# TrevorS/voxtral-mini-realtime-rs

Hardware: AMD Instinct MI355X
Metric: decode_tok_per_s (higher is better)
Workload: dtype f32

## Files before the change

voxtral-mini-realtime-rs_amd/csrc/vox_api.cpp:

```cpp
#include "../../include/voxtral_hip.h"
#include "vox_kernels.h"
#include "vox_page_pool.h"
#include "vox_host_base.h"

#include <dlfcn.h>
#include <fcntl.h>
#include <sys/mman.h>
#include <sys/stat.h>
#include <unistd.h>

#include <algorithm>
#include <array>
#include <cassert>
#include <chrono>
#include <cmath>
#include <cstdarg>
#include <cstdio>
#include <cstdlib>
#include <cstring>
#include <deque>
#include <map>
#include <mutex>
#include <string>
#include <unordered_map>
// ... 969 lines not shown

extern "C" int32_t vox_q4_model_load(vox_ctx* ctx, const char* path, vox_model** out) { return vox_q4_model_load_ex(ctx, path, 0, out); }

extern "C" int32_t vox_q4_model_load_gguf(vox_ctx* ctx, vox_gguf* g, uint32_t flags, vox_model** out) {
    ARGCHK(ctx && g && out, "null argument"); VOXCHK(ctx_bind(ctx));
    GgufSource src; src.g = g;
    const int32_t r = model_build(ctx, &src, true, (flags & VOX_LOAD_LAYOUT_ONLY) != 0, out);
    src.g = nullptr;
    return r;
}
extern "C" int32_t vox_q4_model_load_ex(vox_ctx* ctx, const char* path, uint32_t flags, vox_model** out) {
    ARGCHK(ctx && path && out, "null argument"); VOXCHK(ctx_bind(ctx));
    GgufSource src; VOXCHK(vox_gguf_open(path, &src.g));
    return model_build(ctx, &src, true, (flags & VOX_LOAD_LAYOUT_ONLY) != 0, out);
}

extern "C" int32_t vox_f32_model_load(vox_ctx* ctx, const char* path, vox_model** out) {
    ARGCHK(ctx && path && out, "null argument"); VOXCHK(ctx_bind(ctx));
    SafeTensorsSource src; VOXCHK(src.open(path));
    return model_build(ctx, &src, false, false, out);
}

extern "C" int32_t vox_model_config(const vox_model* m, vox_model_cfg* out) { ARGCHK(m && out, "null argument"); *out = m->cfg; return VOX_OK; }
extern "C" int32_t vox_model_weight_bytes(const vox_model* m, uint64_t* out) { ARGCHK(m && out, "null argument"); *out = m->arena_bytes; return VOX_OK; }
extern "C" int32_t vox_model_memory(const vox_model* m, uint64_t out[4]) {
    ARGCHK(m && out, "null argument");
    out[0] = m->arena_bytes; out[1] = m->arena_primary_bytes;
    out[2] = (m->eng_stream ? eng_stream_bytes(m->cfg.dec_layers, m->cfg.vocab) : 0) + (m->eng_wob ? engb_wo_stream_bytes(m->cfg.dec_layers) : 0);
    out[3] = m->eng_state ? eng_state_bytes() : 0;
    for (int gi = 0; gi < 4; gi++) if (m->engb_state[gi]) out[3] += engb_state_bytes();
    return VOX_OK;
}
extern "C" int32_t vox_model_arena(const vox_model* m, void** p, uint64_t* n) { ARGCHK(m && p && n, "null argument"); *p = m->arena; *n = m->arena_primary_bytes; return VOX_OK; }
extern "C" int32_t vox_model_arena_finalize(vox_model* m) {
    ARGCHK(m, "null argument"); VOXCHK(ctx_bind(m->ctx));
    for (Q4W* w : m->tiled) HIPCHK(launch_q4_tile_build(*w, const_cast<uint4*>(w->qt), const_cast<uint16_t*>(w->st), m->ctx->stream));
    HIPCHK(hipStreamSynchronize(m->ctx->stream));
    m->eng_ready = false; m->eng_offline.cache = nullptr;
    prefix_release(m);
    if (m->eng_wob) { HIPCHK(hipStreamSynchronize(m->ctx->stream)); (void)hipFree(m->eng_wob); m->eng_wob = nullptr; }
    graphs_destroy(m);
    return VOX_OK;
}

extern "C" int32_t vox_model_replicate(const vox_model* src, vox_ctx* dst_ctx, vox_model** out) {
    ARGCHK(src && dst_ctx && out, "null argument");
    if (!src->is_q4 || src->manifest.empty()) return fail(VOX_ERR_UNSUPPORTED, "vox_model_replicate: Q4 (GGUF) models only");
    VOXCHK(ctx_bind(src->ctx)); HIPCHK(hipStreamSynchronize(src->ctx->stream));
    VOXCHK(ctx_bind(dst_ctx));
    ManifestSource ms; ms.m = &src->manifest;
    vox_model* d = nullptr;
    VOXCHK(model_build(dst_ctx, &ms, true, true, &d));
    if (d->arena_primary_bytes != src->arena_primary_bytes || d->arena_bytes != src->arena_bytes) { model_release(d); return fail(VOX_ERR_INVALID, "internal: replica arena layout differs from the source's"); }
    hipError_t e = src->ctx->device == dst_ctx->device ? hipMemcpyAsync(d->arena, src->arena, src->arena_primary_bytes, hipMemcpyDeviceToDevice, dst_ctx->stream)
                                                       : hipMemcpyPeerAsync(d->arena, dst_ctx->device, src->arena, src->ctx->device, src->arena_primary_bytes, dst_ctx->stream);
    if (e == hipSuccess) e = hipStreamSynchronize(dst_ctx->stream);
    if (e != hipSuccess) { model_release(d); return fail(VOX_ERR_HIP, "vox_model_replicate: device copy failed: %s", hipGetErrorString(e)); }
    const int32_t r = vox_model_arena_finalize(d);
    if (r != VOX_OK) { model_release(d); return r; }
    *out = d; return VOX_OK;
}

extern "C" int32_t vox_model_set_t_embed(vox_model* m, const float* t_embed) {
    ARGCHK(m && t_embed, "null argument"); VOXCHK(ctx_bind(m->ctx));
    const vox_model_cfg& c = m->cfg; vox_ctx* cx = m->ctx;
    if (m->t_embed_set && m->t_embed_host.size() == (size_t)c.dec_dim && !std::memcmp(m->t_embed_host.data(), t_embed, (size_t)c.dec_dim * 4)) return VOX_OK;
    DevBuf dt, dh, ones; HIPCHK(dt.alloc((size_t)c.dec_dim * 4)); HIPCHK(dh.alloc((size_t)c.t_cond_dim * 4)); HIPCHK(ones.alloc((size_t)c.dec_dim * 4));
    std::vector<float> one(c.dec_dim, 1.0f);
    HIPCHK(hipMemcpyAsync(dt.p, t_embed, (size_t)c.dec_dim * 4, hipMemcpyHostToDevice, cx->stream));
    HIPCHK(hipMemcpyAsync(ones.p, one.data(), (size_t)c.dec_dim * 4, hipMemcpyHostToDevice, cx->stream));
    for (int i = 0; i < c.dec_layers; i++) {
        VOXCHK(q4_linear_dev(cx, m->dec[i].ada0.w, nullptr, dt.as<float>(), c.dec_dim, 1, dh.as<float>(), c.t_cond_dim, EPI_GELU));
        VOXCHK(q4_linear_dev(cx, m->dec[i].ada2.w, nullptr, dh.as<float>(), c.t_cond_dim, 1, m->dec[i].ada_mul, c.dec_dim, EPI_RESID, ones.as<float>(), c.dec_dim));
    }
    HIPCHK(hipStreamSynchronize(cx->stream));
    m->t_embed_host.assign(t_embed, t_embed + c.dec_dim); m->t_embed_set = true;
    m->pfx.dec_built = false;
    return VOX_OK;
}

static int conv_len(int L) { return (L + 2 - 3) / 2 + 1; }

static int32_t ensure(float** p, size_t* cap, size_t need) {
    if (*cap >= need) return VOX_OK;
    if (*p) HIPCHK(hipFree(*p));
    *p = nullptr; *cap = 0;
    HIPCHK(hipMalloc((void**)p, need * sizeof(float))); *cap = need; return VOX_OK;
}

static int enc_rows(int T) { return conv_len(conv_len(T)); }
static int enc_row_budget(const vox_model* m, const int* T, int n) {
    int mx = 0; for (int i = 0; i < n; i++) mx = std::max(mx, enc_rows(T[i]));
    const int r = m->cfg.reshape_factor; return n == 1 ? mx : (mx + r - 1) / r * r;
}
static size_t conv_scratch_floats(const vox_model* m, int T) {
    const int D = m->cfg.enc_dim, T1 = conv_len(T);
    return std::max((size_t)D * T1, (size_t)(T + 2) * m->cfg.n_mels + (size_t)(T1 + 2) * D) + 64;
}
static int32_t conv_stem_dev(vox_model* m, const float* d_mel, int T, float* c1, float* x) {
    const vox_model_cfg& c = m->cfg; hipStream_t s = m->ctx->stream; const int D = c.enc_dim, T1 = conv_len(T), S = conv_len(T1);
    const bool conv_mfma = m->conv1_g.qs && m->conv2_g.qs && !knob_str("VOX_CONV_VALU");
    if (conv_mfma) {
        const int Cm = c.n_mels;
        float* melT = c1; float* c1T = melT + (size_t)(T + 2) * Cm;
        HIPCHK(hipMemsetAsync(melT, 0, (size_t)Cm * 4, s)); HIPCHK(hipMemsetAsync(melT + (size_t)(T + 1) * Cm, 0, (size_t)Cm * 4, s));
        HIPCHK(hipMemsetAsync(c1T, 0, (size_t)D * 4, s)); HIPCHK(hipMemsetAsync(c1T + (size_t)(T1 + 1) * D, 0, (size_t)D * 4, s));
        HIPCHK(launch_transpose(d_mel, Cm, T, melT + Cm, s));
        { GemmParams g{}; g.w = m->conv1_g; g.x = melT; g.x_stride = 2 * Cm; g.M = T1; g.out = c1T + D; g.out_stride = D; g.bias = m->conv1_b; HIPCHK(launch_dense2_gemm(g, EPI_GELU, s)); }
        { GemmParams g{}; g.w = m->conv2_g; g.x = c1T; g.x_stride = 2 * D; g.M = S; g.out = x; g.out_stride = D; g.bias = m->conv2_b; HIPCHK(launch_dense2_gemm(g, EPI_GELU, s)); }
    } else {
        HIPCHK(launch_conv1d_gelu(d_mel, c.n_mels, T, m->conv1_w, m->conv1_b, D, c1, 0, s));
        HIPCHK(launch_conv1d_gelu(c1, D, T1, m->conv2_w, m->conv2_b, D, x, 1, s));
    }
    return VOX_OK;
}
static int enc_packed_rows_of(const vox_model* m, int T) { const int R = m->cfg.reshape_factor; return std::max((enc_rows(T) + R - 1) / R * R, R * 40); }
static long enc_packed_rows(const vox_model* m, const int* T, int n) { long r = 0; for (int i = 0; i < n; i++) r += enc_packed_rows_of(m, T[i]); return r; }
struct EncForms { long Mtot = 0; int ksp = 0, ksp_wo = 0, fused_rope = 0; };
static int32_t encode_batch_dev(vox_model* m, int n, const float* const* d_mels, const int* T, float* audio_out, int audio_rows, int* S4_out, long* audio_off_out = nullptr,
                                EncForms* forms = nullptr, int prefix_rows = 0) {
    const vox_model_cfg& c = m->cfg; vox_ctx* cx = m->ctx; hipStream_t s = cx->stream;
    const int D = c.enc_dim, H = c.enc_heads, hd = c.enc_head_dim, QD = H * hd, F = c.enc_ffn, R = c.reshape_factor;
    const bool packed = audio_off_out != nullptr;
    ARGCHK(n <= 128, "internal: encoder stack of %d utterances", n);
    const int S_pad = enc_row_budget(m, T, n);
    int T1max = 0; bool any = false;
    std::vector<int> S(n);
    for (int i = 0; i < n; i++) { S[i] = enc_rows(T[i]); S4_out[i] = S[i] / R; T1max = std::max(T1max, conv_len(T[i])); any = any || S4_out[i] > 0; }
    if (!any || S_pad <= 0) return VOX_OK;
    ARGCHK(S_pad <= m->enc_rope_len, "audio too long for the encoder RoPE table (%d > %d positions); chunk it (--max-mel-frames)", S_pad, m->enc_rope_len);
    std::vector<int> roff(n + 1, 0);
    if (packed) for (int i = 0; i < n; i++) roff[i + 1] = roff[i] + enc_packed_rows_of(m, T[i]);
    const int r0 = prefix_rows;
    ARGCHK(r0 == 0 || (n == 1 && !packed && r0 % R == 0 && r0 < S_pad && m->pfx.enc_built && r0 == m->pfx.RC), "internal: encoder prefix of %d rows", r0);
    const int Mfull = packed ? roff[n] : n * S_pad;
    const int Mtot = Mfull - r0, M4 = packed ? Mtot / R : n == 1 ? S4_out[0] - r0 / R : Mtot / R;
    ARGCHK(!m->pfx.capture || (n == 1 && !packed && r0 == 0 && m->pfx.capture_rows <= S_pad), "internal: prefix capture");
    ARGCHK(packed || n == 1 || audio_rows >= S_pad / R, "internal: audio row budget %d < %d", audio_rows, S_pad / R);
    int Tmax = 0; for (int i = 0; i < n; i++) Tmax = std::max(Tmax, T[i]);
    (void)T1max;
    const size_t c1_floats = conv_scratch_floats(m, Tmax);
    int ksp = 0;
    {
        const Q4W& w2 = m->enc[0].w2.w;
        const long wgs = (long)((w2.N + 127) / 128) * ((Mtot + 31) / 32);
        const bool geom_ok = w2.fmt == WFMT_Q4_0 && w2.qt && w2.st && w2.nb % 16 == 0 && Mtot > 48 && D % 4 == 0 && D <= 4096;
        if (geom_ok && wgs < 1024) ksp = 4;
        if (const char* e = knob_str("VOX_ENC_SPLITK")) ksp = geom_ok && atoi(e) > 1 ? std::min(atoi(e), w2.nb / 4) : 0;
        for (int l = 0; ksp && l < c.enc_layers; l++) if (m->enc[l].w2.w.fmt != WFMT_Q4_0 || !m->enc[l].w2.w.qt || m->enc[l].w2.w.nb / 4 < ksp) ksp = 0;
    }
    int ksp_wo = ksp ? 2 : 0;
    if (ksp) { if (const char* e = knob_str("VOX_ENC_SPLITK_WO")) ksp_wo = atoi(e) > 1 ? std::min(atoi(e), ksp) : 0; }
    for (int l = 0; ksp_wo && l < c.enc_layers; l++) if (m->enc[l].wo.w.fmt != WFMT_Q4_0 || !m->enc[l].wo.w.qt || m->enc[l].wo.w.nb / 4 < ksp_wo || m->enc[l].wo.w.nb % 4) ksp_wo = 0;
    const size_t need = c1_floats + (size_t)Mfull * D + (size_t)Mtot * D + (size_t)Mtot * QD * 4 + (size_t)Mtot * F + (size_t)(M4 + 1) * m->ad0.w.N + (size_t)ksp * Mtot * D + 1024;
    VOXCHK(ensure(&m->ws, &m->ws_floats, need));
    if (forms) { forms->Mtot = Mtot; forms->ksp = ksp; forms->ksp_wo = ksp_wo; forms->fused_rope = 0; }
    float* c1 = m->ws; float* x0 = c1 + c1_floats / 64 * 64; float* x = x0 + (size_t)r0 * D; float* xn = x0 + (size_t)Mfull * D; float* qkv = xn + (size_t)Mtot * D;
    float* att = qkv + (size_t)Mtot * QD * 3; float* ffn = att + (size_t)Mtot * QD; float* ah = ffn + (size_t)Mtot * F; float* w2p = ah + (size_t)(M4 + 1) * m->ad0.w.N;
    const int* d_len = nullptr; const int* d_roff = nullptr; const int* d_rpos = nullptr;
    if (n > 1 || packed) {
        HIPCHK(hipMemsetAsync(x, 0, (size_t)Mtot * D * 4, s));
        HIPCHK(hipMemsetAsync(att, 0, (size_t)Mtot * QD * 4, s));
        if (!m->d_seq_len) HIPCHK(hipMalloc((void**)&m->d_seq_len, 128 * sizeof(int)));
        m->h_seq_len.assign(S.begin(), S.end());
        HIPCHK(hipMemcpyAsync(m->d_seq_len, m->h_seq_len.data(), (size_t)n * 4, hipMemcpyHostToDevice, s));
        d_len = m->d_seq_len;
    }
    if (packed) {
        if (!m->d_seq_off) HIPCHK(hipMalloc((void**)&m->d_seq_off, 128 * sizeof(int)));
        if (m->row_pos_cap < (size_t)Mtot) { if (m->d_row_pos) { HIPCHK(hipStreamSynchronize(s)); HIPCHK(hipFree(m->d_row_pos)); } m->d_row_pos = nullptr; m->row_pos_cap = 0;
                                              HIPCHK(hipMalloc((void**)&m->d_row_pos, (size_t)Mtot * sizeof(int))); m->row_pos_cap = (size_t)Mtot; }
        HIPCHK(hipStreamSynchronize(s));
        m->h_seq_off.assign(roff.begin(), roff.begin() + n); m->h_row_pos.resize((size_t)Mtot);
        for (int i = 0; i < n; i++) for (int r = roff[i]; r < roff[i + 1]; r++) m->h_row_pos[(size_t)r] = std::min(r - roff[i], m->enc_rope_len - 1);
        HIPCHK(hipMemcpyAsync(m->d_seq_off, m->h_seq_off.data(), (size_t)n * 4, hipMemcpyHostToDevice, s)); HIPCHK(hipMemcpyAsync(m->d_row_pos, m->h_row_pos.data(), (size_t)Mtot * 4, hipMemcpyHostToDevice, s));
        d_roff = m->d_seq_off; d_rpos = m->d_row_pos;
    }
    for (int i = 0; i < n; i++) {
        if (S[i] <= 0) continue;
        VOXCHK(conv_stem_dev(m, d_mels[i], T[i], c1, x0 + (packed ? (size_t)roff[i] : (size_t)i * S_pad) * D));
    }
    const int seq_rows = packed ? 0 : n > 1 ? S_pad : 0;
    for (int l = 0; l < c.enc_layers; l++) {
        const EncLayer& L = m->enc[l];
        if (ksp && l > 0) HIPCHK(launch_rms_norm_sumk(x, D, Mtot, D, w2p, (size_t)Mtot * D, ksp, L.attn_norm, c.norm_eps, xn, D, s));
        else HIPCHK(launch_rms_norm(x, D, Mtot, D, L.attn_norm, nullptr, c.norm_eps, xn, D, s));
        if (Mtot > 48) {
            GemmParams g{}; g.w = L.wqkv.w; g.x = xn; g.x_stride = D; g.M = Mtot; g.out = qkv; g.out_stride = 3 * QD; g.bias = L.wqkv.bias;
            g.rope_cos = m->enc_cos + (size_t)r0 * (hd / 2); g.rope_sin = m->enc_sin + (size_t)r0 * (hd / 2);
            g.hd = hd; g.n_q = 2 * QD; g.pos = d_rpos; g.rope_seq_rows = seq_rows;
            bool fused = false; HIPCHK(launch_q4_gemm(g, EPI_ROPE_ROWS, s, &fused));
            if (forms && fused) forms->fused_rope++;
        } else {
            VOXCHK(q4_linear_dev(cx, L.wqkv.w, L.wqkv.bias, xn, D, Mtot, qkv, 3 * QD));
            HIPCHK(launch_rope(qkv, Mtot, 3 * QD, 2 * QD, hd, r0, m->enc_cos, m->enc_sin, s, seq_rows, d_rpos));
        }
        if (m->pfx.capture)
            HIPCHK(hipMemcpy2DAsync(m->pfx.capture + (size_t)l * m->pfx.capture_rows * 2 * QD, (size_t)2 * QD * 4, qkv + QD, (size_t)3 * QD * 4, (size_t)2 * QD * 4, (size_t)m->pfx.capture_rows,
                                    hipMemcpyDeviceToDevice, s));
        AttnParams ap{}; ap.q = qkv; ap.q_stride = 3 * QD; ap.k = qkv + QD; ap.v = qkv + 2 * QD; ap.kv_row_stride = 3 * QD; ap.kv_head_stride = hd;
        ap.out = att; ap.out_stride = QD; ap.M = S_pad - r0; ap.kv_len = S_pad; ap.n_heads = H; ap.n_kv_heads = H; ap.offset = r0; ap.window = c.enc_window;
        if (r0) { ap.prefix_k = m->pfx.enc_kv + (size_t)l * r0 * 2 * QD; ap.prefix_v = ap.prefix_k + QD; ap.prefix_len = r0; ap.prefix_row_stride = 2 * QD; ap.prefix_head_stride = hd; }
        ap.seq_len = d_len; ap.q_seq_stride = S_pad * 3 * QD; ap.out_seq_stride = S_pad * QD; ap.kv_seq_stride = (long)S_pad * 3 * QD; ap.seq_row_off = d_roff;
        HIPCHK(launch_attn_prefill(ap, hd, s, n));
        if (ksp_wo) {
            VOXCHK(q4_linear_dev(cx, L.wo.w, L.wo.bias, att, QD, Mtot, w2p, D, EPI_STORE, nullptr, 0, ksp_wo));
            HIPCHK(launch_rms_norm_sumk(x, D, Mtot, D, w2p, (size_t)Mtot * D, ksp_wo, L.ffn_norm, c.norm_eps, xn, D, s));
        } else {
            VOXCHK(q4_linear_dev(cx, L.wo.w, L.wo.bias, att, QD, Mtot, x, D, EPI_RESID, x, D));
            HIPCHK(launch_rms_norm(x, D, Mtot, D, L.ffn_norm, nullptr, c.norm_eps, xn, D, s));
        }
        VOXCHK(q4_linear_dev(cx, L.w13.w, nullptr, xn, D, Mtot, ffn, F, EPI_SWIGLU));
        if (ksp) VOXCHK(q4_linear_dev(cx, L.w2.w, L.w2.bias, ffn, F, Mtot, w2p, D, EPI_STORE, nullptr, 0, ksp));
        else VOXCHK(q4_linear_dev(cx, L.w2.w, L.w2.bias, ffn, F, Mtot, x, D, EPI_RESID, x, D));
    }
    if (ksp && c.enc_layers > 0) HIPCHK(launch_rms_norm_sumk(x, D, Mtot, D, w2p, (size_t)Mtot * D, ksp, m->enc_norm, c.norm_eps, xn, D, s));
    else HIPCHK(launch_rms_norm(x, D, Mtot, D, m->enc_norm, nullptr, c.norm_eps, xn, D, s));
    VOXCHK(q4_linear_dev(cx, m->ad0.w, nullptr, xn, D * R, M4, ah, m->ad0.w.N, EPI_GELU));
    if (packed) { for (int i = 0; i < n; i++) audio_off_out[i] = (long)(roff[i] / R) * c.dec_dim; }
    if (packed || n == 1 || audio_rows * R == S_pad) VOXCHK(q4_linear_dev(cx, m->ad2.w, nullptr, ah, m->ad0.w.N, M4, audio_out + (size_t)(r0 / R) * c.dec_dim, c.dec_dim));
    else for (int i = 0; i < n; i++)
        VOXCHK(q4_linear_dev(cx, m->ad2.w, nullptr, ah + (size_t)i * (S_pad / R) * m->ad0.w.N, m->ad0.w.N, S_pad / R, audio_out + (size_t)i * audio_rows * c.dec_dim, c.dec_dim));
    return VOX_OK;
}
static int32_t encode_dev(vox_model* m, const float* d_mel, int T, int* S4_out, int prefix_rows = 0) {
    const int S4 = enc_rows(T) / m->cfg.reshape_factor;
    if (S4 > 0) { size_t cap = (size_t)m->audio_cap * m->cfg.dec_dim; VOXCHK(ensure(&m->d_audio, &cap, (size_t)S4 * m->cfg.dec_dim)); m->audio_cap = (int)(cap / m->cfg.dec_dim); }
    return encode_batch_dev(m, 1, &d_mel, &T, m->d_audio, S4, S4_out, nullptr, nullptr, prefix_rows);
}

static int32_t cache_alloc(vox_model* m, int max_seq, vox_cache** out) {
    const vox_model_cfg& c = m->cfg;
    ARGCHK(max_seq > 0 && max_seq <= m->dec_rope_len, "max_seq %d out of range (1..%d)", max_seq, m->dec_rope_len);
    vox_cache* k = new vox_cache(); k->m = m; k->ctx = m->ctx; k->max_seq = max_seq;
    const size_t n = (size_t)c.dec_layers * c.dec_kv_heads * max_seq * c.dec_head_dim * 4;
    if (hipMalloc((void**)&k->k, n) != hipSuccess || hipMalloc((void**)&k->v, n) != hipSuccess) { if (k->k) (void)hipFree(k->k); delete k; return fail(VOX_ERR_HIP, "hipMalloc of KV cache failed"); }
    HIPCHK(hipMemsetAsync(k->k, 0, n, m->ctx->stream)); HIPCHK(hipMemsetAsync(k->v, 0, n, m->ctx->stream));
    k->layer_stride = (size_t)c.dec_kv_heads * max_seq * c.dec_head_dim;
    cache_register(k);
    *out = k; return VOX_OK;
}
extern "C" int32_t vox_decoder_cache_create(vox_model* m, int32_t max_seq, vox_cache** out) { ARGCHK(m && out, "null argument"); VOXCHK(ctx_bind(m->ctx)); return cache_alloc(m, max_seq, out); }
extern "C" int32_t vox_cache_free(vox_cache* k) {
    if (!k) return VOX_OK;
    (void)hipSetDevice(k->ctx->device); (void)hipStreamSynchronize(k->ctx->stream);
    cache_release(k); return VOX_OK;
}
static int32_t pw_sync(vox_model* m);
static int32_t cache_settle_pending(vox_cache* kc) {
    vox_model* m = kc->m;
    if (m && m->pw_pend_rows > 0 && m->pw_pend_cache == kc) { VOXCHK(ctx_bind(kc->ctx)); VOXCHK(pw_sync(m)); }
    return VOX_OK;
}
extern "C" int32_t vox_cache_update(vox_cache* kc, int32_t layer, int32_t pos, const float* k, const float* v, int32_t n_rows, int32_t mem_kind) {
    ARGCHK(kc && k && v && n_rows > 0 && pos >= 0, "bad argument"); VOXCHK(ctx_bind(kc->ctx)); VOXCHK(cache_settle_pending(kc));
    const vox_model_cfg& c = kc->m->cfg;
    const int L = kc->kind == 1 ? c.enc_layers : c.dec_layers, H = kc->kind == 1 ? c.enc_heads : c.dec_kv_heads, hd = kc->kind == 1 ? c.enc_head_dim : c.dec_head_dim;
    ARGCHK(layer >= 0 && layer < L, "layer %d out of range (0..%d)", layer, L - 1);
    ARGCHK(pos + n_rows <= kc->max_seq, "KV cache overflow: %d + %d > %d", pos, n_rows, kc->max_seq);
    hipStream_t s = kc->ctx->stream; const hipMemcpyKind kind = mem_kind == VOX_MEM_DEVICE ? hipMemcpyDeviceToDevice : hipMemcpyHostToDevice;
    for (int h = 0; h < H; h++) {
        const size_t dst = (size_t)layer * kc->layer_stride + ((size_t)h * kc->max_seq + pos) * hd, src = (size_t)h * n_rows * hd, nb = (size_t)n_rows * hd * 4;
        HIPCHK(hipMemcpyAsync(kc->k + dst, k + src, nb, kind, s)); HIPCHK(hipMemcpyAsync(kc->v + dst, v + src, nb, kind, s));
    }
    if (mem_kind != VOX_MEM_DEVICE) HIPCHK(hipStreamSynchronize(s));
    kc->len = std::max(kc->len, pos + n_rows);
    return VOX_OK;
}
extern "C" int32_t vox_cache_truncate(vox_cache* kc, int32_t len) {
    ARGCHK(kc, "null cache"); VOXCHK(cache_settle_pending(kc)); ARGCHK(len >= 0 && len <= kc->len, "truncate to %d: the cache holds %d rows", len, kc->len);
    if (kc->kind == 1) kc->abs_pos -= kc->len - len;
    kc->len = len; return VOX_OK;
}
extern "C" int32_t vox_cache_seq_len(const vox_cache* k, int32_t* out) { ARGCHK(k && out, "null argument"); *out = k->len; return VOX_OK; }
extern "C" int32_t vox_cache_reset(vox_cache* k) {
    ARGCHK(k, "null cache");
    (void)cache_settle_pending(k);
    k->len = 0; k->abs_pos = 0; return VOX_OK;
}

extern "C" int32_t vox_encoder_cache_create(vox_model* m, int32_t capacity_rows, vox_cache** out) {
    ARGCHK(m && out, "null argument"); VOXCHK(ctx_bind(m->ctx));
    const vox_model_cfg& c = m->cfg;
    if (capacity_rows <= 0) capacity_rows = 2 * c.enc_window + 512;
    ARGCHK(capacity_rows > c.enc_window, "encoder cache capacity %d must exceed the sliding window (%d)", capacity_rows, c.enc_window);
    vox_cache* k = new vox_cache(); k->m = m; k->ctx = m->ctx; k->max_seq = capacity_rows; k->kind = 1;
    const size_t n = (size_t)c.enc_layers * c.enc_heads * capacity_rows * c.enc_head_dim * 4;
    if (hipMalloc((void**)&k->k, n) != hipSuccess || hipMalloc((void**)&k->v, n) != hipSuccess) { if (k->k) (void)hipFree(k->k); delete k; return fail(VOX_ERR_HIP, "hipMalloc of encoder KV cache failed"); }
    HIPCHK(hipMemsetAsync(k->k, 0, n, m->ctx->stream)); HIPCHK(hipMemsetAsync(k->v, 0, n, m->ctx->stream));
    k->layer_stride = (size_t)c.enc_heads * capacity_rows * c.enc_head_dim;
    cache_register(k);
    *out = k; return VOX_OK;
}
extern "C" int32_t vox_cache_abs_pos(const vox_cache* k, int32_t* out) { ARGCHK(k && out, "null argument"); *out = k->kind == 1 ? k->abs_pos : k->len; return VOX_OK; }

static int32_t enc_cache_evict(vox_model* m, vox_cache* kc, int keep) {
    const vox_model_cfg& c = m->cfg; hipStream_t s = m->ctx->stream;
    if (keep >= kc->len) return VOX_OK;
    const size_t planes = (size_t)c.enc_layers * c.enc_heads, pitch = (size_t)kc->max_seq * c.enc_head_dim * 4, width = (size_t)keep * c.enc_head_dim * 4;
    VOXCHK(ensure(&m->ws, &m->ws_floats, planes * width / 4 + 64));
    for (float* base : {kc->k, kc->v}) {
        const char* src = reinterpret_cast<const char*>(base) + (size_t)(kc->len - keep) * c.enc_head_dim * 4;
        HIPCHK(hipMemcpy2DAsync(m->ws, width, src, pitch, width, planes, hipMemcpyDeviceToDevice, s));
        HIPCHK(hipMemcpy2DAsync(base, pitch, m->ws, width, width, planes, hipMemcpyDeviceToDevice, s));
    }
    kc->len = keep;
    return VOX_OK;
}
extern "C" int32_t vox_encoder_cache_apply_sliding_window(vox_cache* kc, int32_t window) {
    ARGCHK(kc && kc->kind == 1 && window > 0, "bad argument"); VOXCHK(ctx_bind(kc->ctx));
    VOXCHK(enc_cache_evict(kc->m, kc, window)); HIPCHK(hipStreamSynchronize(kc->ctx->stream)); return VOX_OK;
}

static int32_t enc_stream_rope_ensure(vox_model* m) {
    if (m->enc_cos_s) return VOX_OK;
    const vox_model_cfg& c = m->cfg; const int hd = c.enc_head_dim;
    const int len = 1 << 16, half = hd / 2; std::vector<float> ct((size_t)len * half), st((size_t)len * half);
    for (int i = 0; i < len; i++) for (int j = 0; j < half; j++) { const float inv = 1.0f / std::pow(c.rope_theta, (float)(2 * j) / (float)hd), fr = (float)i * inv; ct[(size_t)i * half + j] = std::cos(fr); st[(size_t)i * half + j] = std::sin(fr); }
    HIPCHK(hipMalloc((void**)&m->enc_cos_s, ct.size() * 4)); HIPCHK(hipMalloc((void**)&m->enc_sin_s, st.size() * 4));
    HIPCHK(hipMemcpy(m->enc_cos_s, ct.data(), ct.size() * 4, hipMemcpyHostToDevice)); HIPCHK(hipMemcpy(m->enc_sin_s, st.data(), st.size() * 4, hipMemcpyHostToDevice));
    m->enc_rope_s_len = len;
    return VOX_OK;
}
static int32_t encode_with_cache_dev(vox_model* m, const float* d_mel, int T, vox_cache* kc, int* S4_out) {
    const vox_model_cfg& c = m->cfg; vox_ctx* cx = m->ctx; hipStream_t s = cx->stream;
    const int D = c.enc_dim, H = c.enc_heads, hd = c.enc_head_dim, QD = H * hd, F = c.enc_ffn, R = c.reshape_factor;
    const int S = enc_rows(T), S4 = S / R; *S4_out = S4;
    if (S <= 0) return VOX_OK;
    ARGCHK(S <= kc->max_seq - std::min(c.enc_window, kc->max_seq - 1), "chunk of %d encoder rows does not fit a cache of %d rows next to the %d-row window", S, kc->max_seq, c.enc_window);
    if (kc->len + S > kc->max_seq) VOXCHK(enc_cache_evict(m, kc, std::min(kc->len, c.enc_window)));
    const float *cos_t = m->enc_cos, *sin_t = m->enc_sin;
    if (kc->abs_pos + S > m->enc_rope_len) {
        VOXCHK(enc_stream_rope_ensure(m));
        ARGCHK(kc->abs_pos + S <= m->enc_rope_s_len, "stream of %d encoder positions exceeds the streaming RoPE table (%d)", kc->abs_pos + S, m->enc_rope_s_len);
        cos_t = m->enc_cos_s; sin_t = m->enc_sin_s;
    }
    if (S4 > 0) { size_t cap = (size_t)m->audio_cap * c.dec_dim; VOXCHK(ensure(&m->d_audio, &cap, (size_t)S4 * c.dec_dim)); m->audio_cap = (int)(cap / c.dec_dim); }
    const size_t c1f = conv_scratch_floats(m, T);
    const size_t need = c1f + (size_t)S * D * 2 + (size_t)S * QD * 4 + (size_t)S * F + (size_t)(S4 + 1) * m->ad0.w.N + 1024;
    VOXCHK(ensure(&m->ws, &m->ws_floats, need));
    float* c1 = m->ws; float* x = c1 + c1f / 64 * 64; float* xn = x + (size_t)S * D; float* qkv = xn + (size_t)S * D;
    float* att = qkv + (size_t)S * QD * 3; float* ffn = att + (size_t)S * QD; float* ah = ffn + (size_t)S * F;
    VOXCHK(conv_stem_dev(m, d_mel, T, c1, x));
    const int off = kc->len; const size_t lf = kc->layer_stride;
    for (int l = 0; l < c.enc_layers; l++) {
        const EncLayer& L = m->enc[l]; float* kl = kc->k + (size_t)l * lf; float* vl = kc->v + (size_t)l * lf;
        HIPCHK(launch_rms_norm(x, D, S, D, L.attn_norm, nullptr, c.norm_eps, xn, D, s));
        VOXCHK(q4_linear_dev(cx, L.wqkv.w, L.wqkv.bias, xn, D, S, qkv, 3 * QD));
        HIPCHK(launch_rope(qkv, S, 3 * QD, 2 * QD, hd, kc->abs_pos, cos_t, sin_t, s, 0));
        HIPCHK(launch_kv_store(qkv, S, 3 * QD, QD, H, hd, off, kl, vl, kc->max_seq * hd, s));
        AttnParams ap{}; ap.q = qkv; ap.q_stride = 3 * QD; ap.k = kl; ap.v = vl; ap.kv_row_stride = hd; ap.kv_head_stride = kc->max_seq * hd;
        ap.out = att; ap.out_stride = QD; ap.M = S; ap.kv_len = off + S; ap.n_heads = H; ap.n_kv_heads = H; ap.offset = off; ap.window = c.enc_window;
        HIPCHK(launch_attn_prefill(ap, hd, s, 1));
        VOXCHK(q4_linear_dev(cx, L.wo.w, L.wo.bias, att, QD, S, x, D, EPI_RESID, x, D));
        HIPCHK(launch_rms_norm(x, D, S, D, L.ffn_norm, nullptr, c.norm_eps, xn, D, s));
        VOXCHK(q4_linear_dev(cx, L.w13.w, nullptr, xn, D, S, ffn, F, EPI_SWIGLU));
        VOXCHK(q4_linear_dev(cx, L.w2.w, L.w2.bias, ffn, F, S, x, D, EPI_RESID, x, D));
    }
    kc->len = off + S; kc->abs_pos += S;
    if (S4 > 0) {
        HIPCHK(launch_rms_norm(x, D, S4 * R, D, m->enc_norm, nullptr, c.norm_eps, xn, D, s));
        VOXCHK(q4_linear_dev(cx, m->ad0.w, nullptr, xn, D * R, S4, ah, m->ad0.w.N, EPI_GELU));
        VOXCHK(q4_linear_dev(cx, m->ad2.w, nullptr, ah, m->ad0.w.N, S4, m->d_audio, c.dec_dim));
    }
    return VOX_OK;
}
// ... 3218 lines not shown
```

voxtral-mini-realtime-rs_amd/csrc/vox_kernels.h:

```cpp
#pragma once
#include <hip/hip_runtime.h>
#include <atomic>
struct DevOnce {
    std::atomic<uint64_t> mask{0};
    bool done(int dev) const { return (mask.load(std::memory_order_acquire) >> (dev & 63)) & 1ull; }
    void set(int dev) { mask.fetch_or(1ull << (dev & 63), std::memory_order_release); }
};
static inline int vox_current_device() { int d = 0; if (hipGetDevice(&d) != hipSuccess) { (void)hipGetLastError(); d = 0; } return d; }
#include <stdint.h>

namespace vox {

struct Q4W {
    const uint4* qs;
    const uint16_t* sc;
    int N, K, nb;
    int fmt;
    const uint4* qt = nullptr; const uint16_t* st = nullptr;
};
enum WFmt { WFMT_Q4_0 = 0, WFMT_BF16 = 1, WFMT_BF16X2 = 2, WFMT_F32 = 3 };

enum Epi { EPI_STORE = 0, EPI_RESID = 1, EPI_SWIGLU = 2, EPI_ROPE_KV = 3, EPI_ARGMAX = 4, EPI_GELU = 5, EPI_SWIGLU_XF = 6, EPI_RESID_XF = 7,
           EPI_ROPE_ROWS = 8,
           EPI_ROPE_KV_PAGED = 9 };
enum Pro { PRO_NONE = 0, PRO_RMS = 1, PRO_RMS_MUL = 2,
           PRO_RMS_MUL_SUM = 3 };

struct GemvParams {
    Q4W w;
    const float* x; int x_stride;
    float* out; int out_stride;
    const float* bias;
    const float* resid; int resid_stride;
    const float* gamma; const float* mul; float eps;
    long long* zero_acc; int zero_n;
    const long long* xacc; float* x_out;
    const int* pos_ptr; int pos_off;
    const float* rope_cos; const float* rope_sin; int hd;
    int n_q, n_k;
    float* kcache; float* vcache; int cache_head_stride;
    float* part_val; int* part_idx;
    int tl_slot;
};
hipError_t launch_q4_gemv(const GemvParams& p, int n_rows_x, int pro, int epi, int R, hipStream_t s);
const char* q4_gemv_kernel_name(int K, int pro, int epi, int R);
int q4_gemv_default_R(int N, int K, int epi);
int q4_gemv_grid(int N, int R);
int q4_gemv_nwv(int K, int epi);
int q4_gemv_grid_k(int N, int K, int R, int epi);
int dense_gemv_grid(int N);

struct GemmParams {
    Q4W w;
    const float* x; int x_stride; int M;
    float* out; int out_stride;
    const float* bias;
    const float* resid; int resid_stride;
    const uint4* xf;
    uint16_t* xf_scratch; size_t xf_scratch_bytes;
    const float* ssq_part; int n_part; float norm_eps;
    uint16_t* xf_out; const float* xf_w; const float* xf_w2; float* ssq_out;
    const int* pos; const float* rope_cos; const float* rope_sin; int hd, n_q, n_kv; float* kc; float* vc; long kv_seq_stride; int kv_head_stride;
    const int* kv_row;
    const int* kv_pos;
    int tl_slot;
    int ksplit;
    float* kz_scratch; size_t kz_scratch_bytes;
    int rope_seq_rows;
    int wide_mt; long xf_gstride , xf_out_gstride , ssq_part_gstride, ssq_out_gstride ;
    int wide_rows;
};
struct WidePlan { int kz, sps, ntw; };
bool q4_wide_plan(const Q4W& w, int mt, int epi, WidePlan* pl);
size_t q4_wide_planes_bytes(const Q4W& w, int mt, const WidePlan& pl);
hipError_t launch_q4_wide(const GemmParams& p, int epi, hipStream_t s);
hipError_t launch_q4_tile_build(Q4W w, uint4* qt, uint16_t* st, hipStream_t s);
hipError_t launch_q4_gemm(const GemmParams& p, int epi, hipStream_t s, bool* fused_rope = nullptr);
hipError_t launch_dense2_gemm(const GemmParams& p, int epi, hipStream_t s);
hipError_t launch_transpose(const float* in, int R, int C, float* out, hipStream_t s);
int q4_skinny_resid_xf_parts(int N);

hipError_t launch_q4_repack(const uint8_t* raw, uint4* qs, uint16_t* sc, int64_t n_blocks, int nb, int row_mul, int row_add, hipStream_t s);
hipError_t launch_q4_dequant(Q4W w, float* out, hipStream_t s);
hipError_t launch_rms_norm(const float* x, int x_stride, int rows, int dim, const float* gamma, const float* mul,
                           float eps, float* out, int out_stride, hipStream_t s);
hipError_t launch_rms_norm_sumk(float* x, int x_stride, int rows, int dim, const float* part, size_t part_stride, int ksplit, const float* gamma, float eps, float* out, int out_stride, hipStream_t s);
int q4_skinny_mt2_plan(const Q4W& w, int M);
hipError_t launch_xf_rows(const float* x, int x_stride, int M, int K, uint16_t* xf, hipStream_t s);
hipError_t launch_q4_skinny_mt2_planes(const GemmParams& p, int KZ, hipStream_t s);
hipError_t launch_splitk_finish_resid(const float* planes, int KZ, int M, int N, float* x, int x_stride, hipStream_t s);
hipError_t launch_splitk_finish_swiglu_xf(const float* planes, int KZ, int M, int N, const float* bias, uint16_t* xf, hipStream_t s);
hipError_t launch_splitk_finish_rope_kv(const float* planes, int KZ, int M, int N, float* q_out, int q_stride, int n_q, int n_kv, int hd, int pos_off,
                                        const float* cos_t, const float* sin_t, float* kc, float* vc, int head_stride, hipStream_t s);
hipError_t launch_rms_norm_xf_sumk(float* x, int x_stride, int rows, int dim, const float* planes, int kz, const float* gamma, const float* mul, float eps, uint16_t* xf, hipStream_t s);
hipError_t launch_rms_norm_xf(const float* x, int x_stride, int rows, int dim, const float* gamma, const float* mul,
                              float eps, uint16_t* xf, hipStream_t s);
hipError_t launch_rope(float* buf, int M, int stride, int n_rot, int hd, int pos_off, const float* cos_t,
                       const float* sin_t, hipStream_t s, int seq_rows = 0, const int* row_pos = nullptr);
hipError_t launch_kv_store(const float* buf, int M, int stride, int k_col, int n_kv, int hd, int pos_off,
                           float* kcache, float* vcache, int cache_head_stride, hipStream_t s, int seq_rows = 0, long kv_seq_stride = 0);

struct AttnParams {
    const float* q; int q_stride;
    const float* k; const float* v;
    int kv_row_stride, kv_head_stride;
    float* out; int out_stride;
    int M, kv_len, n_heads, n_kv_heads, offset, window;
    const int* pos_ptr;
    int pos_per_seq; int q_seq_stride, out_seq_stride; long kv_seq_stride;
    const int* kv_row;
    const int* seq_len;
    const int* seq_row_off;
    uint16_t* out_xf_tiles; long out_xf_tile_stride;
    uint16_t* out_xf;
    long out_xf_gstride;
    int prefer_gqa;
    int no_xcd_remap;
    int tl_slot;
    int spec_zero;
    int spec_rows;
    const float* prefix_k; const float* prefix_v; int prefix_len, prefix_row_stride, prefix_head_stride;
    const int* page_tab; int page_tab_stride, page_shift, score_rows; long page_floats;
};
hipError_t launch_attn_prefill(const AttnParams& p, int hd, hipStream_t s, int n_seq = 1);
bool attn_prefill_prefix_ok(const AttnParams& p, int hd, int n_seq);
bool attn_prefill_small_ok(const AttnParams& p, int hd, int n_seq);
hipError_t launch_attn_decode(const AttnParams& p, int hd, int max_seq, hipStream_t s, int n_seq = 1);
hipError_t launch_attn_decode_paged(const AttnParams& p, int hd, hipStream_t s, int n_seq);
bool attn_wo_supported(const AttnParams& p, const Q4W& wo, int hd, int max_seq);
hipError_t launch_attn_wo(const AttnParams& p, const Q4W& wo, long long* acc, int max_seq, hipStream_t s);
enum AttnForm { ATTN_FORM_PREFILL_SMALL, ATTN_FORM_PREFILL_MFMA, ATTN_FORM_PREFILL_F32, ATTN_FORM_DECODE, ATTN_FORM_DECODE_SPEC, ATTN_FORM_DECODE_GQA, ATTN_FORM_WO,
                ATTN_FORM_ENGINE, ATTN_FORM_STREAM_RING, ATTN_FORM_GROUP_RESAMPLE, ATTN_FORM_STREAM_RESAMPLE,
                ATTN_FORM_DECODE_PAGED, ATTN_FORM_DECODE_GQA_PAGED,
                ATTN_FORM_COUNT };
void attn_form_note(AttnForm f);
void attn_form_counts(unsigned long long out[ATTN_FORM_COUNT]);
enum GemmForm { GEMM_FORM_GEMV_R1, GEMM_FORM_GEMV_R2, GEMM_FORM_GEMV_R4, GEMM_FORM_DENSE_GEMV, GEMM_FORM_SKINNY, GEMM_FORM_SKINNY_MT, GEMM_FORM_SKINNY_MT2, GEMM_FORM_XF_ROWS,
                GEMM_FORM_SPLITK_FINISH, GEMM_FORM_TILE_11, GEMM_FORM_TILE_12, GEMM_FORM_TILE_21, GEMM_FORM_TILE_22, GEMM_FORM_TILE_21_TB, GEMM_FORM_TILE_22_TB, GEMM_FORM_K32,
                GEMM_FORM_BIG, GEMM_FORM_BIG_ROPE, GEMM_FORM_DENSE2, GEMM_FORM_WIDE, GEMM_FORM_COUNT };
void gemm_form_counts(unsigned long long out[GEMM_FORM_COUNT]);

hipError_t launch_conv1d_gelu(const float* in, int Cin, int L, const float* w, const float* b, int Cout, float* out,
                              int out_token_major, hipStream_t s);

struct MelTables { const float* window; const float* cos_t; const float* sin_t; const float* fb; const int* fb_lo; const int* fb_hi; };
hipError_t launch_mel(const float* audio, long n, long left, long right, const float* scale_ptr, MelTables t,
                      float* out, int T, int transposed, hipStream_t s);
hipError_t launch_resample_matrix(const double* H, int new_len, int fft_in, int fft_out, float* At, hipStream_t s);
hipError_t launch_resample(const float* x, long n_in, const float* At, int fft_in, int fft_out, int delay, float* out, long n_out, hipStream_t s);
hipError_t launch_absmax(const float* x, long n, float target_peak, float* scale_out, hipStream_t s);
hipError_t launch_absmax_group(const float* x, long n, unsigned* group_max_cell, hipStream_t s);
hipError_t launch_group_scale(const unsigned* group_max, const int* unit_group, int n, float target, float* unit_scale, hipStream_t s);

hipError_t launch_embed(Q4W tok, const int* ids, int n, const float* audio, int D, const int* pos_ptr, int id_off,
                        int a_off, float* out, hipStream_t s);
hipError_t launch_argmax_final(const float* part_val, const int* part_idx, int n_parts, int* tokens, int* pos_ptr,
                               int tok_off, int inc, hipStream_t s);
hipError_t launch_argmax_embed(const float* part_val, const int* part_idx, int n_parts, int* tokens, int* pos_ptr, Q4W tok,
                               const float* audio, int D, float* h, hipStream_t s);
hipError_t launch_rope_kv_batch(float* qkv, int n, int stride, int n_q, int n_kv, int hd, const int* pos, const float* cos_t, const float* sin_t,
                                float* kcache, float* vcache, long seq_stride, int head_stride, hipStream_t s);
hipError_t launch_argmax_embed_batch(const float* logits, int n, int vocab, int* tokens, int tok_stride, int* pos, const int* seq_len, Q4W tok,
                                     const float* audio, long audio_seq_stride, int D, float* h, hipStream_t s,
                                     uint16_t* xf = nullptr, const float* xf_w = nullptr, float* ssq_out = nullptr,
                                     long xf_group_stride = 0, int ssq_group_stride = 0,
                                     const long* audio_off = nullptr);
struct SlotStepParams {
    const float* logits; int vocab;
    int* tokens; int tok_stride; const int* clip_len;
    int* slot_clip; int* slot_qpos; const int* queue; int q_stride;
    int* pos; int* kv_row; int n_clips; int first_pos;
    Q4W tok; const float* audio; const long* audio_off; int D;
    const float* h0;
    float* h;
    uint16_t* xf; const float* xf_w; float* ssq_out; long xf_group_stride; int ssq_group_stride;
    int init;
};
hipError_t launch_argmax_embed_slots(const SlotStepParams& p, int n_slots, hipStream_t s);
struct BatchTapParams {
    const float* logits; int vocab;
    const int* slot_clip; int clip0; const int* pos; const int* seq_len;
    const int* clip_unit; int n_clips;
    float* out; int* rows; int n_units, max_rows, first_pos;
};
hipError_t launch_batch_tap(const BatchTapParams& p, int n_rows, hipStream_t s);
hipError_t launch_occupy(int workgroups, int micros, hipStream_t s);
hipError_t launch_add_rows(const float* a, const float* b, float* out, long n, hipStream_t s);
hipError_t launch_gelu(float* x, long n, hipStream_t s);
hipError_t launch_argmax_rows(const float* x, int rows, int V, int* out, hipStream_t s);

struct EngLayerTab { const float* attn_norm; const float* ffn_norm; const float* ada_mul; float* kc; float* vc; };
struct EngParams {
    const unsigned char* stream; size_t cu_stride;
    const EngLayerTab* layers; int n_layers;
    const float* h_in;
    const float* final_norm;
    const int* pos_ptr; int pos_off;
    const float* rope_cos; const float* rope_sin;
    int max_seq, window; float eps;
    unsigned long long *H0, *H1, *G, *PW, *A, *P2;
    unsigned long long *SS0, *SS1;
    unsigned long long* XC;
    unsigned* serial; unsigned* err;
    float* part_val; int* part_idx;
    int* tokens; int* pos_rw; const uint4* tok_qs; const uint16_t* tok_sc; int tok_nb; const float* audio;
    float* logits_out;
    int vocab;
    unsigned long long* tl; int tl_layer;
    int flags;
    int ag_delay_ticks;
    int pace_ticks;
};
bool eng_geometry_ok(int D, int n_heads, int n_kv, int hd, int ffn, int vocab, int max_seq);
size_t eng_stream_bytes(int n_layers, int vocab);
size_t eng_state_bytes();
hipError_t launch_eng_pack(const Q4W& w, int op, int layer, int n_layers, unsigned char* stream, int vocab, hipStream_t s);
void eng_state_carve(unsigned char* state, EngParams* p);
hipError_t launch_decode_engine(const EngParams& p, hipStream_t s);
hipError_t launch_eng_hidden(const EngParams& p, float* out, hipStream_t s);
hipError_t eng_occupancy(int* blocks_per_cu);
int eng_lds_bytes();

struct EngBParams {
    const unsigned char* stream;
    const unsigned char* stream_wo;
    const EngLayerTab* layers; int n_layers;
    long kv_seq_stride;
    const float* h_in; int h_stride; int n_rows;
    const float* final_norm;
    const int* pos;
    const int* kv_row;
    const float* rope_cos; const float* rope_sin;
    int max_seq, window; float eps;
    unsigned char *XH0, *XH1;
    float *SS0, *SS1;
    unsigned long long* G;
    unsigned char* XO;
    float* PW;
    unsigned char* XA;
    float* P2;
    unsigned *F0, *F1, *FO, *FW, *FA, *F2;
    unsigned long long* XC; unsigned* serial; unsigned* err;
    uint16_t* xf_out; float* ssq_out;
    unsigned long long* tl; int tl_layer;
    int flags;
};
size_t engb_state_bytes();
size_t engb_wo_stream_bytes(int n_layers);
void engb_state_carve(unsigned char* state, EngBParams* p);
hipError_t engb_state_init(unsigned char* state, hipStream_t s);
hipError_t launch_decode_engine_b16(const EngBParams& p, hipStream_t s);
hipError_t launch_decode_engine_b16x2(const EngBParams& a, const EngBParams& b, hipStream_t s);
hipError_t engb_occupancy(int* blocks_per_cu);
hipError_t engb_prepare_kernels();
hipError_t launch_engb_ssq_fold(const float* ssq256, float* ssq16, hipStream_t s);
int engb_lds_bytes();
int engb_lds_bytes2();

void knobs_load_once();
void knobs_reload();
#define VOX_NO_PK_F32 __attribute__((target("no-packed-fp32-ops")))
const char* knob_str(const char* name);

hipError_t tl_configure(unsigned long long* buf, int n_slots, int n_waves);
int tl_slots_used();
void tl_slot_meta(int slot, int out[4]);

enum StreamWord { STRM_POS = 0,
                  STRM_ENC_POS = 1,
                  STRM_FRAME = 2,
                  STRM_HEAD = 3,
                  STRM_TICKS = 4,
                  STRM_TAP_ROWS = 5,
                  STRM_WORDS = 16 };
struct TokenScore { float logprob, margin; int runner_up, id; };
static const int VOX_ALTS_MAX = 8;
struct TokenAlt { int id; float logprob; };
struct TokenAlts { float entropy; int n; TokenAlt alt[VOX_ALTS_MAX]; };
// ... 65 lines not shown
```

voxtral-mini-realtime-rs_amd/csrc/vox_kernels.hip:

```cpp
#include "vox_kernels.h"

#include <hip/hip_fp16.h>

#include <unistd.h>

#include <algorithm>
#include <atomic>
#include <cstdio>
#include <cstdlib>
#include <cstring>
#include <string>
#include <mutex>
#include <unordered_map>

namespace vox {

static int g_tl_next = -1, g_tl_slots = 0;
#ifdef VOX_TIMELINE
__device__ unsigned long long* g_tl_buf = nullptr;
__device__ int g_tl_waves = 0;
__device__ __forceinline__ void tl_stamp(int slot, int wave_global, int k) {
    if (slot >= 0 && (wave_global & 3) == 0 && (threadIdx.x & 63) == 0 && g_tl_buf && wave_global < g_tl_waves)
        g_tl_buf[((size_t)slot * g_tl_waves + wave_global) * 4 + k] = wall_clock64();
}
// ... 555 lines not shown
    __syncthreads();
    int best_i = 0x7fffffff; float best = -INFINITY;
    const int pos = (EPI == EPI_ROPE_KV) ? (p.pos_ptr ? *p.pos_ptr : 0) + p.pos_off : 0;
    const int n_groups = N / R, n_waves = gridDim.x * 4;
    for (int g = blockIdx.x * 4 + wave; g < n_groups; g += n_waves) {
        const int row0 = g * R;
        const uint4* w0 = (F32W ? p.w.qt : p.w.qs) + (size_t)row0 * nc * (F32W ? 2 : 1);
        const uint4* w1 = w0 + nc * (F32W ? 2 : 1);
        float acc[R] = {0.f, 0.f};
        for (int c0 = 0; c0 < nc; c0 += 128) {
            const int ca = c0 + lane, cb = ca + 64, cca = min(ca, nc - 1), ccb = min(cb, nc - 1);
            const float4 xea = xe[cca], xoa = xo[cca], xeb = xe[ccb], xob = xo[ccb];
            const float ma = ca < nc ? 1.0f : 0.0f, mb = cb < nc ? 1.0f : 0.0f;
            if (F32W) {
                const uint4 a0e = ld_nt_u4(w0 + 2 * cca), a0o = ld_nt_u4(w0 + 2 * cca + 1), a1e = ld_nt_u4(w0 + 2 * ccb), a1o = ld_nt_u4(w0 + 2 * ccb + 1);
                const uint4 b0e = ld_nt_u4(w1 + 2 * cca), b0o = ld_nt_u4(w1 + 2 * cca + 1), b1e = ld_nt_u4(w1 + 2 * ccb), b1o = ld_nt_u4(w1 + 2 * ccb + 1);
                acc[0] += ma * dot8_f32(a0e, a0o, xea, xoa) + mb * dot8_f32(a1e, a1o, xeb, xob);
                acc[1] += ma * dot8_f32(b0e, b0o, xea, xoa) + mb * dot8_f32(b1e, b1o, xeb, xob);
            } else {
                const uint4 a0 = ld_nt_u4(w0 + cca), a1 = ld_nt_u4(w0 + ccb), b0 = ld_nt_u4(w1 + cca), b1 = ld_nt_u4(w1 + ccb);
                acc[0] += ma * dot8_bf16(a0, xea, xoa) + mb * dot8_bf16(a1, xeb, xob);
                acc[1] += ma * dot8_bf16(b0, xea, xoa) + mb * dot8_bf16(b1, xeb, xob);
            }
        }
        acc[0] = wave_sum(acc[0]); acc[1] = wave_sum(acc[1]);
        if (EPI == EPI_STORE || EPI == EPI_RESID || EPI == EPI_GELU) {
#pragma unroll
            for (int r = 0; r < R; r++) {
                const int n = row0 + r;
                if (lane == r) {
                    float v = acc[r];
                    if (p.bias) v += p.bias[n];
                    if (EPI == EPI_RESID) v = v + p.resid[(size_t)y * p.resid_stride + n];
                    if (EPI == EPI_GELU) v = gelu_f(v);
                    p.out[(size_t)y * p.out_stride + n] = v;
                }
            }
        } else if (EPI == EPI_SWIGLU) {
            if (lane == 0) p.out[(size_t)y * p.out_stride + (row0 >> 1)] = silu_f(acc[0]) * acc[1];
        } else if (EPI == EPI_ROPE_KV) {
            const int hd = p.hd, half = hd >> 1, n = row0;
            if (lane == 0) {
                const float a = acc[0], b = acc[1];
                if (n < p.n_q + p.n_k) {
                    const int dd = n % hd;
                    const float c = p.rope_cos[(size_t)pos * half + (dd >> 1)], sn = p.rope_sin[(size_t)pos * half + (dd >> 1)];
                    const float ra = a * c - b * sn, rb = a * sn + b * c;
                    if (n < p.n_q) { p.out[n] = ra; p.out[n + 1] = rb; }
                    else {
                        const int kn = n - p.n_q, kh = kn / hd;
                        float* dst = p.kcache + (size_t)kh * p.cache_head_stride + (size_t)pos * hd + dd;
                        dst[0] = ra; dst[1] = rb;
                    }
                } else {
                    const int vn = n - p.n_q - p.n_k, vh = vn / hd, dd = vn % hd;
                    float* dst = p.vcache + (size_t)vh * p.cache_head_stride + (size_t)pos * hd + dd;
                    dst[0] = a; dst[1] = b;
                }
            }
        } else if (EPI == EPI_ARGMAX) {
#pragma unroll
            for (int r = 0; r < R; r++) {
                const int n = row0 + r;
                if (p.out && lane == r) p.out[(size_t)y * p.out_stride + n] = acc[r];
                argmax_take(best, best_i, acc[r], n);
            }
        }
    }
    if (EPI == EPI_ARGMAX) {
        if (lane == 0) { red[4 + wave] = best; reinterpret_cast<int*>(red)[8 + wave] = best_i; }
        __syncthreads();
        if (tid == 0) {
            float bv = red[4]; int bidx = reinterpret_cast<int*>(red)[8];
            for (int wv = 1; wv < 4; wv++) argmax_take(bv, bidx, red[4 + wv], reinterpret_cast<int*>(red)[8 + wv]);
            p.part_val[(size_t)y * gridDim.x + blockIdx.x] = bv;
            p.part_idx[(size_t)y * gridDim.x + blockIdx.x] = bidx;
        }
    }
}

int dense_gemv_grid(int N) { const int wgs = (N / 2 + 3) / 4; return wgs > 2048 ? 2048 : (wgs < 1 ? 1 : wgs); }

template <int PRO, int EPI>
static hipError_t dense_launch_t(const GemvParams& p, int ny, hipStream_t s) {
    const size_t lds = (size_t)(p.w.K + 16) * sizeof(float);
    gemm_form_note(GEMM_FORM_DENSE_GEMV);
    if (p.w.fmt == WFMT_F32) dense_gemv_kernel<PRO, EPI, 1><<<dim3(dense_gemv_grid(p.w.N), ny), dim3(256), lds, s>>>(p);
    else dense_gemv_kernel<PRO, EPI, 0><<<dim3(dense_gemv_grid(p.w.N), ny), dim3(256), lds, s>>>(p);
    return hipGetLastError();
}
static hipError_t launch_dense_gemv(const GemvParams& p, int ny, int pro, int epi, hipStream_t s) {
    if (p.w.K % 32 || p.w.K > 10240 || p.w.N % 2) return hipErrorInvalidValue;
    if ((pro == PRO_RMS_MUL || pro == PRO_RMS_MUL_SUM) && p.mul == nullptr) return hipErrorInvalidValue;
    if (pro == PRO_RMS_MUL_SUM) return hipErrorInvalidValue;
#define VOX_CASE(P_, E_) if (pro == P_ && epi == E_) return dense_launch_t<P_, E_>(p, ny, s)
    VOX_CASE(PRO_NONE, EPI_STORE); VOX_CASE(PRO_NONE, EPI_RESID); VOX_CASE(PRO_NONE, EPI_GELU); VOX_CASE(PRO_NONE, EPI_SWIGLU);
    VOX_CASE(PRO_RMS, EPI_STORE); VOX_CASE(PRO_RMS, EPI_ARGMAX); VOX_CASE(PRO_RMS, EPI_SWIGLU); VOX_CASE(PRO_RMS_MUL, EPI_SWIGLU);
    VOX_CASE(PRO_RMS, EPI_ROPE_KV);
#undef VOX_CASE
    return hipErrorInvalidValue;
}

typedef __attribute__((__vector_size__(8 * sizeof(__bf16)))) __bf16 bf16x8;
typedef __attribute__((__vector_size__(4 * sizeof(float)))) float f32x4;

__device__ __forceinline__ uint32_t bf16_rne_bits(float x) {
    const uint32_t u = __float_as_uint(x);
    return (u + 0x7FFFu + ((u >> 16) & 1u)) >> 16;
}
typedef __bf16 bf16x2_t __attribute__((ext_vector_type(2)));
typedef float f32x2_t __attribute__((ext_vector_type(2)));
__device__ __forceinline__ uint32_t cvt_pk_bf16(float a, float b) {
    const f32x2_t v = {a, b};
    union { bf16x2_t b; uint32_t u; } c; c.b = __builtin_convertvector(v, bf16x2_t); return c.u;
}
__device__ __forceinline__ void split_pair(float a, float b, uint32_t& hi, uint32_t& lo) {
    hi = cvt_pk_bf16(a, b);
    lo = cvt_pk_bf16(a - __uint_as_float(hi << 16), b - __uint_as_float(hi & 0xFFFF0000u));
}
__device__ __forceinline__ void split_bf16x8(const float4 a, const float4 b, uint4& hi, uint4& lo) {
    split_pair(a.x, a.y, hi.x, lo.x); split_pair(a.z, a.w, hi.y, lo.y);
    split_pair(b.x, b.y, hi.z, lo.z); split_pair(b.z, b.w, hi.w, lo.w);
}
__device__ __forceinline__ uint32_t pack_bf16_exact(float a, float b) {
    return (__float_as_uint(a) >> 16) | (__float_as_uint(b) & 0xFFFF0000u);
}
__device__ __forceinline__ uint4 q4_dword_to_bf16x8(uint32_t w) {
    const uint32_t lo = w & 0x0F0F0F0Fu, hi = (w >> 4) & 0x0F0F0F0Fu;
    uint4 o;
    o.x = pack_bf16_exact(ub0(lo) - 8.0f, ub1(lo) - 8.0f);
    o.y = pack_bf16_exact(ub2(lo) - 8.0f, ub3(lo) - 8.0f);
    o.z = pack_bf16_exact(ub0(hi) - 8.0f, ub1(hi) - 8.0f);
    o.w = pack_bf16_exact(ub2(hi) - 8.0f, ub3(hi) - 8.0f);
    return o;
}
__device__ __forceinline__ bf16x8 as_bf16x8(uint4 v) {
    union { uint4 u; bf16x8 b; } c; c.u = v; return c.b;
}

__device__ __forceinline__ uint4 q4_dword_to_bf16x8_biased(uint32_t w) {
    const uint32_t lo = w & 0x0F0F0F0Fu, hi = (w >> 4) & 0x0F0F0F0Fu, c = 0x43434343u;
    return make_uint4(__builtin_amdgcn_perm(lo, c, 0x00060004u), __builtin_amdgcn_perm(hi, c, 0x00060004u),
                      __builtin_amdgcn_perm(lo, c, 0x00070005u), __builtin_amdgcn_perm(hi, c, 0x00070005u));
}

__device__ __forceinline__ void xf_store4(uint16_t* __restrict__ xf, int K, int row, int k, float4 v) {
    const int q = k >> 7, j = (k >> 5) & 3, e = k & 31, half = e >> 4, g = (e & 15) >> 2;
    const size_t base = ((size_t)((q * 4 + j) * 64 + g * 16 + row)) * 8 + 2 * half;
    const size_t plane = (size_t)(K >> 7) * 256 * 8;
    uint32_t hi, lo;
    split_pair(v.x, v.z, hi, lo); *reinterpret_cast<uint32_t*>(xf + base) = hi; *reinterpret_cast<uint32_t*>(xf + plane + base) = lo;
    split_pair(v.y, v.w, hi, lo); *reinterpret_cast<uint32_t*>(xf + base + 4) = hi; *reinterpret_cast<uint32_t*>(xf + plane + base + 4) = lo;
}

template <int EPI, int FMT>
__global__ __launch_bounds__(256) __attribute__((amdgpu_waves_per_eu(2))) void q4_gemm_k32_kernel(const GemmParams p) {
    __shared__ __attribute__((aligned(16))) uint4 lds[2][2][256];
    const int K = p.w.K, nb = p.w.nb, N = p.w.N, M = p.M;
    (void)K;
    const int tid = threadIdx.x, lane = tid & 63, wave = tid >> 6;
    const int m0 = blockIdx.y * 64, n0 = blockIdx.x * 64;
    const int sm = tid >> 2, sg = tid & 3;
    const bool srow_ok = (m0 + sm) < M;
    const float* xrow = p.x + (size_t)(srow_ok ? (m0 + sm) : 0) * p.x_stride;
    const int slot = ((sm >> 4) * 4 + sg) * 16 + (sm & 15);
    const int wn = n0 + wave * 16 + (lane & 15), wg = lane >> 4;
    const bool wrow_ok = wn < N;
    const uint32_t* wq = reinterpret_cast<const uint32_t*>(p.w.qs) + (size_t)(wrow_ok ? wn : 0) * nb * 4 + wg;
    const uint16_t* ws = FMT == WFMT_Q4_0 ? p.w.sc + (size_t)(wrow_ok ? wn : 0) * nb : nullptr;
    const uint4* wd16 = p.w.qs + (size_t)(wrow_ok ? wn : 0) * nb * 4 + wg;
    const int xoff_a = FMT == WFMT_Q4_0 ? 4 * sg : 8 * sg, xoff_b = FMT == WFMT_Q4_0 ? 16 + 4 * sg : 8 * sg + 4;

    f32x4 acc[4];
#pragma unroll
    for (int i = 0; i < 4; i++) acc[i] = (f32x4){0.f, 0.f, 0.f, 0.f};

#define VOX_GLOAD(B_)                                                                              \
    xa = *reinterpret_cast<const float4*>(xrow + 32 * (B_) + xoff_a);        \
    xb = *reinterpret_cast<const float4*>(xrow + 32 * (B_) + xoff_b);                                               \
    if (FMT == WFMT_Q4_0) { wd = wq[(size_t)(B_) * 4]; wsc = ws[(B_)]; }    \
    else { wdv = wd16[(size_t)(B_) * 4]; }
#define VOX_STAGE(BUF_)                                                                            \
    { uint4 hi_, lo_; split_bf16x8(xa, xb, hi_, lo_); lds[(BUF_)][0][slot] = hi_; lds[(BUF_)][1][slot] = lo_; }
    float4 xa, xb; uint32_t wd = 0; uint16_t wsc = 0; uint4 wdv = make_uint4(0, 0, 0, 0);
    VOX_GLOAD(0)
    VOX_STAGE(0)
    uint32_t cur_wd = wd; uint16_t cur_sc = wsc; uint4 cur_wdv = wdv;
    { const int b1 = min(1, nb - 1); VOX_GLOAD(b1) }
    __syncthreads();
    for (int b = 0; b < nb; b++) {
        const int buf = b & 1;
        const float4 sxa = xa, sxb = xb; const uint32_t swd = wd; const uint16_t ssc = wsc; const uint4 swdv = wdv;
        { const int b2 = min(b + 2, nb - 1); VOX_GLOAD(b2) }
        const bf16x8 bw = as_bf16x8(FMT == WFMT_Q4_0 ? q4_dword_to_bf16x8(cur_wd) : cur_wdv);
        const float d = FMT == WFMT_Q4_0 ? f16_bits_to_f32(cur_sc) : 1.0f;
#pragma unroll
        for (int mt = 0; mt < 4; mt++) {
            const bf16x8 ah = as_bf16x8(lds[buf][0][mt * 64 + lane]);
            const bf16x8 al = as_bf16x8(lds[buf][1][mt * 64 + lane]);
            f32x4 t = __builtin_amdgcn_mfma_f32_16x16x32_bf16(ah, bw, (f32x4){0.f, 0.f, 0.f, 0.f}, 0, 0, 0);
            t = __builtin_amdgcn_mfma_f32_16x16x32_bf16(al, bw, t, 0, 0, 0);
            acc[mt][0] = fmaf(d, t[0], acc[mt][0]); acc[mt][1] = fmaf(d, t[1], acc[mt][1]);
            acc[mt][2] = fmaf(d, t[2], acc[mt][2]); acc[mt][3] = fmaf(d, t[3], acc[mt][3]);
        }
        if (b + 1 < nb) {
            uint4 hi_, lo_; split_bf16x8(sxa, sxb, hi_, lo_); lds[buf ^ 1][0][slot] = hi_; lds[buf ^ 1][1][slot] = lo_;
            cur_wd = swd; cur_sc = ssc; cur_wdv = swdv;
        }
        __syncthreads();
    }
#undef VOX_GLOAD
#undef VOX_STAGE
    const float bias = (p.bias && wrow_ok) ? p.bias[wn] : 0.f;
#pragma unroll
    for (int mt = 0; mt < 4; mt++)
#pragma unroll
        for (int r = 0; r < 4; r++) {
            const int m = m0 + mt * 16 + 4 * (lane >> 4) + r;
            float v = acc[mt][r] + bias;
            if (EPI == EPI_SWIGLU) {
                const float other = dpp_mov<0xB1>(v);
                if (m < M && wrow_ok && !(wn & 1)) p.out[(size_t)m * p.out_stride + (wn >> 1)] = silu_f(v) * other;
            } else if (m < M && wrow_ok) {
                if (EPI == EPI_RESID) v = v + p.resid[(size_t)m * p.resid_stride + wn];
                if (EPI == EPI_GELU) v = gelu_f(v);
                p.out[(size_t)m * p.out_stride + wn] = v;
            }
        }
}

template <int MT, int NT, int EPI, int FMT, int TB = 0>
__global__ __launch_bounds__(256) __attribute__((amdgpu_waves_per_eu(2))) void q4_gemm_kernel(const GemmParams p) {
    extern __shared__ __attribute__((aligned(16))) uint4 glds[];
    constexpr int PLANE = 4 * MT * 64, BUF = 2 * PLANE;
    const int nb = p.w.nb, N = p.w.N, M = p.M, nq = nb >> 2;
    const int tid = threadIdx.x, lane = tid & 63, wave = tid >> 6;
    const int m0 = blockIdx.y * (16 * MT), n0 = blockIdx.x * (64 * NT);
    const int KSP = p.ksplit > 1 ? p.ksplit : 1, kz = blockIdx.z;
    const int qb = (int)((long)nq * kz / KSP), qe = (int)((long)nq * (kz + 1) / KSP);
    const float* xrow[MT]; int slot[MT], xo_a[MT], xo_b[MT];
#pragma unroll
    for (int i = 0; i < MT; i++) {
        const int f = tid + 256 * i, sm = f >> 4, j = (f >> 2) & 3, g = f & 3;
        xrow[i] = p.x + (size_t)min(m0 + sm, M - 1) * p.x_stride;
        slot[i] = (j * MT + (sm >> 4)) * 64 + g * 16 + ((sm & 15) ^ (4 * j + g));
        xo_a[i] = 32 * j + (FMT == WFMT_Q4_0 ? 4 * g : 8 * g); xo_b[i] = 32 * j + (FMT == WFMT_Q4_0 ? 16 + 4 * g : 8 * g + 4);
    }
    const int wg = lane >> 4;
    int rdl[4];
#pragma unroll
    for (int j = 0; j < 4; j++) rdl[j] = (lane & 48) | ((lane & 15) ^ (4 * j + wg));
    const uint32_t* wq[NT]; const uint16_t* ws[NT]; const uint4* wd16[NT]; const uint4* wqt[NT]; int wn[NT]; bool wok[NT];
#pragma unroll
    for (int t = 0; t < NT; t++) {
        wn[t] = n0 + (wave * NT + t) * 16 + (lane & 15); wok[t] = wn[t] < N;
        const size_t row = (size_t)min(wn[t], N - 1);
        wq[t] = reinterpret_cast<const uint32_t*>(p.w.qs) + row * nb * 4 + wg;
        ws[t] = FMT == WFMT_Q4_0 ? p.w.sc + row * nb : nullptr;
        wd16[t] = p.w.qs + row * nb * 4 + wg;
        const size_t T = (size_t)min((n0 >> 4) + wave * NT + t, ((N + 15) >> 4) - 1);
        wqt[t] = TB ? p.w.qt + T * nq * 64 + lane : nullptr;
    }
    f32x4 acc[NT][MT];
#pragma unroll
    for (int t = 0; t < NT; t++)
#pragma unroll
        for (int i = 0; i < MT; i++) acc[t][i] = (f32x4){0.f, 0.f, 0.f, 0.f};

    float4 xa[MT], xb[MT];
    uint32_t wd[NT][4]; uint2 wsc[NT]; uint4 wdv[NT][4];
#define VOX_GLOAD(Q_)                                                                                          \
    _Pragma("unroll") for (int i = 0; i < MT; i++) {                                                           \
        xa[i] = *reinterpret_cast<const float4*>(xrow[i] + 128 * (Q_) + xo_a[i]);                              \
        xb[i] = *reinterpret_cast<const float4*>(xrow[i] + 128 * (Q_) + xo_b[i]);                              \
    }                                                                                                          \
    _Pragma("unroll") for (int t = 0; t < NT; t++) {                                                           \
        if (FMT == WFMT_Q4_0) {                                                                                \
            if (TB) { const uint4 w4 = ld_nt_u4(wqt[t] + (size_t)64 * (Q_)); wd[t][0] = w4.x; wd[t][1] = w4.y; wd[t][2] = w4.z; wd[t][3] = w4.w; } \
            else { _Pragma("unroll") for (int j = 0; j < 4; j++) wd[t][j] = wq[t][(size_t)(4 * (Q_) + j) * 4]; } \
            wsc[t] = *reinterpret_cast<const uint2*>(ws[t] + 4 * (Q_));                                        \
        } else {                                                                                               \
            _Pragma("unroll") for (int j = 0; j < 4; j++) wdv[t][j] = wd16[t][(size_t)(4 * (Q_) + j) * 4];     \
        }                                                                                                      \
    }
#define VOX_STAGE(BUF_)                                                                                        \
    _Pragma("unroll") for (int i = 0; i < MT; i++) {                                                           \
        uint4 hi_, lo_; split_bf16x8(sxa[i], sxb[i], hi_, lo_);                                                \
        glds[(BUF_) * BUF + slot[i]] = hi_; glds[(BUF_) * BUF + PLANE + slot[i]] = lo_;                        \
    }
    VOX_GLOAD(qb)
    float4 sxa[MT], sxb[MT];
#pragma unroll
    for (int i = 0; i < MT; i++) { sxa[i] = xa[i]; sxb[i] = xb[i]; }
    VOX_STAGE(0)
    uint32_t cwd[NT][4]; uint2 csc[NT]; uint4 cwdv[NT][4];
#pragma unroll
    for (int t = 0; t < NT; t++) { csc[t] = wsc[t];
#pragma unroll
        for (int j = 0; j < 4; j++) { cwd[t][j] = wd[t][j]; cwdv[t][j] = wdv[t][j]; } }
    { const int q1 = min(qb + 1, qe - 1); VOX_GLOAD(q1) }
    __syncthreads();
    for (int q = qb; q < qe; q++) {
        const int buf = (q - qb) & 1;
#pragma unroll
        for (int i = 0; i < MT; i++) { sxa[i] = xa[i]; sxb[i] = xb[i]; }
        uint32_t nwd[NT][4]; uint2 nsc[NT]; uint4 nwdv[NT][4];
#pragma unroll
        for (int t = 0; t < NT; t++) { nsc[t] = wsc[t];
#pragma unroll
            for (int j = 0; j < 4; j++) { nwd[t][j] = wd[t][j]; nwdv[t][j] = wdv[t][j]; } }
        { const int q2 = min(q + 2, qe - 1); VOX_GLOAD(q2) }
#pragma unroll
        for (int j = 0; j < 4; j++) {
#pragma unroll
            for (int t = 0; t < NT; t++) {
                const bf16x8 bw = as_bf16x8(FMT == WFMT_Q4_0 ? q4_dword_to_bf16x8(cwd[t][j]) : cwdv[t][j]);
                float d = 1.0f;
                if (FMT == WFMT_Q4_0) {
                    const uint32_t pr = (j & 2) ? csc[t].y : csc[t].x;
                    d = f16_bits_to_f32((uint16_t)((j & 1) ? (pr >> 16) : (pr & 0xFFFFu)));
                }
#pragma unroll
                for (int i = 0; i < MT; i++) {
                    const bf16x8 ah = as_bf16x8(glds[buf * BUF + (j * MT + i) * 64 + rdl[j]]);
                    const bf16x8 al = as_bf16x8(glds[buf * BUF + PLANE + (j * MT + i) * 64 + rdl[j]]);
                    f32x4 tt = __builtin_amdgcn_mfma_f32_16x16x32_bf16(ah, bw, (f32x4){0.f, 0.f, 0.f, 0.f}, 0, 0, 0);
                    tt = __builtin_amdgcn_mfma_f32_16x16x32_bf16(al, bw, tt, 0, 0, 0);
                    acc[t][i][0] = fmaf(d, tt[0], acc[t][i][0]); acc[t][i][1] = fmaf(d, tt[1], acc[t][i][1]);
                    acc[t][i][2] = fmaf(d, tt[2], acc[t][i][2]); acc[t][i][3] = fmaf(d, tt[3], acc[t][i][3]);
                }
            }
        }
        if (q + 1 < qe) {
            VOX_STAGE(buf ^ 1)
#pragma unroll
            for (int t = 0; t < NT; t++) { csc[t] = nsc[t];
#pragma unroll
                for (int j = 0; j < 4; j++) { cwd[t][j] = nwd[t][j]; cwdv[t][j] = nwdv[t][j]; } }
        }
        __syncthreads();
    }
#undef VOX_GLOAD
#undef VOX_STAGE
#pragma unroll
    for (int t = 0; t < NT; t++) {
        const float bias = (p.bias && wok[t] && kz == 0) ? p.bias[wn[t]] : 0.f;
#pragma unroll
        for (int i = 0; i < MT; i++)
#pragma unroll
            for (int r = 0; r < 4; r++) {
                const int m = m0 + i * 16 + 4 * (lane >> 4) + r;
                float v = acc[t][i][r] + bias;
                if (EPI == EPI_SWIGLU) {
                    const float other = dpp_mov<0xB1>(v);
                    if (m < M && wok[t] && !(wn[t] & 1)) p.out[(size_t)m * p.out_stride + (wn[t] >> 1)] = silu_f(v) * other;
                } else if (m < M && wok[t]) {
                    if (EPI == EPI_RESID) v = v + p.resid[(size_t)m * p.resid_stride + wn[t]];
                    if (EPI == EPI_GELU) v = gelu_f(v);
                    (p.out + (size_t)kz * p.M * p.out_stride)[(size_t)m * p.out_stride + wn[t]] = v;
                }
            }
    }
}

__global__ void q4_tile_build_kernel(Q4W w, uint4* __restrict__ qt, uint16_t* __restrict__ st, int n_tiles) {
    const int nq = w.nb >> 2;
    const long total = (long)n_tiles * nq * 64;
    for (long i = (long)blockIdx.x * blockDim.x + threadIdx.x; i < total; i += (long)gridDim.x * blockDim.x) {
        const int lane = (int)(i & 63); const long tq = i >> 6; const int q = (int)(tq % nq), T = (int)(tq / nq);
        const int g = lane >> 4, n = T * 16 + (lane & 15);
        uint32_t d[4] = {0x88888888u, 0x88888888u, 0x88888888u, 0x88888888u};
        if (n < w.N) {
            const uint32_t* src = reinterpret_cast<const uint32_t*>(w.qs) + ((size_t)n * w.nb + 4 * q) * 4 + g;
#pragma unroll
            for (int j = 0; j < 4; j++) d[j] = src[j * 4];
        }
        qt[i] = make_uint4(d[0], d[1], d[2], d[3]);
        if (g == 0) {
#pragma unroll
            for (int j = 0; j < 4; j++) st[(tq * 16 + (lane & 15)) * 4 + j] = n < w.N ? w.sc[(size_t)n * w.nb + 4 * q + j] : (uint16_t)0;
        }
    }
}
hipError_t launch_q4_tile_build(Q4W w, uint4* qt, uint16_t* st, hipStream_t s) {
    if (w.nb % 4) return hipErrorInvalidValue;
    const int n_tiles = (w.N + 15) / 16;
    q4_tile_build_kernel<<<dim3(2048), dim3(256), 0, s>>>(w, qt, st, n_tiles);
    return hipGetLastError();
}

template <int NTW, int EPI, int TILED, int XIN, int PRO, int STEPS = 0>
__global__ __launch_bounds__(NTW == 3 ? 256 : 512, NTW == 3 ? 3 : 1) void q4_skinny_kernel(const GemmParams p) {
    extern __shared__ __attribute__((aligned(16))) float sred[];
    __shared__ float s_rstd[16]; __shared__ float s_pp[32 * 16];
    constexpr bool KVP = EPI == EPI_ROPE_KV_PAGED, ROPE_KV = EPI == EPI_ROPE_KV || KVP;
    const int nb = p.w.nb, N = p.w.N, M = p.M, nq = nb >> 2;
    const int tid = threadIdx.x, lane = tid & 63, wave = tid >> 6, KS = blockDim.x >> 6;
    const int g = lane >> 4, li = lane & 15;
    const int nbase = blockIdx.x * (16 * NTW);
    const int tlw = wave == 0 ? (int)blockIdx.x * 4 : 1; (void)tlw;
    VOX_TL(p.tl_slot, tlw, 0);
    const float* xrow = p.x + (size_t)min(li, M - 1) * p.x_stride;
    const uint4* wq[NTW]; const uint16_t* ws[NTW];
    const int n_tiles = (N + 15) >> 4;
#pragma unroll
    for (int t = 0; t < NTW; t++) {
        if (TILED) {
            const size_t T = (size_t)min(blockIdx.x * NTW + t, n_tiles - 1);
            wq[t] = p.w.qt + T * nq * 64 + lane; ws[t] = p.w.st + (T * nq * 16 + li) * 4;
        } else {
            const size_t row = (size_t)min(nbase + t * 16 + li, N - 1);
            wq[t] = p.w.qs + row * nb + g; ws[t] = p.w.sc + row * nb;
        }
    }
    f32x4 acc[NTW];
#pragma unroll
    for (int t = 0; t < NTW; t++) acc[t] = (f32x4){0.f, 0.f, 0.f, 0.f};
    uint4 wv[NTW], wvn[NTW]; uint2 sv[NTW], svn[NTW]; float4 xa[4], xb[4];
    const uint4* xfh = p.xf + lane; const uint4* xfl = p.xf + (size_t)nq * 256 + lane;
#define VOX_WLOAD(WV_, SV_, Q_)                                                                            \
    _Pragma("unroll") for (int t = 0; t < NTW; t++) {                                                      \
        WV_[t] = ld_nt_u4(wq[t] + (TILED ? 64 : 4) * (Q_)); SV_[t] = *reinterpret_cast<const uint2*>(ws[t] + (TILED ? 64 : 4) * (Q_)); }
#define VOX_XLOAD(Q_)                                                                                      \
    _Pragma("unroll") for (int j = 0; j < 4; j++) {                                                        \
        if (XIN) {                                                                                         \
            xa[j] = *reinterpret_cast<const float4*>(xfh + ((Q_) * 4 + j) * 64);                           \
            xb[j] = *reinterpret_cast<const float4*>(xfl + ((Q_) * 4 + j) * 64);                           \
        } else {                                                                                           \
            xa[j] = *reinterpret_cast<const float4*>(xrow + 128 * (Q_) + 32 * j + 4 * g);                  \
            xb[j] = *reinterpret_cast<const float4*>(xrow + 128 * (Q_) + 32 * j + 16 + 4 * g); } }
#define VOX_SSTEP(WV_, SV_, XA_, XB_)                                                                      \
    {                                                                                                      \
        const bf16x8 m136 = as_bf16x8(make_uint4(0xC308C308u, 0xC308C308u, 0xC308C308u, 0xC308C308u));     \
        uint32_t dw[NTW][4];                                                                               \
        _Pragma("unroll") for (int t = 0; t < NTW; t++) {                                                  \
            dw[t][0] = WV_[t].x; dw[t][1] = WV_[t].y; dw[t][2] = WV_[t].z; dw[t][3] = WV_[t].w;            \
            if (!TILED) {                            \
                auto s01 = __builtin_amdgcn_permlane16_swap(WV_[t].x, WV_[t].y, false, false);             \
                auto s23 = __builtin_amdgcn_permlane16_swap(WV_[t].z, WV_[t].w, false, false);             \
                auto u02 = __builtin_amdgcn_permlane32_swap(s01[0], s23[0], false, false);                 \
                auto u13 = __builtin_amdgcn_permlane32_swap(s01[1], s23[1], false, false);                 \
                dw[t][0] = u02[0]; dw[t][1] = u13[0]; dw[t][2] = u02[1]; dw[t][3] = u13[1];                \
            }                                                                                              \
        }                                                                                                  \
               \
        _Pragma("unroll") for (int j = 0; j < 4; j++) {                                                    \
            uint4 ah, al;                                                                                  \
            if (XIN) {                                                                                     \
                ah = make_uint4(__float_as_uint(XA_[j].x), __float_as_uint(XA_[j].y), __float_as_uint(XA_[j].z), __float_as_uint(XA_[j].w)); \
                al = make_uint4(__float_as_uint(XB_[j].x), __float_as_uint(XB_[j].y), __float_as_uint(XB_[j].z), __float_as_uint(XB_[j].w)); \
            } else {                                                                                       \
                split_pair(XA_[j].x, XA_[j].z, ah.x, al.x); split_pair(XB_[j].x, XB_[j].z, ah.y, al.y);    \
                split_pair(XA_[j].y, XA_[j].w, ah.z, al.z); split_pair(XB_[j].y, XB_[j].w, ah.w, al.w);    \
            }                                                                                              \
            const f32x4 sx = __builtin_amdgcn_mfma_f32_16x16x32_bf16(as_bf16x8(ah), m136, (f32x4){0.f, 0.f, 0.f, 0.f}, 0, 0, 0); \
            const f32x4 cs = __builtin_amdgcn_mfma_f32_16x16x32_bf16(as_bf16x8(al), m136, sx, 0, 0, 0);    \
            _Pragma("unroll") for (int t = 0; t < NTW; t++) {                                              \
                const bf16x8 bw = as_bf16x8(q4_dword_to_bf16x8_biased(dw[t][j]));                          \
                const uint32_t sc2 = (j >> 1) ? SV_[t].y : SV_[t].x;                                       \
                const float d = f16_bits_to_f32((uint16_t)((j & 1) ? (sc2 >> 16) : (sc2 & 0xFFFFu)));      \
                f32x4 tt = __builtin_amdgcn_mfma_f32_16x16x32_bf16(as_bf16x8(ah), bw, cs, 0, 0, 0);        \
                tt = __builtin_amdgcn_mfma_f32_16x16x32_bf16(as_bf16x8(al), bw, tt, 0, 0, 0);              \
                acc[t] = __builtin_elementwise_fma((f32x4){d, d, d, d}, tt, acc[t]);                        \
            }                                                                                              \
        }                                                                                                  \
    }
    float pv[12]; const int prow = tid & 15, pch = tid >> 4, nch = blockDim.x >> 4;
    float pre_res[4] = {0.f, 0.f, 0.f, 0.f}; float pre_xw = 0.f; int pre_pos[4] = {0, 0, 0, 0}; int pre_row[4] = {0, 0, 0, 0}; int pre_kvp[4] = {0, 0, 0, 0};
#define VOX_PRELOADS                                                                                       \
    {                                                                                                      \
        if (PRO) {                                                                                         \
            _Pragma("unroll") for (int u = 0; u < 12; u++) {                                               \
                const int pi = pch + u * nch;                                                              \
                const float v = p.ssq_part[(size_t)min(pi, p.n_part - 1) * 16 + prow];                     \
                pv[u] = pi < p.n_part ? v : 0.f;                                                           \
            }                                                                                              \
        }                                                                                                  \
        const int n0_ = min(nbase + min(wave, NTW - 1) * 16 + li, N - 1);                                  \
        if (EPI == EPI_RESID_XF || EPI == EPI_RESID) {                                                     \
            _Pragma("unroll") for (int r = 0; r < 4; r++) pre_res[r] = p.resid[(size_t)min(4 * g + r, M - 1) * p.resid_stride + n0_]; \
        }                                                                                                  \
        if (EPI == EPI_RESID_XF) { pre_xw = p.xf_w[n0_]; if (p.xf_w2) pre_xw *= p.xf_w2[n0_]; }            \
        if (ROPE_KV) {                                                                                     \
            _Pragma("unroll") for (int r = 0; r < 4; r++) pre_pos[r] = p.pos[min(4 * g + r, M - 1)];       \
            _Pragma("unroll") for (int r = 0; r < 4; r++) pre_row[r] = p.kv_row ? p.kv_row[min(4 * g + r, M - 1)] : min(4 * g + r, M - 1); \
            if (KVP) { _Pragma("unroll") for (int r = 0; r < 4; r++) pre_kvp[r] = p.kv_pos[min(4 * g + r, M - 1)]; } \
        }                                                                                                  \
    }
    constexpr bool STRAIGHT = STEPS > 0 && TILED && XIN;
    if (!STRAIGHT) VOX_PRELOADS
    const int per = (nq + KS - 1) / KS;
    int q = TILED ? wave * per : wave;
    const int qend = TILED ? min(q + per, nq) : nq, qs = TILED ? 1 : KS;
    if (STRAIGHT) {
        constexpr int D = NTW >= 3 ? 2 : 3, DB = STEPS <= 0 ? 1 : (D < STEPS ? D : STEPS);
        uint4 wr[DB][NTW]; uint2 sr[DB][NTW]; float4 xr[DB][2][4];
#define VOX_ISSUE(B_, Q_)                                                                                  \
        { VOX_WLOAD(wr[B_], sr[B_], (Q_))                                                                  \
          _Pragma("unroll") for (int j = 0; j < 4; j++) {                                                  \
              xr[B_][0][j] = *reinterpret_cast<const float4*>(xfh + ((Q_) * 4 + j) * 64);                  \
              xr[B_][1][j] = *reinterpret_cast<const float4*>(xfl + ((Q_) * 4 + j) * 64); } }
        VOX_ISSUE(0, q)
        __builtin_amdgcn_sched_barrier(0);
        VOX_PRELOADS
        __builtin_amdgcn_sched_barrier(0);
#pragma unroll
        for (int u = 1; u < DB; u++) VOX_ISSUE(u, q + u)
#pragma unroll
// ... 641 lines not shown
}
template <int MT, int NTW>
static hipError_t skinny_mt_launch(const GemmParams& p, int epi, hipStream_t s) {
    dim3 grid((p.w.N + 16 * NTW - 1) / (16 * NTW));
    const size_t lds = (size_t)4 * MT * NTW * 64 * 4 * sizeof(float);
    if (epi != EPI_STORE && epi != EPI_RESID && epi != EPI_GELU && epi != EPI_SWIGLU) return hipErrorInvalidValue;
    gemm_form_note(GEMM_FORM_SKINNY_MT);
    if (p.xf) {
        switch (epi) {
        case EPI_STORE: q4_skinny_mt_kernel<MT, NTW, EPI_STORE, true><<<grid, dim3(256), lds, s>>>(p); break;
        case EPI_RESID: q4_skinny_mt_kernel<MT, NTW, EPI_RESID, true><<<grid, dim3(256), lds, s>>>(p); break;
        case EPI_GELU: q4_skinny_mt_kernel<MT, NTW, EPI_GELU, true><<<grid, dim3(256), lds, s>>>(p); break;
        case EPI_SWIGLU: q4_skinny_mt_kernel<MT, NTW, EPI_SWIGLU, true><<<grid, dim3(256), lds, s>>>(p); break;
        default: return hipErrorInvalidValue;
        }
        return hipGetLastError();
    }
    switch (epi) {
    case EPI_STORE: q4_skinny_mt_kernel<MT, NTW, EPI_STORE><<<grid, dim3(256), lds, s>>>(p); break;
    case EPI_RESID: q4_skinny_mt_kernel<MT, NTW, EPI_RESID><<<grid, dim3(256), lds, s>>>(p); break;
    case EPI_GELU: q4_skinny_mt_kernel<MT, NTW, EPI_GELU><<<grid, dim3(256), lds, s>>>(p); break;
    case EPI_SWIGLU: q4_skinny_mt_kernel<MT, NTW, EPI_SWIGLU><<<grid, dim3(256), lds, s>>>(p); break;
    default: return hipErrorInvalidValue;
    }
    return hipGetLastError();
}
static bool prefill_wide_plan(const Q4W& w, int M, WidePlan* pl) {
    return M > 16 && M <= 48 && w.N % 16 == 0 && q4_wide_plan(w, (M + 15) / 16, EPI_ROPE_KV, pl);
}
int q4_skinny_mt2_plan(const Q4W& w, int M) {
    if (w.fmt != WFMT_Q4_0 || !w.qt || !w.st || w.nb % 4 || w.N % 2 || M <= 16 || M > 48) return 0;
    { WidePlan pl; if (prefill_wide_plan(w, M, &pl)) return pl.kz; }
    const int tiles = (w.N + 15) / 16, nq = w.nb / 4, wg1 = (tiles + 3) / 4;
    return std::min(std::min(8, nq), std::max(1, (384 + wg1 - 1) / wg1));
}
hipError_t launch_xf_rows(const float* x, int x_stride, int M, int K, uint16_t* xf, hipStream_t s) {
    const int mt = (M + 15) / 16; const long total = (long)mt * 16 * (K >> 2);
    if (K % 128) return hipErrorInvalidValue;
    gemm_form_note(GEMM_FORM_XF_ROWS);
    xf_rows_kernel<<<dim3((unsigned)std::min<long>((total + 255) / 256, 1024)), dim3(256), 0, s>>>(x, x_stride, M, K, xf, mt);
    return hipGetLastError();
}
hipError_t launch_q4_skinny_mt2_planes(const GemmParams& p_in, int KZ, hipStream_t s) {
    GemmParams p = p_in; p.ksplit = KZ; p.out = p_in.kz_scratch;
    const int mt = (p.M + 15) / 16, n_tiles = (p.w.N + 15) / 16;
    if (!p.xf || !p.kz_scratch || (size_t)KZ * p.M * p.w.N * 4 > p.kz_scratch_bytes || KZ < 1) return hipErrorInvalidValue;
    { WidePlan pl;
      if (prefill_wide_plan(p.w, p.M, &pl) && pl.kz == KZ) {
          GemmParams q = p_in; q.wide_mt = mt; q.wide_rows = p.M; q.M = 16 * mt; q.xf_gstride = (long)2 * (p.w.nb / 4) * 256;
          return launch_q4_wide(q, EPI_ROPE_KV | 0x100, s);
      } }
    if (mt == 2 || mt == 3) gemm_form_note(GEMM_FORM_SKINNY_MT2);
    if (mt == 2) q4_skinny_mt2_kernel<2, 1><<<dim3((n_tiles + 3) / 4, KZ), dim3(256), (size_t)2 * 2 * 8 * 64 * 16, s>>>(p);
    else if (mt == 3) q4_skinny_mt2_kernel<3, 1><<<dim3((n_tiles + 3) / 4, KZ), dim3(256), (size_t)2 * 3 * 8 * 64 * 16, s>>>(p);
    else return hipErrorInvalidValue;
    return hipGetLastError();
}
__global__ __launch_bounds__(256) void splitk_finish_swiglu_xf_kernel(const float* __restrict__ planes, int KZ, int M, int N, const float* __restrict__ bias, uint16_t* __restrict__ xf) {
    const int K2 = N >> 1, k4 = K2 >> 2;
    const long total = (long)M * k4; const size_t plane = (size_t)M * N, tile_stride = (size_t)2 * (K2 >> 7) * 256 * 8;
    for (long i = (long)blockIdx.x * blockDim.x + threadIdx.x; i < total; i += (long)gridDim.x * blockDim.x) {
        const int row = (int)(i / k4), k = (int)(i % k4) * 4, n = 2 * k;
        const float4* p0 = reinterpret_cast<const float4*>(planes + (size_t)row * N + n);
        float4 a = p0[0], b = p0[1];
        if (KZ > 1) { plane_sum_add(a, p0 + (plane >> 2), plane >> 2, KZ - 1); plane_sum_add(b, p0 + (plane >> 2) + 1, plane >> 2, KZ - 1); }
        if (bias) { const float4 ba = *reinterpret_cast<const float4*>(bias + n), bb = *reinterpret_cast<const float4*>(bias + n + 4); a = a + ba; b = b + bb; }
        xf_store4(xf + (size_t)(row >> 4) * tile_stride, K2, row & 15, k, make_float4(silu_f(a.x) * a.y, silu_f(a.z) * a.w, silu_f(b.x) * b.y, silu_f(b.z) * b.w));
    }
}
__global__ __launch_bounds__(256) void splitk_finish_rope_kv_kernel(const float* __restrict__ planes, int KZ, int M, int N, float* __restrict__ q_out, int q_stride, int n_q, int n_kv, int hd,
                                                                   int pos_off, const float* __restrict__ cos_t, const float* __restrict__ sin_t, float* __restrict__ kc, float* __restrict__ vc,
                                                                   int head_stride) {
    const int n4 = N >> 2, kd = n_kv * hd;
    const long total = (long)M * n4; const size_t plane = (size_t)M * N;
    for (long i = (long)blockIdx.x * blockDim.x + threadIdx.x; i < total; i += (long)gridDim.x * blockDim.x) {
        const int m = (int)(i / n4), n = (int)(i % n4) * 4;
        const float4* p0 = reinterpret_cast<const float4*>(planes + (size_t)m * N + n);
        float4 v = p0[0];
        if (KZ > 1) plane_sum_add(v, p0 + (plane >> 2), plane >> 2, KZ - 1);
        const int pos = pos_off + m;
        if (n < n_q + kd) {
            const size_t ti = (size_t)pos * (hd >> 1) + ((n % hd) >> 1);
            const float c0 = cos_t[ti], s0 = sin_t[ti], c1 = cos_t[ti + 1], s1 = sin_t[ti + 1];
            v = make_float4(v.x * c0 - v.y * s0, v.x * s0 + v.y * c0, v.z * c1 - v.w * s1, v.z * s1 + v.w * c1);
        }
        if (n < n_q) *reinterpret_cast<float4*>(q_out + (size_t)m * q_stride + n) = v;
        else {
            const int cidx = n < n_q + kd ? n - n_q : n - n_q - kd;
            float* dst = (n < n_q + kd ? kc : vc) + (size_t)(cidx / hd) * head_stride + (size_t)pos * hd + (cidx % hd);
            *reinterpret_cast<float4*>(dst) = v;
        }
    }
}
hipError_t launch_splitk_finish_swiglu_xf(const float* planes, int KZ, int M, int N, const float* bias, uint16_t* xf, hipStream_t s) {
    if (KZ < 1 || M < 1 || M > 48 || N % 256) return hipErrorInvalidValue;
    const long total = (long)M * (N >> 3);
    splitk_finish_swiglu_xf_kernel<<<(int)std::min<long>((total + 255) / 256, 2048), 256, 0, s>>>(planes, KZ, M, N, bias, xf);
    return hipGetLastError();
}
hipError_t launch_splitk_finish_rope_kv(const float* planes, int KZ, int M, int N, float* q_out, int q_stride, int n_q, int n_kv, int hd, int pos_off,
                                        const float* cos_t, const float* sin_t, float* kc, float* vc, int head_stride, hipStream_t s) {
    if (KZ < 1 || M < 1 || N % 4 || hd % 4 || n_q % hd || N != n_q + 2 * n_kv * hd) return hipErrorInvalidValue;
    const long total = (long)M * (N >> 2);
    splitk_finish_rope_kv_kernel<<<(int)std::min<long>((total + 255) / 256, 2048), 256, 0, s>>>(planes, KZ, M, N, q_out, q_stride, n_q, n_kv, hd, pos_off, cos_t, sin_t, kc, vc, head_stride);
    return hipGetLastError();
}
hipError_t launch_splitk_finish_resid(const float* planes, int KZ, int M, int N, float* x, int x_stride, hipStream_t s) {
    const long total = (long)M * N;
    gemm_form_note(GEMM_FORM_SPLITK_FINISH);
    splitk_finish_kernel<EPI_RESID><<<(int)std::min<long>((total + 255) / 256, 2048), 256, 0, s>>>(planes, KZ, M, N, nullptr, x, x_stride, x, x_stride);
    return hipGetLastError();
}
static hipError_t launch_q4_skinny_mt(const GemmParams& p_in, int epi, hipStream_t s) {
    GemmParams p = p_in;
    const int mt = (p.M + 15) / 16, tiles = (p.w.N + 15) / 16;
    if (!p.xf && p.xf_scratch && p.xf_scratch_bytes >= (size_t)mt * p.w.K * 64 && p.w.K % 128 == 0) {
        const long total = (long)mt * 16 * (p.w.K >> 2);
        gemm_form_note(GEMM_FORM_XF_ROWS);
        xf_rows_kernel<<<dim3((unsigned)std::min<long>((total + 255) / 256, 1024)), dim3(256), 0, s>>>(p.x, p.x_stride, p.M, p.w.K, p.xf_scratch, mt);
        p.xf = reinterpret_cast<const uint4*>(p.xf_scratch);
    }
    int ntw = tiles >= 512 ? 2 : 1;
    if (p.xf && p.kz_scratch && p.w.N % 2 == 0) {
        ntw = 1;
        const int nq = p.w.nb / 4, wg1 = (tiles + 3) / 4;
        const int KZ = std::min(std::min(8, nq), std::max(1, (384 + wg1 - 1) / wg1));
        if ((size_t)KZ * p.M * p.w.N * 4 <= p.kz_scratch_bytes) {
            if (mt == 2) return skinny_mt2_launch<2, 1>(p, epi, KZ, s);
            if (mt == 3) return skinny_mt2_launch<3, 1>(p, epi, KZ, s);
        }
    }
#define VOX_MTN(M_, N_) if (mt == M_ && ntw == N_) return skinny_mt_launch<M_, N_>(p, epi, s)
    VOX_MTN(2, 1); VOX_MTN(2, 2); VOX_MTN(3, 1); VOX_MTN(3, 2);
#undef VOX_MTN
    return hipErrorInvalidValue;
}

__device__ __forceinline__ f32x4 scale_fma(float d, f32x4 t, f32x4 acc) {
    float dd = d; asm("" : "+v"(dd));
    f32x4 o;
#pragma unroll
    for (int r = 0; r < 4; r++) { float a = fmaf(dd, t[r], acc[r]); asm("" : "+v"(a)); o[r] = a; }
    return o;
}

typedef __amdgpu_buffer_rsrc_t vsrd_t;
typedef unsigned vu32x4_t __attribute__((ext_vector_type(4)));
typedef unsigned vu32x2_t __attribute__((ext_vector_type(2)));
__device__ __forceinline__ vsrd_t vmake_srd(const void* base, unsigned bytes) { return __builtin_amdgcn_make_buffer_rsrc(const_cast<void*>(base), 0, (int)bytes, 0x00020000); }
__device__ __forceinline__ float4 vbuf_f4(vsrd_t sd, unsigned voff, unsigned soff) { const vu32x4_t v = __builtin_bit_cast(vu32x4_t, __builtin_amdgcn_raw_buffer_load_b128(sd, (int)voff, (int)soff, 0)); return make_float4(__uint_as_float(v.x), __uint_as_float(v.y), __uint_as_float(v.z), __uint_as_float(v.w)); }
__device__ __forceinline__ uint4 vbuf_u4(vsrd_t sd, unsigned voff, unsigned soff) { const vu32x4_t v = __builtin_bit_cast(vu32x4_t, __builtin_amdgcn_raw_buffer_load_b128(sd, (int)voff, (int)soff, 0)); return make_uint4(v.x, v.y, v.z, v.w); }
__device__ __forceinline__ uint2 vbuf_u2(vsrd_t sd, unsigned voff, unsigned soff) { const vu32x2_t v = __builtin_bit_cast(vu32x2_t, __builtin_amdgcn_raw_buffer_load_b64(sd, (int)voff, (int)soff, 0)); return make_uint2(v.x, v.y); }

template <int WGM, int WGN, int EPI>
__global__ __launch_bounds__(256) __attribute__((amdgpu_waves_per_eu(2))) void q4_gemm_big_kernel(const GemmParams p) {
    constexpr int BM = 64 * WGM, MTB = BM / 16;
    constexpr int PAIRS = 4 * MTB, NU = PAIRS / 4;
    extern __shared__ __attribute__((aligned(16))) uint4 blds[];
    constexpr int PLANE = 4 * MTB * 64;
    const int nb = p.w.nb, N = p.w.N, M = p.M, nq = nb >> 2;
    const int tid = threadIdx.x, lane = tid & 63, wave = tid >> 6, g = lane >> 4, li = lane & 15;
    const int wm = wave / WGN, wn = wave % WGN;
    const int m0 = blockIdx.y * BM, n0 = blockIdx.x * (64 * WGN);
    const int n_tiles = (N + 15) >> 4;
    static_assert(WGM == 1, "the staging map below is written for 64-row workgroups");
    const vsrd_t xsrd = vmake_srd(p.x, (unsigned)min((size_t)0xFFFFFFF0u, ((size_t)(M - 1) * p.x_stride + (size_t)p.w.K) * 4));
    const vsrd_t qsrd = vmake_srd(p.w.qt, (unsigned)((size_t)n_tiles * nq * 1024)), ssrd = vmake_srd(p.w.st, (unsigned)((size_t)n_tiles * nq * 128));
    const unsigned xo = (unsigned)(((size_t)min(m0 + 16 * wave + li, M - 1) * p.x_stride + 4 * g) * 4);
    const unsigned qo = (unsigned)lane * 16u, so = (unsigned)li * 8u;
    const int tile0 = __builtin_amdgcn_readfirstlane((n0 >> 4) + wn * 4);
    f32x4 acc[4][4];
#pragma unroll
    for (int t = 0; t < 4; t++)
#pragma unroll
        for (int i = 0; i < 4; i++) acc[t][i] = (f32x4){0.f, 0.f, 0.f, 0.f};
    float4 xa[NU], xb[NU]; uint4 bw[4], bwn[4]; uint2 bs[4], bsn[4];
#define VOX_ALOAD(Q_)                                                                                          \
    _Pragma("unroll") for (int u = 0; u < NU; u++) {                                                           \
        xa[u] = vbuf_f4(xsrd, xo + (unsigned)(Q_) * 512u + (unsigned)u * 128u, 0);                             \
        xb[u] = vbuf_f4(xsrd, xo + (unsigned)(Q_) * 512u + (unsigned)u * 128u + 64u, 0); }
#define VOX_BLOAD(W_, S_, Q_)                                                                                  \
    _Pragma("unroll") for (int t = 0; t < 4; t++) {                                                            \
        W_[t] = vbuf_u4(qsrd, qo + (unsigned)(Q_) * 1024u, (unsigned)(tile0 + t) * (unsigned)nq * 1024u);      \
        S_[t] = vbuf_u2(ssrd, so + (unsigned)(Q_) * 128u, (unsigned)(tile0 + t) * (unsigned)nq * 128u); }
    VOX_ALOAD(0)
    VOX_BLOAD(bw, bs, 0)
    const bf16x8 m136 = as_bf16x8(make_uint4(0xC308C308u, 0xC308C308u, 0xC308C308u, 0xC308C308u));
    __shared__ __attribute__((aligned(16))) float s_bcs[2][4][MTB][4][4];
#define VOX_STAGE(BUF_)                                                                                        \
    _Pragma("unroll") for (int u = 0; u < NU; u++) {      \
        uint4 hi, lo;                                                                                          \
        split_pair(xa[u].x, xa[u].z, hi.x, lo.x); split_pair(xb[u].x, xb[u].z, hi.y, lo.y);                    \
        split_pair(xa[u].y, xa[u].w, hi.z, lo.z); split_pair(xb[u].y, xb[u].w, hi.w, lo.w);                    \
        f32x4 c_ = __builtin_amdgcn_mfma_f32_16x16x32_bf16(as_bf16x8(hi), m136, (f32x4){0.f, 0.f, 0.f, 0.f}, 0, 0, 0); \
        c_ = __builtin_amdgcn_mfma_f32_16x16x32_bf16(as_bf16x8(lo), m136, c_, 0, 0, 0);                        \
        if (li == 0) *reinterpret_cast<f32x4*>(&s_bcs[(BUF_) == blds ? 0 : 1][u][wave][g][0]) = c_;             \
        (BUF_)[(wave + 4 * u) * 64 + lane] = hi; (BUF_)[PLANE + (wave + 4 * u) * 64 + lane] = lo; }
    VOX_STAGE(blds)
    __syncthreads();
    { const int q1 = min(1, nq - 1); VOX_ALOAD(q1) VOX_BLOAD(bwn, bsn, q1) }
    for (int q = 0; q < nq; q++) {
        uint4* const cur = blds + (q & 1) * (2 * PLANE);
        uint4* const nxt = blds + ((q + 1) & 1) * (2 * PLANE);
        if (q + 1 < nq) { VOX_STAGE(nxt) }
        if (q > 0) { const int q1 = min(q + 1, nq - 1); VOX_BLOAD(bwn, bsn, q1) }
        { const int q2 = min(q + 2, nq - 1); VOX_ALOAD(q2) }
        f32x4 tp[4] = {}; float dp[4] = {0.f, 0.f, 0.f, 0.f};
#pragma unroll
        for (int jj = 0; jj < 4; jj++) {
            bf16x8 bf[4]; float d[4];
#pragma unroll
            for (int t = 0; t < 4; t++) {
                const uint32_t w_ = jj == 0 ? bw[t].x : jj == 1 ? bw[t].y : jj == 2 ? bw[t].z : bw[t].w;
                bf[t] = as_bf16x8(q4_dword_to_bf16x8_biased(w_));
                const uint32_t pr = (jj & 2) ? bs[t].y : bs[t].x;
                d[t] = f16_bits_to_f32((uint16_t)((jj & 1) ? (pr >> 16) : (pr & 0xFFFFu)));
            }
#pragma unroll
            for (int i = 0; i < 4; i++) {
                const bf16x8 ah = as_bf16x8(cur[(jj * MTB + wm * 4 + i) * 64 + lane]);
                const bf16x8 al = as_bf16x8(cur[PLANE + (jj * MTB + wm * 4 + i) * 64 + lane]);
                const f32x4 cs = *reinterpret_cast<const f32x4*>(&s_bcs[q & 1][jj][wm * 4 + i][g][0]);
                f32x4 tn[4];
#pragma unroll
                for (int t = 0; t < 4; t++) tn[t] = __builtin_amdgcn_mfma_f32_16x16x32_bf16(ah, bf[t], cs, 0, 0, 0);
#pragma unroll
                for (int t = 0; t < 4; t++) tn[t] = __builtin_amdgcn_mfma_f32_16x16x32_bf16(al, bf[t], tn[t], 0, 0, 0);
                if (jj > 0 || i > 0) {
                    const int ip = i > 0 ? i - 1 : 3;
#pragma unroll
                    for (int t = 0; t < 4; t++) acc[t][ip] = scale_fma(dp[t], tp[t], acc[t][ip]);
                }
#pragma unroll
                for (int t = 0; t < 4; t++) { tp[t] = tn[t]; dp[t] = d[t]; }
            }
        }
#pragma unroll
        for (int t = 0; t < 4; t++) acc[t][3] = scale_fma(dp[t], tp[t], acc[t][3]);
#pragma unroll
        for (int t = 0; t < 4; t++) { bw[t] = bwn[t]; bs[t] = bsn[t]; }
        __syncthreads();
    }
#undef VOX_STAGE
#undef VOX_ALOAD
#undef VOX_BLOAD
#pragma unroll
    for (int t = 0; t < 4; t++) {
        const int n = n0 + (wn * 4 + t) * 16 + li; const bool nok = n < N;
        const float bias = (p.bias && nok) ? p.bias[n] : 0.f;
#pragma unroll
        for (int i = 0; i < 4; i++)
#pragma unroll
            for (int r = 0; r < 4; r++) {
                const int m = m0 + (wm * 4 + i) * 16 + 4 * g + r;
                float v = acc[t][i][r] + bias;
                if (EPI == EPI_SWIGLU) {
                    const float other = dpp_mov<0xB1>(v);
                    if (m < M && nok && !(n & 1)) p.out[(size_t)m * p.out_stride + (n >> 1)] = silu_f(v) * other;
                } else if (EPI == EPI_ROPE_ROWS) {
                    const float other = dpp_mov<0xB1>(v);
                    if (m < M && nok) {
                        if (n < p.n_q) {
                            const int pos = p.pos ? p.pos[m] : (p.rope_seq_rows > 0 ? m % p.rope_seq_rows : m);
                            const size_t ti = (size_t)pos * (p.hd >> 1) + ((n & (p.hd - 1)) >> 1);
                            const float c = p.rope_cos[ti], sn = p.rope_sin[ti];
                            const float os = __fmul_rn(other, sn);
                            v = (n & 1) ? __fmaf_rn(v, c, os) : __fmaf_rn(v, c, -os);
                        }
                        p.out[(size_t)m * p.out_stride + n] = v;
                    }
                } else if (m < M && nok) {
                    if (EPI == EPI_RESID) v = v + p.resid[(size_t)m * p.resid_stride + n];
                    if (EPI == EPI_GELU) v = gelu_f(v);
                    p.out[(size_t)m * p.out_stride + n] = v;
                }
            }
    }
}
template <int WGM, int WGN>
static hipError_t gemm_big_launch(const GemmParams& p, int epi, hipStream_t s) {
    dim3 grid((p.w.N + 64 * WGN - 1) / (64 * WGN), (p.M + 64 * WGM - 1) / (64 * WGM));
    const size_t lds = (size_t)2 * 2 * 4 * (4 * WGM) * 64 * sizeof(uint4);
#define VOX_E(E_) case E_: { auto kern = q4_gemm_big_kernel<WGM, WGN, E_>; static DevOnce done;          \
        hipError_t e = ensure_dyn_lds(kern, lds, &done); if (e != hipSuccess) return e;                       \
        gemm_form_note(E_ == EPI_ROPE_ROWS ? GEMM_FORM_BIG_ROPE : GEMM_FORM_BIG); kern<<<grid, dim3(256), lds, s>>>(p); break; }
    switch (epi) { VOX_E(EPI_STORE) VOX_E(EPI_RESID) VOX_E(EPI_GELU) VOX_E(EPI_SWIGLU) VOX_E(EPI_ROPE_ROWS) default: return hipErrorInvalidValue; }
#undef VOX_E
    return hipGetLastError();
}

template <int NTW, int EPI, bool KTAIL = false>
__global__ __launch_bounds__(256) __attribute__((amdgpu_waves_per_eu(2))) void dense2_gemm_kernel(const GemmParams p) {
    extern __shared__ __attribute__((aligned(16))) uint4 dlds[];
    constexpr int PLANE = 4 * 4 * 64;
    const int N = p.w.N, K = p.w.K, M = p.M, nq = KTAIL ? (K + 127) >> 7 : K >> 7;
    const int tid = threadIdx.x, lane = tid & 63, wave = tid >> 6, g = lane >> 4, li = lane & 15;
    const int m0 = blockIdx.y * 64, n0 = blockIdx.x * (64 * NTW);
    const float* xrow[4];
#pragma unroll
    for (int u = 0; u < 4; u++) {
        const int pair = wave + 4 * u, j = pair >> 2, i = pair & 3;
        xrow[u] = p.x + (size_t)min(m0 + 16 * i + li, M - 1) * p.x_stride + 32 * j + 8 * g;
    }
    const uint4* wh[NTW]; const uint4* wl[NTW];
#pragma unroll
    for (int t = 0; t < NTW; t++) {
        const size_t row = (size_t)min(n0 + (wave * NTW + t) * 16 + li, N - 1);
        wh[t] = p.w.qs + row * (K >> 3) + g; wl[t] = reinterpret_cast<const uint4*>(p.w.sc) + row * (K >> 3) + g;
    }
    f32x4 acc[NTW][4];
#pragma unroll
    for (int t = 0; t < NTW; t++)
#pragma unroll
        for (int i = 0; i < 4; i++) acc[t][i] = (f32x4){0.f, 0.f, 0.f, 0.f};
    float4 xa[4], xb[4]; uint4 bh[NTW][4], bl[NTW][4], bhn[NTW][4], bln[NTW][4];
#define VOX_ALOAD(Q_)                                                                                          \
    _Pragma("unroll") for (int u = 0; u < 4; u++) {                \
        const int ko = 128 * (Q_) - ((KTAIL && 128 * (Q_) + 32 * u >= K) ? 32 * u : 0);                       \
        xa[u] = *reinterpret_cast<const float4*>(xrow[u] + ko);                                                \
        xb[u] = *reinterpret_cast<const float4*>(xrow[u] + ko + 4); }
#define VOX_BLOAD(H_, L_, Q_)                                                                                  \
    _Pragma("unroll") for (int t = 0; t < NTW; t++)                                                            \
        _Pragma("unroll") for (int j = 0; j < 4; j++) { const int jo = (KTAIL && 128 * (Q_) + 32 * j >= K) ? 0 : j * 4;   \
            H_[t][j] = wh[t][(Q_) * 16 + jo]; L_[t][j] = wl[t][(Q_) * 16 + jo]; }
    VOX_ALOAD(0)
    VOX_BLOAD(bh, bl, 0)
    for (int q = 0; q < nq; q++) {
        __syncthreads();
#pragma unroll
        for (int u = 0; u < 4; u++) {
            uint4 hi, lo; split_bf16x8(xa[u], xb[u], hi, lo);
            if (KTAIL && 128 * q + 32 * u >= K) hi = lo = make_uint4(0u, 0u, 0u, 0u);
            dlds[(wave + 4 * u) * 64 + lane] = hi; dlds[PLANE + (wave + 4 * u) * 64 + lane] = lo;
        }
        __syncthreads();
        { const int q1 = min(q + 1, nq - 1); VOX_ALOAD(q1) VOX_BLOAD(bhn, bln, q1) }
        __builtin_amdgcn_sched_barrier(0);
#pragma unroll
        for (int j = 0; j < 4; j++)
#pragma unroll
            for (int i = 0; i < 4; i++) {
                const bf16x8 ah = as_bf16x8(dlds[(j * 4 + i) * 64 + lane]);
                const bf16x8 al = as_bf16x8(dlds[PLANE + (j * 4 + i) * 64 + lane]);
#pragma unroll
                for (int t = 0; t < NTW; t++) {
                    acc[t][i] = __builtin_amdgcn_mfma_f32_16x16x32_bf16(ah, as_bf16x8(bh[t][j]), acc[t][i], 0, 0, 0);
                    acc[t][i] = __builtin_amdgcn_mfma_f32_16x16x32_bf16(al, as_bf16x8(bh[t][j]), acc[t][i], 0, 0, 0);
                    acc[t][i] = __builtin_amdgcn_mfma_f32_16x16x32_bf16(ah, as_bf16x8(bl[t][j]), acc[t][i], 0, 0, 0);
                }
            }
#pragma unroll
        for (int t = 0; t < NTW; t++)
#pragma unroll
            for (int j = 0; j < 4; j++) { bh[t][j] = bhn[t][j]; bl[t][j] = bln[t][j]; }
    }
#undef VOX_ALOAD
#undef VOX_BLOAD
#pragma unroll
    for (int t = 0; t < NTW; t++) {
        const int n = n0 + (wave * NTW + t) * 16 + li; const bool nok = n < N;
        const float bias = (p.bias && nok) ? p.bias[n] : 0.f;
#pragma unroll
        for (int i = 0; i < 4; i++)
#pragma unroll
            for (int r = 0; r < 4; r++) {
                const int m = m0 + i * 16 + 4 * g + r;
                float v = acc[t][i][r] + bias;
                if (EPI == EPI_SWIGLU) {
                    const float other = dpp_mov<0xB1>(v);
                    if (m < M && nok && !(n & 1)) p.out[(size_t)m * p.out_stride + (n >> 1)] = silu_f(v) * other;
                } else {
                    if (EPI == EPI_GELU) v = gelu_f(v);
                    if (EPI == EPI_RESID && m < M && nok) v = v + p.resid[(size_t)m * p.resid_stride + n];
                    if (m < M && nok) p.out[(size_t)m * p.out_stride + n] = v;
                }
            }
    }
}
hipError_t launch_dense2_gemm(const GemmParams& p, int epi, hipStream_t s) {
    if (p.w.fmt != WFMT_BF16X2 || p.w.K % 32 || (p.x_stride % 4) || p.M <= 0) return hipErrorInvalidValue;
    if (p.w.K % 128) {
        dim3 tgrid((p.w.N + 63) / 64, (p.M + 63) / 64);
        switch (epi) {
#define VOX_D2T(E_) case E_: gemm_form_note(GEMM_FORM_DENSE2); dense2_gemm_kernel<1, E_, true><<<tgrid, dim3(256), (size_t)2 * 4 * 4 * 64 * sizeof(uint4), s>>>(p); break;
        VOX_D2T(EPI_STORE) VOX_D2T(EPI_GELU) VOX_D2T(EPI_RESID) VOX_D2T(EPI_SWIGLU) default: return hipErrorInvalidValue;
#undef VOX_D2T
        }
        return hipGetLastError();
    }
    const long wg2 = (long)((p.w.N + 127) / 128) * ((p.M + 63) / 64);
    const size_t lds = (size_t)2 * 4 * 4 * 64 * sizeof(uint4);
    const bool wide = wg2 >= 400;
    dim3 grid(wide ? (p.w.N + 127) / 128 : (p.w.N + 63) / 64, (p.M + 63) / 64);
#define VOX_D2(E_) case E_: gemm_form_note(GEMM_FORM_DENSE2); if (wide) dense2_gemm_kernel<2, E_><<<grid, dim3(256), lds, s>>>(p); else dense2_gemm_kernel<1, E_><<<grid, dim3(256), lds, s>>>(p); break;
    switch (epi) { VOX_D2(EPI_STORE) VOX_D2(EPI_GELU) VOX_D2(EPI_RESID) VOX_D2(EPI_SWIGLU) default: return hipErrorInvalidValue; }
#undef VOX_D2
    return hipGetLastError();
}
__global__ void transpose_kernel(const float* __restrict__ in, int R, int C, float* __restrict__ out) {
    __shared__ float tile[32][33];
    const int c0 = blockIdx.x * 32, r0 = blockIdx.y * 32, tx = threadIdx.x & 31, ty = threadIdx.x >> 5;
    for (int k = ty; k < 32; k += 8) { const int r = r0 + k, c = c0 + tx; tile[k][tx] = (r < R && c < C) ? in[(size_t)r * C + c] : 0.f; }
    __syncthreads();
    for (int k = ty; k < 32; k += 8) { const int c = c0 + k, r = r0 + tx; if (c < C && r < R) out[(size_t)c * R + r] = tile[tx][k]; }
}
hipError_t launch_transpose(const float* in, int R, int C, float* out, hipStream_t s) {
    transpose_kernel<<<dim3((C + 31) / 32, (R + 31) / 32), dim3(256), 0, s>>>(in, R, C, out);
    return hipGetLastError();
}

template <int NTW, int TILED>
static hipError_t skinny_launch_n(const GemmParams& p, int epi, int ks, hipStream_t s) {
    if (epi == EPI_ROPE_KV && p.kv_pos) epi = EPI_ROPE_KV_PAGED;
    dim3 grid((p.w.N + 16 * NTW - 1) / (16 * NTW));
    const size_t lds = (size_t)ks * NTW * 64 * 4 * sizeof(float);
    if (p.xf) {
        if (!TILED) return hipErrorInvalidValue;
        const bool pro = p.ssq_part != nullptr;
        if (pro && (p.n_part < 1 || p.n_part > 12 * (64 * ks / 16))) return hipErrorInvalidValue;
        const int nq = p.w.nb / 4, per = nq % ks == 0 ? nq / ks : 0;
        if (per) {
#define VOX_ST(N_, E_, P_, S_) if (NTW == N_ && epi == E_ && (int)pro == P_ && per == S_) { \
            if (E_ == EPI_RESID_XF && (!p.xf_out || !p.xf_w || !p.ssq_out)) return hipErrorInvalidValue; \
            q4_skinny_kernel<N_, E_, 1, 1, P_, S_><<<grid, dim3(64 * ks), lds, s>>>(p); return hipGetLastError(); }
            VOX_ST(2, EPI_ROPE_KV, 1, 3) VOX_ST(2, EPI_ROPE_KV_PAGED, 1, 3) VOX_ST(2, EPI_SWIGLU_XF, 1, 6) VOX_ST(1, EPI_SWIGLU_XF, 1, 6) VOX_ST(1, EPI_RESID_XF, 0, 4) VOX_ST(4, EPI_SWIGLU_XF, 1, 6) VOX_ST(1, EPI_RESID_XF, 0, 9) VOX_ST(4, EPI_STORE, 1, 6)
#undef VOX_ST
        }
        if (epi == EPI_RESID_XF) {
            if (NTW != 1 || pro || !p.xf_out || !p.xf_w || !p.ssq_out) return hipErrorInvalidValue;
            q4_skinny_kernel<1, EPI_RESID_XF, 1, 1, 0><<<grid, dim3(64 * ks), lds, s>>>(p);
        } else if (pro) {
            switch (epi) {
            case EPI_STORE: q4_skinny_kernel<NTW, EPI_STORE, 1, 1, 1><<<grid, dim3(64 * ks), lds, s>>>(p); break;
            case EPI_ROPE_KV: q4_skinny_kernel<NTW, EPI_ROPE_KV, 1, 1, 1><<<grid, dim3(64 * ks), lds, s>>>(p); break;
            case EPI_ROPE_KV_PAGED: q4_skinny_kernel<NTW, EPI_ROPE_KV_PAGED, 1, 1, 1><<<grid, dim3(64 * ks), lds, s>>>(p); break;
            case EPI_SWIGLU_XF: q4_skinny_kernel<NTW, EPI_SWIGLU_XF, 1, 1, 1><<<grid, dim3(64 * ks), lds, s>>>(p); break;
            default: return hipErrorInvalidValue;
            }
        } else {
            switch (epi) {
            case EPI_STORE: q4_skinny_kernel<NTW, EPI_STORE, 1, 1, 0><<<grid, dim3(64 * ks), lds, s>>>(p); break;
            case EPI_RESID: q4_skinny_kernel<NTW, EPI_RESID, 1, 1, 0><<<grid, dim3(64 * ks), lds, s>>>(p); break;
            case EPI_SWIGLU_XF: q4_skinny_kernel<NTW, EPI_SWIGLU_XF, 1, 1, 0><<<grid, dim3(64 * ks), lds, s>>>(p); break;
            default: return hipErrorInvalidValue;
            }
        }
        return hipGetLastError();
    }
    switch (epi) {
    case EPI_STORE: q4_skinny_kernel<NTW, EPI_STORE, TILED, 0, 0><<<grid, dim3(64 * ks), lds, s>>>(p); break;
    case EPI_RESID: q4_skinny_kernel<NTW, EPI_RESID, TILED, 0, 0><<<grid, dim3(64 * ks), lds, s>>>(p); break;
    case EPI_GELU: q4_skinny_kernel<NTW, EPI_GELU, TILED, 0, 0><<<grid, dim3(64 * ks), lds, s>>>(p); break;
    case EPI_SWIGLU: q4_skinny_kernel<NTW, EPI_SWIGLU, TILED, 0, 0><<<grid, dim3(64 * ks), lds, s>>>(p); break;
    default: return hipErrorInvalidValue;
    }
    return hipGetLastError();
}
int q4_skinny_resid_xf_parts(int N) { return (N + 15) / 16; }
static hipError_t launch_q4_skinny(const GemmParams& p_in, int epi, hipStream_t s) {
    GemmParams p = p_in; p.tl_slot = tl_take_slot(2, epi, p.w.N, p.w.K);
    const int nq = p.w.nb / 4, tiles = (p.w.N + 15) / 16;
    int ntw = tiles >= 4 * 192 ? 4 : (tiles >= 2 * 192 ? 2 : 1);
    int ks = nq >= 4 ? 4 : (nq >= 2 ? 2 : 1);
    if (tiles / ntw < 256 && nq >= 16) ks = 8;
    if (epi == EPI_RESID_XF) ntw = 1;
    const bool tiled = p.w.qt && p.w.st;
    hipError_t e;
    if (ntw == 4) e = tiled ? skinny_launch_n<4, 1>(p, epi, ks, s) : skinny_launch_n<4, 0>(p, epi, ks, s);
    else if (ntw == 2) e = tiled ? skinny_launch_n<2, 1>(p, epi, ks, s) : skinny_launch_n<2, 0>(p, epi, ks, s);
    else e = tiled ? skinny_launch_n<1, 1>(p, epi, ks, s) : skinny_launch_n<1, 0>(p, epi, ks, s);
    if (e == hipSuccess) gemm_form_note(GEMM_FORM_SKINNY);
    return e;
}

template <int MT, int NT, int FMT, int TB = 0>
static hipError_t gemm_launch_mn(const GemmParams& p, int epi, hipStream_t s) {
    if (p.ksplit > 1 && (epi != EPI_STORE || p.ksplit > p.w.nb / 4)) return hipErrorInvalidValue;
    dim3 grid((p.w.N + 64 * NT - 1) / (64 * NT), (p.M + 16 * MT - 1) / (16 * MT), p.ksplit > 1 ? p.ksplit : 1);
    const size_t lds = (size_t)2 * 2 * 4 * MT * 64 * sizeof(uint4);
#define VOX_E(E_) case E_: { auto kern = q4_gemm_kernel<MT, NT, E_, FMT, TB>; static DevOnce done;      \
        hipError_t e = ensure_dyn_lds(kern, lds, &done); if (e != hipSuccess) return e;                       \
        gemm_form_note(TB ? (NT == 2 ? GEMM_FORM_TILE_22_TB : GEMM_FORM_TILE_21_TB) : MT == 1 ? (NT == 2 ? GEMM_FORM_TILE_12 : GEMM_FORM_TILE_11) : (NT == 2 ? GEMM_FORM_TILE_22 : GEMM_FORM_TILE_21)); \
        kern<<<grid, dim3(256), lds, s>>>(p); break; }
    switch (epi) { VOX_E(EPI_STORE) VOX_E(EPI_RESID) VOX_E(EPI_GELU) VOX_E(EPI_SWIGLU) default: return hipErrorInvalidValue; }
#undef VOX_E
    return hipGetLastError();
}
template <int FMT>
static hipError_t gemm_launch_f(const GemmParams& p, int epi, hipStream_t s) {
    if (p.w.nb % 4) {
        dim3 grid((p.w.N + 63) / 64, (p.M + 63) / 64);
        if (epi != EPI_STORE && epi != EPI_RESID && epi != EPI_GELU && epi != EPI_SWIGLU) return hipErrorInvalidValue;
        gemm_form_note(GEMM_FORM_K32);
        switch (epi) {
        case EPI_STORE: q4_gemm_k32_kernel<EPI_STORE, FMT><<<grid, dim3(256), 0, s>>>(p); break;
        case EPI_RESID: q4_gemm_k32_kernel<EPI_RESID, FMT><<<grid, dim3(256), 0, s>>>(p); break;
        case EPI_GELU: q4_gemm_k32_kernel<EPI_GELU, FMT><<<grid, dim3(256), 0, s>>>(p); break;
        case EPI_SWIGLU: q4_gemm_k32_kernel<EPI_SWIGLU, FMT><<<grid, dim3(256), 0, s>>>(p); break;
        default: return hipErrorInvalidValue;
        }
        return hipGetLastError();
    }
    const int mt = p.M <= 48 ? 1 : 2;
    int nt = 2;
    auto wgs = [&](int mt_, int nt_) { return (long)((p.w.N + 64 * nt_ - 1) / (64 * nt_)) * ((p.M + 16 * mt_ - 1) / (16 * mt_)); };
    if (wgs(mt, 2) < 256) nt = 1;
    if (FMT == WFMT_Q4_0 && p.w.qt && p.w.st && mt == 2) {
        if (wgs(2, 2) >= 128) nt = 2;
        return nt == 2 ? gemm_launch_mn<2, 2, WFMT_Q4_0, 1>(p, epi, s) : gemm_launch_mn<2, 1, WFMT_Q4_0, 1>(p, epi, s);
    }
#define VOX_MN(M_, N_) if (mt == M_ && nt == N_) return gemm_launch_mn<M_, N_, FMT>(p, epi, s)
    VOX_MN(1, 1); VOX_MN(1, 2); VOX_MN(2, 1); VOX_MN(2, 2);
#undef VOX_MN
    return hipErrorInvalidValue;
}
hipError_t launch_rope(float* buf, int M, int stride, int n_rot, int hd, int pos_off, const float* cos_t, const float* sin_t, hipStream_t s, int seq_rows, const int* row_pos);
static hipError_t launch_q4_gemm_epi(const GemmParams& p, int epi, hipStream_t s, bool* fused_rope);
hipError_t launch_q4_gemm(const GemmParams& p, int epi, hipStream_t s, bool* fused_rope) {
    if (fused_rope) *fused_rope = false;
    if (epi != EPI_ROPE_ROWS) return launch_q4_gemm_epi(p, epi, s, nullptr);
    if (!p.rope_cos || !p.rope_sin || p.hd <= 0 || p.n_q <= 0 || p.n_q > p.w.N || p.n_q % 2) return hipErrorInvalidValue;
    bool fused = false;
    hipError_t e = launch_q4_gemm_epi(p, EPI_ROPE_ROWS, s, &fused);
    if (fused_rope) *fused_rope = fused;
    if (e != hipSuccess || fused) return e;
    return launch_rope(p.out, p.M, p.out_stride, p.n_q, p.hd, 0, p.rope_cos, p.rope_sin, s, p.rope_seq_rows, p.pos);
}
static hipError_t launch_q4_gemm_epi(const GemmParams& p, int epi_in, hipStream_t s, bool* fused_rope) {
    int epi = epi_in == EPI_ROPE_ROWS ? EPI_STORE : epi_in;
    if (p.w.K % 32 || p.M <= 0) return hipErrorInvalidValue;
    if (p.kv_pos && !(p.xf && p.M <= 16)) return hipErrorInvalidValue;
    if (p.ksplit > 1 && (p.M <= 48 || p.xf || p.w.nb % 4 || p.w.fmt == WFMT_F32)) return hipErrorInvalidValue;
    if (p.w.fmt == WFMT_F32) {
        if (p.xf) return hipErrorInvalidValue;
        GemmParams v = p; v.w.fmt = WFMT_BF16X2; v.w.qt = nullptr; v.w.st = nullptr;
        return launch_dense2_gemm(v, epi, s);
    }
    if (p.xf && p.M > 16) return (p.M <= 48 && p.w.fmt == WFMT_Q4_0 && p.w.nb % 4 == 0 && p.w.qt && p.w.st && (epi == EPI_STORE || epi == EPI_RESID || epi == EPI_GELU || epi == EPI_SWIGLU))
                                     ? launch_q4_skinny_mt(p, epi, s) : hipErrorInvalidValue;
    if (p.xf) return (p.M <= 16 && p.w.fmt == WFMT_Q4_0 && p.w.nb % 4 == 0 && p.w.qt) ? launch_q4_skinny(p, epi, s) : hipErrorInvalidValue;
    if (p.M <= 16 && p.w.fmt == WFMT_Q4_0 && p.w.nb % 4 == 0 && !env_int("VOX_NO_SKINNY")) return launch_q4_skinny(p, epi, s);
    if (p.M > 16 && p.M <= 48 && p.w.fmt == WFMT_Q4_0 && p.w.qt && p.w.st && p.w.nb % 4 == 0 && (p.x_stride % 4) == 0 && (epi == EPI_STORE || epi == EPI_RESID || epi == EPI_GELU || epi == EPI_SWIGLU) &&
        !env_int("VOX_NO_SKINNY_MT")) {
        return launch_q4_skinny_mt(p, epi, s);
    }
    if (p.w.fmt == WFMT_Q4_0 && p.w.qt && p.w.st && p.w.nb % 4 == 0 && (p.x_stride % 4) == 0) {
        const int big = env_int("VOX_GEMM_BIG");
        const long wg14 = (long)((p.w.N + 255) / 256) * ((p.M + 63) / 64);
        const int big_min = 200;
        const bool fits32 = ((size_t)(p.M - 1) * p.x_stride + (size_t)p.w.K) * 4 < 0xFFFFFFF0ull && (size_t)((p.w.N + 15) / 16) * (p.w.nb / 4) * 1024 < 0xFFFFFFF0ull;
        if (p.ksplit <= 1 && fits32 && p.w.N % 256 == 0 && (big == 1 || (big == 0 && wg14 >= big_min))) {
            if (epi_in == EPI_ROPE_ROWS && wg14 >= 1024 && (p.hd & (p.hd - 1)) == 0 && !knob_str("VOX_NO_ROPE_FUSE")) { if (fused_rope) *fused_rope = true; return gemm_big_launch<1, 4>(p, EPI_ROPE_ROWS, s); }
            return gemm_big_launch<1, 4>(p, epi, s);
        }
    }
    return p.w.fmt == WFMT_BF16 ? gemm_launch_f<WFMT_BF16>(p, epi, s) : gemm_launch_f<WFMT_Q4_0>(p, epi, s);
}

__global__ __launch_bounds__(256) void rms_norm_kernel(const float* __restrict__ x, int x_stride, int rows, int dim,
                                                       const float* __restrict__ gamma, const float* __restrict__ mul,
                                                       float eps, float* __restrict__ out, int out_stride) {
    const int row = min(blockIdx.x * 4 + (threadIdx.x >> 6), rows - 1), lane = threadIdx.x & 63;
    const float4* xr = reinterpret_cast<const float4*>(x + (size_t)row * x_stride);
    const int n4 = dim >> 2;
    float4 v[16];
    float ss = 0.f;
#pragma unroll
    for (int i = 0; i < 16; i++) {
        const int c = lane + 64 * i;
        v[i] = xr[min(c, n4 - 1)];
        if (c < n4) ss += (v[i].x * v[i].x + v[i].y * v[i].y) + (v[i].z * v[i].z + v[i].w * v[i].w);
    }
    for (int c = lane + 1024; c < n4; c += 64) { const float4 t = xr[c]; ss += (t.x * t.x + t.y * t.y) + (t.z * t.z + t.w * t.w); }
    ss = wave_sum(ss);
    const float rms = sqrtf(ss / (float)dim + eps);
    float4* o = reinterpret_cast<float4*>(out + (size_t)row * out_stride);
    const float4* g4 = reinterpret_cast<const float4*>(gamma);
    const float4* m4 = reinterpret_cast<const float4*>(mul);
#define VOX_RMS_OUT(T_, C_)                                                                                     \
    { float4 t = (T_); const float4 gm = g4[C_];                                                                \
      t.x = (t.x / rms) * gm.x; t.y = (t.y / rms) * gm.y; t.z = (t.z / rms) * gm.z; t.w = (t.w / rms) * gm.w;   \
      if (mul) { const float4 mm = m4[C_]; t.x *= mm.x; t.y *= mm.y; t.z *= mm.z; t.w *= mm.w; }               \
      o[C_] = t; }
#pragma unroll
    for (int i = 0; i < 16; i++) {
        const int c = lane + 64 * i;
        if (c < n4) VOX_RMS_OUT(v[i], c)
    }
    for (int c = lane + 1024; c < n4; c += 64) VOX_RMS_OUT(xr[c], c)
#undef VOX_RMS_OUT
}
__global__ __launch_bounds__(256) void rms_norm_row_kernel(const float* __restrict__ x, int x_stride, int dim, const float* __restrict__ gamma,
                                                           const float* __restrict__ mul, float eps, float* __restrict__ out, int out_stride,
                                                           uint16_t* __restrict__ xf, const float* __restrict__ planes = nullptr, size_t plane_stride = 0, int kz = 0,
                                                           float* __restrict__ x_rw = nullptr) {
    __shared__ float red[4];
    const int row = blockIdx.x, tid = threadIdx.x, n4 = dim >> 2;
    const float4* xr = reinterpret_cast<const float4*>(x + (size_t)row * x_stride);
    float4 v[10]; float ss = 0.f;
#pragma unroll
    for (int i = 0; i < 10; i++) {
        const int c = tid + 256 * i;
        v[i] = xr[min(c, n4 - 1)];
        if (planes && c < n4) {
            plane_sum_add(v[i], reinterpret_cast<const float4*>(planes + (size_t)row * dim) + c, plane_stride >> 2, kz);
            reinterpret_cast<float4*>(x_rw + (size_t)row * x_stride)[c] = v[i];
        }
        if (c < n4) ss += (v[i].x * v[i].x + v[i].y * v[i].y) + (v[i].z * v[i].z + v[i].w * v[i].w);
    }
    ss = wave_sum(ss);
    if ((tid & 63) == 0) red[tid >> 6] = ss;
    __syncthreads();
    const float rms = sqrtf(((red[0] + red[1]) + (red[2] + red[3])) / (float)dim + eps);
    float4* o = reinterpret_cast<float4*>(out + (size_t)row * out_stride);
    const float4* g4 = reinterpret_cast<const float4*>(gamma);
    const float4* m4 = reinterpret_cast<const float4*>(mul);
#pragma unroll
    for (int i = 0; i < 10; i++) {
        const int c = tid + 256 * i;
        if (c < n4) {
            float4 t = v[i]; const float4 gm = g4[c];
            t.x = (t.x / rms) * gm.x; t.y = (t.y / rms) * gm.y; t.z = (t.z / rms) * gm.z; t.w = (t.w / rms) * gm.w;
            if (mul) { const float4 mm = m4[c]; t.x *= mm.x; t.y *= mm.y; t.z *= mm.z; t.w *= mm.w; }
            if (xf) xf_store4(xf + (size_t)(row >> 4) * ((size_t)2 * (dim >> 7) * 256 * 8), dim, row & 15, 4 * c, t); else o[c] = t;
        }
    }
}
__global__ __launch_bounds__(256) VOX_NO_PK_F32 void rms_norm_sumk_kernel(float* __restrict__ x, int x_stride, int rows, int dim, const float* __restrict__ part, size_t part_stride, int ks,
                                                            const float* __restrict__ gamma, float eps, float* __restrict__ out, int out_stride) {
    const int row = blockIdx.x * 4 + (threadIdx.x >> 6), lane = threadIdx.x & 63;
    if (row >= rows) return;
    float4* xr = reinterpret_cast<float4*>(x + (size_t)row * x_stride);
    const int n4 = dim >> 2;
    float4 v[16];
    float ss = 0.f;
#pragma unroll
    for (int i = 0; i < 16; i++) {
        const int c = lane + 64 * i;
        if (c < n4) {
            float4 a = xr[c];
            plane_sum_add(a, reinterpret_cast<const float4*>(part + (size_t)row * dim) + c, part_stride >> 2, ks);
            v[i] = a; xr[c] = a;
            ss += (a.x * a.x + a.y * a.y) + (a.z * a.z + a.w * a.w);
        } else v[i] = make_float4(0.f, 0.f, 0.f, 0.f);
    }
    ss = wave_sum(ss);
    const float rms = sqrtf(ss / (float)dim + eps);
    float4* o = reinterpret_cast<float4*>(out + (size_t)row * out_stride);
    const float4* g4 = reinterpret_cast<const float4*>(gamma);
#pragma unroll
    for (int i = 0; i < 16; i++) {
        const int c = lane + 64 * i;
        if (c < n4) { const float4 g = g4[c]; o[c] = make_float4((v[i].x / rms) * g.x, (v[i].y / rms) * g.y, (v[i].z / rms) * g.z, (v[i].w / rms) * g.w); }
    }
}
hipError_t launch_rms_norm_sumk(float* x, int x_stride, int rows, int dim, const float* part, size_t part_stride, int ksplit, const float* gamma, float eps, float* out, int out_stride, hipStream_t s) {
    if (dim % 4 || dim > 4096 || rows <= 0 || ksplit < 1) return hipErrorInvalidValue;
    rms_norm_sumk_kernel<<<dim3((rows + 3) / 4), dim3(256), 0, s>>>(x, x_stride, rows, dim, part, part_stride, ksplit, gamma, eps, out, out_stride);
    return hipGetLastError();
}
hipError_t launch_rms_norm_xf_sumk(float* x, int x_stride, int rows, int dim, const float* planes, int kz, const float* gamma, const float* mul, float eps,
                                   uint16_t* xf, hipStream_t s) {
    if (rows > 48 || dim > 10240 || dim % 128 || kz < 1 || !planes) return hipErrorInvalidValue;
    rms_norm_row_kernel<<<dim3(rows), dim3(256), 0, s>>>(x, x_stride, dim, gamma, mul, eps, nullptr, 0, xf, planes, (size_t)rows * dim, kz, x);
    return hipGetLastError();
}
hipError_t launch_rms_norm_xf(const float* x, int x_stride, int rows, int dim, const float* gamma, const float* mul, float eps,
                              uint16_t* xf, hipStream_t s) {
    if (rows > 48 || dim > 10240 || dim % 128) return hipErrorInvalidValue;
    rms_norm_row_kernel<<<dim3(rows), dim3(256), 0, s>>>(x, x_stride, dim, gamma, mul, eps, nullptr, 0, xf);
    return hipGetLastError();
}
hipError_t launch_rms_norm(const float* x, int x_stride, int rows, int dim, const float* gamma, const float* mul, float eps,
                           float* out, int out_stride, hipStream_t s) {
    if (rows <= 64 && dim <= 10240 && dim >= 1024)
        rms_norm_row_kernel<<<dim3(rows), dim3(256), 0, s>>>(x, x_stride, dim, gamma, mul, eps, out, out_stride, nullptr);
    else
        rms_norm_kernel<<<dim3((rows + 3) / 4), dim3(256), 0, s>>>(x, x_stride, rows, dim, gamma, mul, eps, out, out_stride);
    return hipGetLastError();
}

__global__ VOX_NO_PK_F32 void rope_kernel(float* __restrict__ buf, int M, int stride, int n_rot, int hd, int pos_off,
                            const float* __restrict__ cos_t, const float* __restrict__ sin_t, int seq_rows, const int* __restrict__ row_pos) {
    const int half_cols = n_rot >> 1;
    const long total = (long)M * half_cols;
    for (long i = (long)blockIdx.x * blockDim.x + threadIdx.x; i < total; i += (long)gridDim.x * blockDim.x) {
        const int m = (int)(i / half_cols), pc = (int)(i % half_cols);
        const int col = pc * 2, j = (col % hd) >> 1;
        const size_t ti = (size_t)(pos_off + (row_pos ? row_pos[m] : seq_rows > 0 ? m % seq_rows : m)) * (hd >> 1) + j;
        const float c = cos_t[ti], sn = sin_t[ti];
        float* p = buf + (size_t)m * stride + col;
        const float xr = p[0], xi = p[1];
        p[0] = xr * c - xi * sn; p[1] = xr * sn + xi * c;
    }
}
hipError_t launch_rope(float* buf, int M, int stride, int n_rot, int hd, int pos_off, const float* cos_t, const float* sin_t,
                       hipStream_t s, int seq_rows, const int* row_pos) {
    const long total = (long)M * (n_rot / 2);
    int blocks = (int)((total + 255) / 256); if (blocks > 2048) blocks = 2048; if (blocks < 1) blocks = 1;
    rope_kernel<<<dim3(blocks), dim3(256), 0, s>>>(buf, M, stride, n_rot, hd, pos_off, cos_t, sin_t, seq_rows, row_pos);
    return hipGetLastError();
}

__global__ void kv_store_kernel(const float* __restrict__ buf, int M, int stride, int k_col, int n_kv, int hd, int pos_off,
                                float* __restrict__ kc, float* __restrict__ vc, int head_stride, int seq_rows, long kv_seq_stride) {
    const int w = n_kv * hd;
    const long total = (long)M * w;
    for (long i = (long)blockIdx.x * blockDim.x + threadIdx.x; i < total; i += (long)gridDim.x * blockDim.x) {
        const int m = (int)(i / w), c = (int)(i % w), h = c / hd, d = c % hd;
        const int sq = seq_rows > 0 ? m / seq_rows : 0, mm = seq_rows > 0 ? m % seq_rows : m;
        const size_t dst = (size_t)sq * kv_seq_stride + (size_t)h * head_stride + (size_t)(pos_off + mm) * hd + d;
        kc[dst] = buf[(size_t)m * stride + k_col + c];
        vc[dst] = buf[(size_t)m * stride + k_col + w + c];
    }
}
hipError_t launch_kv_store(const float* buf, int M, int stride, int k_col, int n_kv, int hd, int pos_off, float* kc, float* vc,
                           int head_stride, hipStream_t s, int seq_rows, long kv_seq_stride) {
    const long total = (long)M * n_kv * hd;
    int blocks = (int)((total + 255) / 256); if (blocks > 2048) blocks = 2048; if (blocks < 1) blocks = 1;
    kv_store_kernel<<<dim3(blocks), dim3(256), 0, s>>>(buf, M, stride, k_col, n_kv, hd, pos_off, kc, vc, head_stride, seq_rows, kv_seq_stride);
    return hipGetLastError();
}

template <int HD>
__global__ __launch_bounds__(256) void attn_prefill_kernel(const AttnParams p) {
    constexpr int DP = HD / 4;
    extern __shared__ __attribute__((aligned(16))) float smem[];
    float* Ks = smem;
    float* Vs = smem + 64 * HD;
    const int tid = threadIdx.x, lane = tid & 63, wave = tid >> 6;
    const int h = blockIdx.y, kvh = h / (p.n_heads / p.n_kv_heads);
    const int m0 = blockIdx.x * 64;
    const int qi = lane & 15, part = lane >> 4;
    const int m = m0 + wave * 16 + qi;
    const bool q_ok = m < p.M;
    const int pos = p.offset + (q_ok ? m : (p.M - 1));
    const float scale = 1.0f / sqrtf((float)HD);

    float qv[DP], o[DP];
    {
        const float* qp = p.q + (size_t)(q_ok ? m : 0) * p.q_stride + h * HD + part * DP;
#pragma unroll
        for (int e = 0; e < DP; e += 4) {
            const float4 v = *reinterpret_cast<const float4*>(qp + e);
            qv[e] = v.x; qv[e + 1] = v.y; qv[e + 2] = v.z; qv[e + 3] = v.w;
        }
#pragma unroll
        for (int e = 0; e < DP; e++) o[e] = 0.f;
    }
    float mx = -INFINITY, l = 0.f;

    const int last_m = min(m0 + 63, p.M - 1);
    int j_lo = 0;
    if (p.window >= 0) j_lo = max(0, p.offset + m0 - p.window);
    const int j_hi = min(p.kv_len - 1, p.offset + last_m);
    const float* kbase = p.k + (size_t)kvh * p.kv_head_stride;
    const float* vbase = p.v + (size_t)kvh * p.kv_head_stride;

    for (int j0 = (j_lo / 64) * 64; j0 <= j_hi; j0 += 64) {
        __syncthreads();
        for (int i = tid; i < 64 * (HD / 4); i += 256) {
            const int jj = i / (HD / 4), d4 = i % (HD / 4), j = j0 + jj;
            const int jc = min(j, p.kv_len - 1);
            float4 kk = *reinterpret_cast<const float4*>(kbase + (size_t)jc * p.kv_row_stride + d4 * 4);
            float4 vv = *reinterpret_cast<const float4*>(vbase + (size_t)jc * p.kv_row_stride + d4 * 4);
            reinterpret_cast<float4*>(Ks)[i] = kk;
            reinterpret_cast<float4*>(Vs)[i] = vv;
        }
        __syncthreads();
        for (int jj = 0; jj < 64; jj += 4) {
            float sc[4];
#pragma unroll
            for (int kk = 0; kk < 4; kk++) {
                const float* kr = Ks + (jj + kk) * HD + part * DP;
                float s = 0.f;
#pragma unroll
                for (int e = 0; e < DP; e += 4) {
                    const float4 kv = *reinterpret_cast<const float4*>(kr + e);
                    s = fmaf(qv[e], kv.x, s); s = fmaf(qv[e + 1], kv.y, s); s = fmaf(qv[e + 2], kv.z, s); s = fmaf(qv[e + 3], kv.w, s);
                }
                s += __shfl_xor(s, 16, 64); s += __shfl_xor(s, 32, 64);
                const int j = j0 + jj + kk;
                bool vis = (j < p.kv_len) && (j <= pos);
                if (p.window >= 0) vis = vis && (pos - j <= p.window);
                sc[kk] = vis ? s * scale : -INFINITY;
            }
            const float mnew = fmaxf(fmaxf(fmaxf(sc[0], sc[1]), fmaxf(sc[2], sc[3])), mx);
            if (mnew > -INFINITY) {
                const float alpha = expf(mx - mnew);
                float pr[4];
#pragma unroll
                for (int kk = 0; kk < 4; kk++) pr[kk] = expf(sc[kk] - mnew);
                l = l * alpha + ((pr[0] + pr[1]) + (pr[2] + pr[3]));
#pragma unroll
                for (int e = 0; e < DP; e++) o[e] *= alpha;
#pragma unroll
                for (int kk = 0; kk < 4; kk++) {
                    const float* vr = Vs + (jj + kk) * HD + part * DP;
#pragma unroll
                    for (int e = 0; e < DP; e += 4) {
                        const float4 vv = *reinterpret_cast<const float4*>(vr + e);
                        o[e] = fmaf(pr[kk], vv.x, o[e]); o[e + 1] = fmaf(pr[kk], vv.y, o[e + 1]);
                        o[e + 2] = fmaf(pr[kk], vv.z, o[e + 2]); o[e + 3] = fmaf(pr[kk], vv.w, o[e + 3]);
                    }
                }
                mx = mnew;
            }
        }
    }
    if (q_ok) {
        float* op = p.out + (size_t)m * p.out_stride + h * HD + part * DP;
// ... 13 lines not shown
    uint16_t* Vl = Vh + HD * VROW;
    const int tid = threadIdx.x, lane = tid & 63, wave = tid >> 6, c = lane & 15, g = lane >> 4;
    int bx = blockIdx.x, h = blockIdx.y, sq = blockIdx.z;
    {
        const int nblk = gridDim.x, pairs = gridDim.y * gridDim.z;
        if (nblk > 1 && pairs % 8 == 0) {
            const int lin = (blockIdx.z * gridDim.y + blockIdx.y) * nblk + blockIdx.x, xcd = lin & 7, slot = lin >> 3;
            const int pair = xcd * (pairs >> 3) + slot / nblk;
            bx = slot % nblk; h = pair % (int)gridDim.y; sq = pair / (int)gridDim.y;
        }
    }
    const int kvh = h / (p.n_heads / p.n_kv_heads);
    const int M = p.seq_len ? p.seq_len[sq] : p.M, kv_len = p.seq_len ? p.offset + M : p.kv_len;
    const int m0 = ((int)gridDim.x - 1 - bx) * 64;
    if (m0 >= M) return;
    const int m = m0 + wave * 16 + c;
    const int mq = min(m, M - 1);
    const int pos = p.offset + mq;
    const int wave_pos_hi = p.offset + min(m0 + wave * 16 + 15, M - 1);
    const float scale = 1.0f / sqrtf((float)HD);

    bf16x8 qh[KS], ql[KS];
    {
        const float* qp = p.q + (p.seq_row_off ? (size_t)p.seq_row_off[sq] * p.q_stride : (size_t)sq * p.q_seq_stride) + (size_t)mq * p.q_stride + h * HD + 8 * g;
#pragma unroll
        for (int ks = 0; ks < KS; ks++) {
            const float4 a = *reinterpret_cast<const float4*>(qp + ks * 32), b = *reinterpret_cast<const float4*>(qp + ks * 32 + 4);
            uint4 hi, lo; split_bf16x8(a, b, hi, lo); qh[ks] = as_bf16x8(hi); ql[ks] = as_bf16x8(lo);
        }
    }
    f32x4 o[DT];
#pragma unroll
    for (int dt = 0; dt < DT; dt++) o[dt] = (f32x4){0.f, 0.f, 0.f, 0.f};
    float mx = -INFINITY, lsum = 0.f;

    const int last_m = min(m0 + 63, M - 1);
    int j_lo = 0;
    if (p.window >= 0) j_lo = max(0, p.offset + m0 - p.window);
    const int j_hi = min(kv_len - 1, p.offset + last_m);
    const size_t kvso = p.seq_row_off ? (size_t)p.seq_row_off[sq] * p.kv_row_stride : (size_t)sq * p.kv_seq_stride;
    const float* kbase = p.k + kvso + (size_t)kvh * p.kv_head_stride;
    const float* vbase = p.v + kvso + (size_t)kvh * p.kv_head_stride;
    const int n_pfx = PFX ? p.prefix_len : 0;
    const float* pkbase = PFX ? p.prefix_k + (size_t)kvh * p.prefix_head_stride : nullptr;
    const float* pvbase = PFX ? p.prefix_v + (size_t)kvh * p.prefix_head_stride : nullptr;
#define VOX_ATT_ROW(BASE_, PBASE_, J_) \
    ((PFX && (J_) < n_pfx) ? (PBASE_) + (size_t)(J_) * p.prefix_row_stride : (BASE_) + (size_t)((J_) - n_pfx) * p.kv_row_stride)

    constexpr int NK = (64 * (HD / 4)) / 256, NV = (32 * (HD / 4)) / 256;
    float4 kreg[NK], vra[NV], vrb[NV];
#define VOX_ATT_LOAD(J0_)                                                                                           \
    _Pragma("unroll") for (int u = 0; u < NK; u++) {                                                                \
        const int i = tid + 256 * u, key = i / (HD / 4), d4 = i % (HD / 4);                                         \
        const int jc = min((J0_) + key, kv_len - 1);      \
        kreg[u] = *reinterpret_cast<const float4*>(VOX_ATT_ROW(kbase, pkbase, jc) + d4 * 4);                        \
    }                                                                                                               \
    _Pragma("unroll") for (int u = 0; u < NV; u++) {                                                                \
        const int i = tid + 256 * u, kp = i / (HD / 4), d4 = i % (HD / 4);                                          \
        const int ja = min((J0_) + 2 * kp, kv_len - 1), jb = min((J0_) + 2 * kp + 1, kv_len - 1);               \
        vra[u] = *reinterpret_cast<const float4*>(VOX_ATT_ROW(vbase, pvbase, ja) + d4 * 4);                         \
        vrb[u] = *reinterpret_cast<const float4*>(VOX_ATT_ROW(vbase, pvbase, jb) + d4 * 4);                         \
    }
    const int j_first = (j_lo / 64) * 64, j_last = (j_hi / 64) * 64;
    VOX_ATT_LOAD(j_first)
    for (int j0 = j_first; j0 <= j_hi; j0 += 64) {
        __syncthreads();
#pragma unroll
        for (int u = 0; u < NK; u++) {
            const int i = tid + 256 * u, key = i / (HD / 4), d4 = i % (HD / 4);
            uint2 hi, lo; split_pair(kreg[u].x, kreg[u].y, hi.x, lo.x); split_pair(kreg[u].z, kreg[u].w, hi.y, lo.y);
            *reinterpret_cast<uint2*>(Kh + key * KROW + d4 * 4) = hi;
            *reinterpret_cast<uint2*>(Kl + key * KROW + d4 * 4) = lo;
        }
#pragma unroll
        for (int u = 0; u < NV; u++) {
            const int i = tid + 256 * u, kp = i / (HD / 4), d4 = i % (HD / 4);
            const float4 va = vra[u], vb = vrb[u];
            uint32_t hi, lo;
            split_pair(va.x, vb.x, hi, lo); *reinterpret_cast<uint32_t*>(Vh + (d4 * 4 + 0) * VROW + 2 * kp) = hi; *reinterpret_cast<uint32_t*>(Vl + (d4 * 4 + 0) * VROW + 2 * kp) = lo;
            split_pair(va.y, vb.y, hi, lo); *reinterpret_cast<uint32_t*>(Vh + (d4 * 4 + 1) * VROW + 2 * kp) = hi; *reinterpret_cast<uint32_t*>(Vl + (d4 * 4 + 1) * VROW + 2 * kp) = lo;
            split_pair(va.z, vb.z, hi, lo); *reinterpret_cast<uint32_t*>(Vh + (d4 * 4 + 2) * VROW + 2 * kp) = hi; *reinterpret_cast<uint32_t*>(Vl + (d4 * 4 + 2) * VROW + 2 * kp) = lo;
            split_pair(va.w, vb.w, hi, lo); *reinterpret_cast<uint32_t*>(Vh + (d4 * 4 + 3) * VROW + 2 * kp) = hi; *reinterpret_cast<uint32_t*>(Vl + (d4 * 4 + 3) * VROW + 2 * kp) = lo;
        }
        __syncthreads();
        { const int jn = min(j0 + 64, j_last); VOX_ATT_LOAD(jn) }
        __builtin_amdgcn_sched_barrier(0);
        if (j0 > wave_pos_hi) continue;

        f32x4 sc[4];
#pragma unroll
        for (int kt = 0; kt < 4; kt++) {
            sc[kt] = (f32x4){0.f, 0.f, 0.f, 0.f};
            if (j0 + kt * 16 <= wave_pos_hi) {
#pragma unroll
                for (int ks = 0; ks < KS; ks++) {
                    const bf16x8 ah = as_bf16x8(*reinterpret_cast<const uint4*>(Kh + (kt * 16 + c) * KROW + ks * 32 + 8 * g));
                    const bf16x8 al = as_bf16x8(*reinterpret_cast<const uint4*>(Kl + (kt * 16 + c) * KROW + ks * 32 + 8 * g));
                    sc[kt] = __builtin_amdgcn_mfma_f32_16x16x32_bf16(ah, qh[ks], sc[kt], 0, 0, 0);
                    sc[kt] = __builtin_amdgcn_mfma_f32_16x16x32_bf16(ah, ql[ks], sc[kt], 0, 0, 0);
                    sc[kt] = __builtin_amdgcn_mfma_f32_16x16x32_bf16(al, qh[ks], sc[kt], 0, 0, 0);
                }
            }
        }
        float mt = -INFINITY;
#pragma unroll
        for (int kt = 0; kt < 4; kt++)
#pragma unroll
            for (int r = 0; r < 4; r++) {
                const int j = j0 + kt * 16 + 4 * g + r;
                bool vis = (j < kv_len) && (j <= pos);
                if (p.window >= 0) vis = vis && (pos - j <= p.window);
                const float v = vis ? sc[kt][r] * scale : -INFINITY;
                sc[kt][r] = v; mt = fmaxf(mt, v);
            }
        mt = fmaxf(mt, __shfl_xor(mt, 16, 64)); mt = fmaxf(mt, __shfl_xor(mt, 32, 64));
        const float mnew = fmaxf(mx, mt);
        const float msafe = (mnew == -INFINITY) ? 0.f : mnew;
        const float alpha = __expf(mx - msafe);
        float ps = 0.f;
#pragma unroll
        for (int kt = 0; kt < 4; kt++)
#pragma unroll
            for (int r = 0; r < 4; r++) { const float e = __expf(sc[kt][r] - msafe); sc[kt][r] = e; ps += e; }
        lsum = lsum * alpha + ps; mx = mnew;
#pragma unroll
        for (int dt = 0; dt < DT; dt++) { o[dt][0] *= alpha; o[dt][1] *= alpha; o[dt][2] *= alpha; o[dt][3] *= alpha; }
#pragma unroll
        for (int kk = 0; kk < 2; kk++) {
            if (j0 + kk * 32 <= wave_pos_hi) {
                uint4 ph, pl;
                split_pair(sc[2 * kk][0], sc[2 * kk][1], ph.x, pl.x); split_pair(sc[2 * kk][2], sc[2 * kk][3], ph.y, pl.y);
                split_pair(sc[2 * kk + 1][0], sc[2 * kk + 1][1], ph.z, pl.z); split_pair(sc[2 * kk + 1][2], sc[2 * kk + 1][3], ph.w, pl.w);
                const bf16x8 bh = as_bf16x8(ph), bl = as_bf16x8(pl);
#pragma unroll
                for (int dt = 0; dt < DT; dt++) {
                    const uint16_t* vh = Vh + (dt * 16 + c) * VROW + kk * 32 + 4 * g;
                    const uint16_t* vl = Vl + (dt * 16 + c) * VROW + kk * 32 + 4 * g;
                    const uint2 h0 = *reinterpret_cast<const uint2*>(vh), h1 = *reinterpret_cast<const uint2*>(vh + 16);
                    const uint2 l0 = *reinterpret_cast<const uint2*>(vl), l1 = *reinterpret_cast<const uint2*>(vl + 16);
                    const bf16x8 ah = as_bf16x8(make_uint4(h0.x, h0.y, h1.x, h1.y)), al = as_bf16x8(make_uint4(l0.x, l0.y, l1.x, l1.y));
                    o[dt] = __builtin_amdgcn_mfma_f32_16x16x32_bf16(ah, bh, o[dt], 0, 0, 0);
                    o[dt] = __builtin_amdgcn_mfma_f32_16x16x32_bf16(ah, bl, o[dt], 0, 0, 0);
                    o[dt] = __builtin_amdgcn_mfma_f32_16x16x32_bf16(al, bh, o[dt], 0, 0, 0);
                }
            }
        }
    }
#undef VOX_ATT_LOAD
#undef VOX_ATT_ROW
    lsum += __shfl_xor(lsum, 16, 64); lsum += __shfl_xor(lsum, 32, 64);
    if (m < M) {
        const float inv = 1.0f / lsum;
        float* op = p.out + (p.seq_row_off ? (size_t)p.seq_row_off[sq] * p.out_stride : (size_t)sq * p.out_seq_stride) + (size_t)m * p.out_stride + h * HD + 4 * g;
#pragma unroll
        for (int dt = 0; dt < DT; dt++)
            *reinterpret_cast<float4*>(op + dt * 16) = make_float4(o[dt][0] * inv, o[dt][1] * inv, o[dt][2] * inv, o[dt][3] * inv);
    }
}
template <int HD, bool PFX>
static hipError_t attn_prefill_mfma_launch(const AttnParams& p, hipStream_t s, int n_seq) {
    constexpr size_t lds = ((size_t)2 * 64 * (HD + 8) + (size_t)2 * HD * 72) * sizeof(uint16_t);
    auto kern = attn_prefill_mfma_kernel<HD, PFX>;
    static DevOnce attr_done;
    hipError_t e = ensure_dyn_lds(kern, lds, &attr_done);
    if (e != hipSuccess) return e;
    kern<<<dim3((p.M + 63) / 64, p.n_heads, n_seq), dim3(256), lds, s>>>(p);
    attn_form_note(ATTN_FORM_PREFILL_MFMA);
    return hipGetLastError();
}
template <int HD>
__global__ __launch_bounds__(256) void attn_prefill_small_kernel(const AttnParams p) {
    constexpr int KROW = HD + 4, MAXR = 48;
    extern __shared__ __attribute__((aligned(16))) float sms[];
    float* Ks = sms; float* Vs = Ks + MAXR * KROW; float* Qs = Vs + MAXR * HD; float* Ps = Qs + 4 * HD;
    const int tid = threadIdx.x, lane = tid & 63, wave = tid >> 6;
    const int h = blockIdx.x, sq = blockIdx.y, kvh = h / (p.n_heads / p.n_kv_heads);
    const int M = p.seq_len ? p.seq_len[sq] : p.M;
    const int r = 4 * (int)blockIdx.z + wave;
    const int n_keys = min(M, 4 * (int)blockIdx.z + 4);
    if (4 * (int)blockIdx.z >= M) {
        if (p.out_xf_tiles && lane < 32) xf_store4(p.out_xf_tiles + (size_t)(r >> 4) * p.out_xf_tile_stride, p.n_heads * HD, r & 15, h * HD + 4 * lane, make_float4(0.f, 0.f, 0.f, 0.f));
        return;
    }
    const size_t kvso = (size_t)sq * p.kv_seq_stride;
    const float* kbase = p.k + kvso + (size_t)kvh * p.kv_head_stride; const float* vbase = p.v + kvso + (size_t)kvh * p.kv_head_stride;
    for (int i = tid; i < n_keys * (HD / 4); i += 256) {
        const int j = i / (HD / 4), d4 = i % (HD / 4);
        *reinterpret_cast<float4*>(Ks + j * KROW + 4 * d4) = *reinterpret_cast<const float4*>(kbase + (size_t)j * p.kv_row_stride + 4 * d4);
        *reinterpret_cast<float4*>(Vs + j * HD + 4 * d4) = *reinterpret_cast<const float4*>(vbase + (size_t)j * p.kv_row_stride + 4 * d4);
    }
    float* qs = Qs + wave * HD; float* ps = Ps + wave * 64;
    if (r < M) { const float* qp = p.q + (size_t)sq * p.q_seq_stride + (size_t)r * p.q_stride + h * HD; for (int d = lane; d < HD; d += 64) qs[d] = qp[d]; }
    __syncthreads();
    const float scale = 1.0f / sqrtf((float)HD);
    float4 o = make_float4(0.f, 0.f, 0.f, 0.f);
    if (r < M) {
        const float* kr = Ks + min(lane, n_keys - 1) * KROW;
        float s0 = 0.f, s1 = 0.f, s2 = 0.f, s3 = 0.f;
#pragma unroll 8
        for (int d = 0; d < HD; d += 4) {
            const float4 kv = *reinterpret_cast<const float4*>(kr + d), qv = *reinterpret_cast<const float4*>(qs + d);
            s0 = fmaf(qv.x, kv.x, s0); s1 = fmaf(qv.y, kv.y, s1); s2 = fmaf(qv.z, kv.z, s2); s3 = fmaf(qv.w, kv.w, s3);
        }
        const bool vis = lane <= r && (p.window < 0 || r - lane <= p.window);
        const float sc = vis ? ((s0 + s1) + (s2 + s3)) * scale : -INFINITY;
        const float mx = wave_max(sc);
        const float e = vis ? expf(sc - mx) : 0.f;
        const float sum = wave_sum(e);
        ps[lane] = e / sum;
        __builtin_amdgcn_wave_barrier();
        const int c = lane & 31, half = lane >> 5;
        for (int j = half; j <= r; j += 2) {
            const float pj = ps[j]; const float4 vv = *reinterpret_cast<const float4*>(Vs + j * HD + 4 * c);
            o.x = fmaf(pj, vv.x, o.x); o.y = fmaf(pj, vv.y, o.y); o.z = fmaf(pj, vv.z, o.z); o.w = fmaf(pj, vv.w, o.w);
        }
        o.x += __shfl_xor(o.x, 32, 64); o.y += __shfl_xor(o.y, 32, 64); o.z += __shfl_xor(o.z, 32, 64); o.w += __shfl_xor(o.w, 32, 64);
    }
    if (lane < 32) {
        const int col = h * HD + 4 * lane;
        if (p.out_xf_tiles) xf_store4(p.out_xf_tiles + (size_t)(r >> 4) * p.out_xf_tile_stride, p.n_heads * HD, r & 15, col, o);
        else if (r < M) *reinterpret_cast<float4*>(p.out + (size_t)sq * p.out_seq_stride + (size_t)r * p.out_stride + col) = o;
    }
}
bool attn_prefill_small_ok(const AttnParams& p, int hd, int n_seq) {
    return hd == 128 && p.M >= 1 && p.M <= 48 && p.offset == 0 && p.kv_len == p.M && !p.seq_row_off && (p.window < 0 || p.window >= p.M) && (p.q_stride % 4) == 0 && (p.kv_row_stride % 4) == 0 &&
           n_seq == 1  &&
           !env_int("VOX_ATTN_F32");
}
static hipError_t attn_prefill_small_launch(const AttnParams& p, hipStream_t s, int n_seq) {
    constexpr int HD = 128;
    const size_t lds = (size_t)(48 * (HD + 4) + 48 * HD + 4 * HD + 4 * 64) * sizeof(float);
    auto kern = attn_prefill_small_kernel<HD>; static DevOnce done;
    hipError_t e = ensure_dyn_lds(kern, lds, &done); if (e != hipSuccess) return e;
    const int rows = p.out_xf_tiles ? ((p.M + 15) / 16) * 16 : p.M;
    kern<<<dim3(p.n_heads, n_seq, (rows + 3) / 4), dim3(256), lds, s>>>(p);
    attn_form_note(ATTN_FORM_PREFILL_SMALL);
    return hipGetLastError();
}
bool attn_prefill_prefix_ok(const AttnParams& p, int hd, int n_seq) {
    return (hd == 64 || hd == 128) && n_seq == 1 && !p.seq_len && !p.seq_row_off && !p.out_xf_tiles && p.prefix_k && p.prefix_v && p.prefix_len > 0 && p.offset == p.prefix_len &&
           p.M >= 1 && p.kv_len == p.prefix_len + p.M && (p.q_stride % 4) == 0 && (p.kv_row_stride % 4) == 0 && (p.prefix_row_stride % 4) == 0 && (p.prefix_head_stride % 4) == 0 &&
           !env_int("VOX_ATTN_F32");
}
hipError_t launch_attn_prefill(const AttnParams& p, int hd, hipStream_t s, int n_seq) {
    if (attn_prefill_small_ok(p, hd, n_seq)) return attn_prefill_small_launch(p, s, n_seq);
    if (p.out_xf_tiles) return hipErrorInvalidValue;
    const int f32_only = env_int("VOX_ATTN_F32");
    if (p.prefix_len > 0) {
        if (!attn_prefill_prefix_ok(p, hd, n_seq)) return hipErrorInvalidValue;
        return hd == 64 ? attn_prefill_mfma_launch<64, true>(p, s, 1) : attn_prefill_mfma_launch<128, true>(p, s, 1);
    }
    if (!f32_only && (p.q_stride % 4) == 0 && (p.kv_row_stride % 4) == 0) {
        if (hd == 64) return attn_prefill_mfma_launch<64, false>(p, s, n_seq);
        if (hd == 128) return attn_prefill_mfma_launch<128, false>(p, s, n_seq);
    }
    if (n_seq != 1 || p.seq_len) return hipErrorInvalidValue;
    dim3 grid((p.M + 63) / 64, p.n_heads);
    const size_t lds = (size_t)2 * 64 * hd * sizeof(float);
    if (hd == 64) {
        attn_prefill_kernel<64><<<grid, dim3(256), lds, s>>>(p);
    } else if (hd == 128) {
        auto kern = attn_prefill_kernel<128>;
        static DevOnce attr_done;
        hipError_t e = ensure_dyn_lds(kern, lds, &attr_done);
        if (e != hipSuccess) return e;
        kern<<<grid, dim3(256), lds, s>>>(p);
    } else return hipErrorInvalidValue;
    attn_form_note(ATTN_FORM_PREFILL_F32);
    return hipGetLastError();
}

template <bool NT>
__device__ __forceinline__ float4 ldf4(const float* p) {
    if (NT) { const u32x4_t v = __builtin_nontemporal_load(reinterpret_cast<const u32x4_t*>(p)); return make_float4(__uint_as_float(v.x), __uint_as_float(v.y), __uint_as_float(v.z), __uint_as_float(v.w)); }
    return *reinterpret_cast<const float4*>(p);
}
template <int HD, bool NT, bool LATE_V, bool SPEC, class Hook, class Rows>
__device__ __forceinline__ float4 attn_decode_core(const float* __restrict__ qh, const Rows rows,
                                                   int pos_in, int window, float* __restrict__ sc, float* __restrict__ red, float4* __restrict__ osum, int tl_slot, int tlw,
                                                   int spec_rows, Hook after_issue) {
    static_assert(HD == 128 || HD == 64, "head_dim");
    constexpr int PER = HD / 8;
    const int tid = threadIdx.x, lane = tid & 63, wave = tid >> 6;
    const float scale = 1.0f / sqrtf((float)HD);
    const int ks = tid >> 3, part = tid & 7;
    (void)tl_slot; (void)tlw;
    float qv[PER];
#pragma unroll
    for (int e = 0; e < PER; e += 4) {
        const float4 v = ldf4<NT>(qh + part * PER + e);
        qv[e] = v.x; qv[e + 1] = v.y; qv[e + 2] = v.z; qv[e + 3] = v.w;
    }
    constexpr int NPRE = LATE_V ? 4 : 5, COLS = HD / 4, GROUPS = 256 / COLS;
    static_assert(4 * GROUPS == 32 || HD != 128, "prefetch tiling assumes 32 keys per P.V iteration for HD = 128");
    const int grp = tid / COLS, col = tid % COLS;
    float4 kpre[NPRE][PER / 4], vpre[NPRE][4];
#define VOX_KPRE(ROW_)                                                                                        \
    _Pragma("unroll") for (int u = 0; u < NPRE; u++) {                                                        \
        const int jc = (ROW_);                                                                                \
        const float* kr = rows.k(jc) + part * PER;                                                            \
        _Pragma("unroll") for (int e = 0; e < PER / 4; e++) kpre[u][e] = ldf4<NT>(kr + 4 * e);                \
    }
#define VOX_VPRE_AT(ROW_)                                                                                     \
    _Pragma("unroll") for (int u = 0; u < NPRE; u++)                                                          \
        _Pragma("unroll") for (int w = 0; w < 4; w++) {                                                       \
            const int iv = u * 4 * GROUPS + grp + w * GROUPS;                                                 \
            vpre[u][w] = ldf4<NT>(rows.v(ROW_) + col * 4);                                                    \
        }
#define VOX_VPRE VOX_VPRE_AT(j_lo + min(iv, n - 1))
    static_assert(!SPEC || !LATE_V, "speculative rows: K and V are both requested up front");
    if (SPEC) {
        VOX_KPRE(min(32 * u + ks, spec_rows - 1))
        VOX_VPRE_AT(min(iv, spec_rows - 1))
        __builtin_amdgcn_sched_barrier(0);
    }
    const int pos = SPEC ? __builtin_amdgcn_readfirstlane(pos_in) : pos_in;
    const int len = pos + 1;
    const int j_lo = window >= 0 ? max(0, pos - window) : 0;
    const int n = len - j_lo;
    if (SPEC) {
        if (j_lo != 0) {
            VOX_KPRE(j_lo + min(32 * u + ks, n - 1))
            VOX_VPRE
        }
    } else {
        VOX_KPRE(j_lo + min(32 * u + ks, n - 1))
        if (!LATE_V) { VOX_VPRE }
    }
    __builtin_amdgcn_sched_barrier(0);
    after_issue();
    __builtin_amdgcn_sched_barrier(0);
#undef VOX_KPRE
#pragma unroll
    for (int u = 0; u < NPRE; u++) {
        float s = 0.f;
#pragma unroll
        for (int e = 0; e < PER / 4; e++) {
            const float4 kv = kpre[u][e];
            s = fmaf(qv[4 * e], kv.x, s); s = fmaf(qv[4 * e + 1], kv.y, s); s = fmaf(qv[4 * e + 2], kv.z, s); s = fmaf(qv[4 * e + 3], kv.w, s);
        }
        s = group8_sum(s);
        const int i = 32 * u + ks;
        if (part == 0 && i < n) sc[i] = s * scale;
    }
    if (LATE_V) { VOX_VPRE }
#undef VOX_VPRE
#undef VOX_VPRE_AT
    for (int i0 = 32 * NPRE; i0 < n; i0 += 64) {
        float s2[2];
#pragma unroll
        for (int u = 0; u < 2; u++) {
            const int i = i0 + 32 * u + ks, jc = j_lo + min(i, n - 1);
            const float* kr = rows.k(jc) + part * PER;
            float s = 0.f;
#pragma unroll
            for (int e = 0; e < PER; e += 4) {
                const float4 kv = ldf4<NT>(kr + e);
                s = fmaf(qv[e], kv.x, s); s = fmaf(qv[e + 1], kv.y, s); s = fmaf(qv[e + 2], kv.z, s); s = fmaf(qv[e + 3], kv.w, s);
            }
            s2[u] = s;
        }
#pragma unroll
        for (int u = 0; u < 2; u++) {
            const float s = group8_sum(s2[u]);
            const int i = i0 + 32 * u + ks;
            if (part == 0 && i < n) sc[i] = s * scale;
        }
    }
    __syncthreads();
    VOX_TL(tl_slot, tlw, 1);
    float mx = -INFINITY;
    for (int i = tid; i < n; i += 256) mx = fmaxf(mx, sc[i]);
    mx = wave_max(mx);
    if (lane == 0) red[wave] = mx;
    __syncthreads();
    mx = fmaxf(fmaxf(red[0], red[1]), fmaxf(red[2], red[3]));
    float sum = 0.f;
    for (int i = tid; i < n; i += 256) { const float e = expf(sc[i] - mx); sc[i] = e; sum += e; }
    sum = wave_sum(sum);
    if (lane == 0) red[4 + wave] = sum;
    __syncthreads();
    VOX_TL(tl_slot, tlw, 2);
    sum = (red[4] + red[5]) + (red[6] + red[7]);
    float4 o = make_float4(0.f, 0.f, 0.f, 0.f);
    if (4 * GROUPS == 32) {
#pragma unroll
        for (int u = 0; u < NPRE; u++)
#pragma unroll
            for (int w = 0; w < 4; w++) {
                const int i = u * 32 + grp + w * GROUPS;
                const float pr = i < n ? sc[min(i, n - 1)] : 0.f;
                float4 vv = vpre[u][w];
                if (SPEC && i >= n) vv = make_float4(0.f, 0.f, 0.f, 0.f);
                o.x = fmaf(pr, vv.x, o.x); o.y = fmaf(pr, vv.y, o.y); o.z = fmaf(pr, vv.z, o.z); o.w = fmaf(pr, vv.w, o.w);
            }
    }
    for (int i0 = (4 * GROUPS == 32 ? 32 * NPRE : 0) + grp; i0 < n; i0 += 4 * GROUPS) {
// ... 1487 lines not shown
```

Before: 1491.

## Emit split-bf16 activation tiles from encoder producers and consume them in Q4 GEMMs

Encoder RMS norm, attention prefill and the SwiGLU GEMM epilogue now write their outputs directly in the pre-split bf16 hi/lo tile layout that the Q4 GEMM consumes. A new XIN template path in the GEMM kernel loads these pre-swizzled tiles instead of converting f32 rows on the fly. This aims to cut per-GEMM conversion work and global traffic in the encoder prefill. The trade-off is padding buffers to 16 rows and adding more kernel specializations and layout-consistency checks across layers. Since this touches only the encoder, the decode throughput metric may move little.

```diff
diff --git a/voxtral-mini-realtime-rs_amd/csrc/vox_api.cpp b/voxtral-mini-realtime-rs_amd/csrc/vox_api.cpp
--- a/voxtral-mini-realtime-rs_amd/csrc/vox_api.cpp
+++ b/voxtral-mini-realtime-rs_amd/csrc/vox_api.cpp
@@ -1145,15 +1145,31 @@
     int ksp_wo = ksp ? 2 : 0;
     if (ksp) { if (const char* e = knob_str("VOX_ENC_SPLITK_WO")) ksp_wo = atoi(e) > 1 ? std::min(atoi(e), ksp) : 0; }
     for (int l = 0; ksp_wo && l < c.enc_layers; l++) if (m->enc[l].wo.w.fmt != WFMT_Q4_0 || !m->enc[l].wo.w.qt || m->enc[l].wo.w.nb / 4 < ksp_wo || m->enc[l].wo.w.nb % 4) ksp_wo = 0;
-    const size_t need = c1_floats + (size_t)Mfull * D + (size_t)Mtot * D + (size_t)Mtot * QD * 4 + (size_t)Mtot * F + (size_t)(M4 + 1) * m->ad0.w.N + (size_t)ksp * Mtot * D + 1024;
+    int xf_qkv = 0, xf_wo = 0, xf_w13 = 0, xf_w2 = 0;
+    if (Mtot > 48 && !(knob_str("VOX_ENC_XF") && atoi(knob_str("VOX_ENC_XF")) == 0)) {
+        xf_qkv = q4_gemm_xf_rows_form(m->enc[0].wqkv.w, Mtot, 0); xf_wo = q4_gemm_xf_rows_form(m->enc[0].wo.w, Mtot, ksp_wo);
+        xf_w13 = q4_gemm_xf_rows_form(m->enc[0].w13.w, Mtot, 0); xf_w2 = q4_gemm_xf_rows_form(m->enc[0].w2.w, Mtot, ksp);
+        for (int l = 1; l < c.enc_layers; l++) {
+            const EncLayer& L = m->enc[l];
+            if (q4_gemm_xf_rows_form(L.wqkv.w, Mtot, 0) != xf_qkv) xf_qkv = 0;
+            if (q4_gemm_xf_rows_form(L.wo.w, Mtot, ksp_wo) != xf_wo) xf_wo = 0;
+            if (q4_gemm_xf_rows_form(L.w13.w, Mtot, 0) != xf_w13) xf_w13 = 0;
+            if (q4_gemm_xf_rows_form(L.w2.w, Mtot, ksp) != xf_w2) xf_w2 = 0;
+        }
+        if (D % 128 || D > 4096) xf_qkv = xf_w13 = 0;
+        if (!xf_w13 || F % 128) xf_w2 = 0;
+    }
+    const size_t Mt16 = ((size_t)Mtot + 15) / 16 * 16;
+    const size_t need = c1_floats + (size_t)Mfull * D + Mt16 * D + (size_t)Mtot * QD * 3 + Mt16 * QD + Mt16 * F + (size_t)(M4 + 1) * m->ad0.w.N + (size_t)ksp * Mtot * D + 1024;
     VOXCHK(ensure(&m->ws, &m->ws_floats, need));
     if (forms) { forms->Mtot = Mtot; forms->ksp = ksp; forms->ksp_wo = ksp_wo; forms->fused_rope = 0; }
-    float* c1 = m->ws; float* x0 = c1 + c1_floats / 64 * 64; float* x = x0 + (size_t)r0 * D; float* xn = x0 + (size_t)Mfull * D; float* qkv = xn + (size_t)Mtot * D;
-    float* att = qkv + (size_t)Mtot * QD * 3; float* ffn = att + (size_t)Mtot * QD; float* ah = ffn + (size_t)Mtot * F; float* w2p = ah + (size_t)(M4 + 1) * m->ad0.w.N;
+    float* c1 = m->ws; float* x0 = c1 + c1_floats / 64 * 64; float* x = x0 + (size_t)r0 * D; float* xn = x0 + (size_t)Mfull * D; float* qkv = xn + Mt16 * D;
+    float* att = qkv + (size_t)Mtot * QD * 3; float* ffn = att + Mt16 * QD; float* ah = ffn + Mt16 * F; float* w2p = ah + (size_t)(M4 + 1) * m->ad0.w.N;
+    uint16_t* const xn_xf = reinterpret_cast<uint16_t*>(xn); uint16_t* const att_xf = reinterpret_cast<uint16_t*>(att); uint16_t* const ffn_xf = reinterpret_cast<uint16_t*>(ffn);
     const int* d_len = nullptr; const int* d_roff = nullptr; const int* d_rpos = nullptr;
     if (n > 1 || packed) {
         HIPCHK(hipMemsetAsync(x, 0, (size_t)Mtot * D * 4, s));
-        HIPCHK(hipMemsetAsync(att, 0, (size_t)Mtot * QD * 4, s));
+        HIPCHK(hipMemsetAsync(att, 0, Mt16 * QD * 4, s));
         if (!m->d_seq_len) HIPCHK(hipMalloc((void**)&m->d_seq_len, 128 * sizeof(int)));
         m->h_seq_len.assign(S.begin(), S.end());
         HIPCHK(hipMemcpyAsync(m->d_seq_len, m->h_seq_len.data(), (size_t)n * 4, hipMemcpyHostToDevice, s));
@@ -1174,12 +1190,16 @@
         VOXCHK(conv_stem_dev(m, d_mels[i], T[i], c1, x0 + (packed ? (size_t)roff[i] : (size_t)i * S_pad) * D));
     }
     const int seq_rows = packed ? 0 : n > 1 ? S_pad : 0;
+    if (xf_wo && Mt16 > (size_t)Mtot && !(n > 1 || packed)) HIPCHK(hipMemsetAsync(att + (Mt16 - 16) * QD, 0, (size_t)16 * QD * 4, s));
+    if (xf_w2 && Mt16 > (size_t)Mtot) HIPCHK(hipMemsetAsync(ffn + (Mt16 - 16) * F, 0, (size_t)16 * F * 4, s));
     for (int l = 0; l < c.enc_layers; l++) {
         const EncLayer& L = m->enc[l];
-        if (ksp && l > 0) HIPCHK(launch_rms_norm_sumk(x, D, Mtot, D, w2p, (size_t)Mtot * D, ksp, L.attn_norm, c.norm_eps, xn, D, s));
+        if (ksp && l > 0) HIPCHK(launch_rms_norm_sumk(x, D, Mtot, D, w2p, (size_t)Mtot * D, ksp, L.attn_norm, c.norm_eps, xn, D, s, xf_qkv ? xn_xf : nullptr, xf_qkv == 2));
+        else if (xf_qkv) HIPCHK(launch_rms_norm_xf_rows(x, D, Mtot, D, L.attn_norm, c.norm_eps, xn_xf, xf_qkv == 2, s));
         else HIPCHK(launch_rms_norm(x, D, Mtot, D, L.attn_norm, nullptr, c.norm_eps, xn, D, s));
         if (Mtot > 48) {
             GemmParams g{}; g.w = L.wqkv.w; g.x = xn; g.x_stride = D; g.M = Mtot; g.out = qkv; g.out_stride = 3 * QD; g.bias = L.wqkv.bias;
+            if (xf_qkv) { g.x = nullptr; g.xf = reinterpret_cast<const uint4*>(xn_xf); g.xf_nat = xf_qkv == 2; }
             g.rope_cos = m->enc_cos + (size_t)r0 * (hd / 2); g.rope_sin = m->enc_sin + (size_t)r0 * (hd / 2);
             g.hd = hd; g.n_q = 2 * QD; g.pos = d_rpos; g.rope_seq_rows = seq_rows;
             bool fused = false; HIPCHK(launch_q4_gemm(g, EPI_ROPE_ROWS, s, &fused));
@@ -1195,16 +1215,28 @@
         ap.out = att; ap.out_stride = QD; ap.M = S_pad - r0; ap.kv_len = S_pad; ap.n_heads = H; ap.n_kv_heads = H; ap.offset = r0; ap.window = c.enc_window;
         if (r0) { ap.prefix_k = m->pfx.enc_kv + (size_t)l * r0 * 2 * QD; ap.prefix_v = ap.prefix_k + QD; ap.prefix_len = r0; ap.prefix_row_stride = 2 * QD; ap.prefix_head_stride = hd; }
         ap.seq_len = d_len; ap.q_seq_stride = S_pad * 3 * QD; ap.out_seq_stride = S_pad * QD; ap.kv_seq_stride = (long)S_pad * 3 * QD; ap.seq_row_off = d_roff;
+        const bool att_xf_on = xf_wo && attn_prefill_xf_rows_ok(ap, hd, n);
+        if (att_xf_on) { ap.out_xf_rows = att_xf; ap.out_xf_nat = xf_wo == 2; }
         HIPCHK(launch_attn_prefill(ap, hd, s, n));
+        auto xf_gemm = [&](const Lin& lin, const uint16_t* xf, int form, float* out, int out_stride, int epi, const float* resid, int ksplit, uint16_t* xf_out, int xf_out_form) -> int32_t {
+            GemmParams g{}; g.w = lin.w; g.bias = lin.bias; g.xf = reinterpret_cast<const uint4*>(xf); g.xf_nat = form == 2; g.M = Mtot; g.out = out; g.out_stride = out_stride;
+            g.resid = resid; g.resid_stride = D; g.ksplit = ksplit; g.xf_out = xf_out; g.xf_out_nat = xf_out_form == 2;
+            HIPCHK(launch_q4_gemm(g, epi, s)); return VOX_OK;
+        };
         if (ksp_wo) {
-            VOXCHK(q4_linear_dev(cx, L.wo.w, L.wo.bias, att, QD, Mtot, w2p, D, EPI_STORE, nullptr, 0, ksp_wo));
-            HIPCHK(launch_rms_norm_sumk(x, D, Mtot, D, w2p, (size_t)Mtot * D, ksp_wo, L.ffn_norm, c.norm_eps, xn, D, s));
+            if (att_xf_on) VOXCHK(xf_gemm(L.wo, att_xf, xf_wo, w2p, D, EPI_STORE, nullptr, ksp_wo, nullptr, 0));
+            else VOXCHK(q4_linear_dev(cx, L.wo.w, L.wo.bias, att, QD, Mtot, w2p, D, EPI_STORE, nullptr, 0, ksp_wo));
+            HIPCHK(launch_rms_norm_sumk(x, D, Mtot, D, w2p, (size_t)Mtot * D, ksp_wo, L.ffn_norm, c.norm_eps, xn, D, s, xf_w13 ? xn_xf : nullptr, xf_w13 == 2));
         } else {
-            VOXCHK(q4_linear_dev(cx, L.wo.w, L.wo.bias, att, QD, Mtot, x, D, EPI_RESID, x, D));
-            HIPCHK(launch_rms_norm(x, D, Mtot, D, L.ffn_norm, nullptr, c.norm_eps, xn, D, s));
-        }
-        VOXCHK(q4_linear_dev(cx, L.w13.w, nullptr, xn, D, Mtot, ffn, F, EPI_SWIGLU));
-        if (ksp) VOXCHK(q4_linear_dev(cx, L.w2.w, L.w2.bias, ffn, F, Mtot, w2p, D, EPI_STORE, nullptr, 0, ksp));
+            if (att_xf_on) VOXCHK(xf_gemm(L.wo, att_xf, xf_wo, x, D, EPI_RESID, x, 0, nullptr, 0));
+            else VOXCHK(q4_linear_dev(cx, L.wo.w, L.wo.bias, att, QD, Mtot, x, D, EPI_RESID, x, D));
+            if (xf_w13) HIPCHK(launch_rms_norm_xf_rows(x, D, Mtot, D, L.ffn_norm, c.norm_eps, xn_xf, xf_w13 == 2, s));
+            else HIPCHK(launch_rms_norm(x, D, Mtot, D, L.ffn_norm, nullptr, c.norm_eps, xn, D, s));
+        }
+        if (xf_w13) VOXCHK(xf_gemm(L.w13, xn_xf, xf_w13, ffn, F, EPI_SWIGLU, nullptr, 0, xf_w2 ? ffn_xf : nullptr, xf_w2));
+        else VOXCHK(q4_linear_dev(cx, L.w13.w, nullptr, xn, D, Mtot, ffn, F, EPI_SWIGLU));
+        if (xf_w2) { if (ksp) VOXCHK(xf_gemm(L.w2, ffn_xf, xf_w2, w2p, D, EPI_STORE, nullptr, ksp, nullptr, 0)); else VOXCHK(xf_gemm(L.w2, ffn_xf, xf_w2, x, D, EPI_RESID, x, 0, nullptr, 0)); }
+        else if (ksp) VOXCHK(q4_linear_dev(cx, L.w2.w, L.w2.bias, ffn, F, Mtot, w2p, D, EPI_STORE, nullptr, 0, ksp));
         else VOXCHK(q4_linear_dev(cx, L.w2.w, L.w2.bias, ffn, F, Mtot, x, D, EPI_RESID, x, D));
     }
     if (ksp && c.enc_layers > 0) HIPCHK(launch_rms_norm_sumk(x, D, Mtot, D, w2p, (size_t)Mtot * D, ksp, m->enc_norm, c.norm_eps, xn, D, s));
diff --git a/voxtral-mini-realtime-rs_amd/csrc/vox_kernels.h b/voxtral-mini-realtime-rs_amd/csrc/vox_kernels.h
--- a/voxtral-mini-realtime-rs_amd/csrc/vox_kernels.h
+++ b/voxtral-mini-realtime-rs_amd/csrc/vox_kernels.h
@@ -69,7 +69,10 @@
     int rope_seq_rows;
     int wide_mt; long xf_gstride , xf_out_gstride , ssq_part_gstride, ssq_out_gstride ;
     int wide_rows;
-};
+    int xf_nat;
+    int xf_out_nat;
+};
+int q4_gemm_xf_rows_form(const Q4W& w, int M, int ksplit);
 struct WidePlan { int kz, sps, ntw; };
 bool q4_wide_plan(const Q4W& w, int mt, int epi, WidePlan* pl);
 size_t q4_wide_planes_bytes(const Q4W& w, int mt, const WidePlan& pl);
@@ -84,7 +87,9 @@
 hipError_t launch_q4_dequant(Q4W w, float* out, hipStream_t s);
 hipError_t launch_rms_norm(const float* x, int x_stride, int rows, int dim, const float* gamma, const float* mul,
                            float eps, float* out, int out_stride, hipStream_t s);
-hipError_t launch_rms_norm_sumk(float* x, int x_stride, int rows, int dim, const float* part, size_t part_stride, int ksplit, const float* gamma, float eps, float* out, int out_stride, hipStream_t s);
+hipError_t launch_rms_norm_sumk(float* x, int x_stride, int rows, int dim, const float* part, size_t part_stride, int ksplit, const float* gamma, float eps, float* out, int out_stride, hipStream_t s,
+                                uint16_t* xf_rows = nullptr, int xf_nat = 0);
+hipError_t launch_rms_norm_xf_rows(const float* x, int x_stride, int rows, int dim, const float* gamma, float eps, uint16_t* xf_rows, int xf_nat, hipStream_t s);
 int q4_skinny_mt2_plan(const Q4W& w, int M);
 hipError_t launch_xf_rows(const float* x, int x_stride, int M, int K, uint16_t* xf, hipStream_t s);
 hipError_t launch_q4_skinny_mt2_planes(const GemmParams& p, int KZ, hipStream_t s);
@@ -112,6 +117,7 @@
     const int* seq_len;
     const int* seq_row_off;
     uint16_t* out_xf_tiles; long out_xf_tile_stride;
+    uint16_t* out_xf_rows; int out_xf_nat;
     uint16_t* out_xf;
     long out_xf_gstride;
     int prefer_gqa;
@@ -124,6 +130,7 @@
 };
 hipError_t launch_attn_prefill(const AttnParams& p, int hd, hipStream_t s, int n_seq = 1);
 bool attn_prefill_prefix_ok(const AttnParams& p, int hd, int n_seq);
+bool attn_prefill_xf_rows_ok(const AttnParams& p, int hd, int n_seq);
 bool attn_prefill_small_ok(const AttnParams& p, int hd, int n_seq);
 hipError_t launch_attn_decode(const AttnParams& p, int hd, int max_seq, hipStream_t s, int n_seq = 1);
 hipError_t launch_attn_decode_paged(const AttnParams& p, int hd, hipStream_t s, int n_seq);
diff --git a/voxtral-mini-realtime-rs_amd/csrc/vox_kernels.hip b/voxtral-mini-realtime-rs_amd/csrc/vox_kernels.hip
--- a/voxtral-mini-realtime-rs_amd/csrc/vox_kernels.hip
+++ b/voxtral-mini-realtime-rs_amd/csrc/vox_kernels.hip
@@ -731,6 +731,42 @@
     split_pair(v.x, v.z, hi, lo); *reinterpret_cast<uint32_t*>(xf + base) = hi; *reinterpret_cast<uint32_t*>(xf + plane + base) = lo;
     split_pair(v.y, v.w, hi, lo); *reinterpret_cast<uint32_t*>(xf + base + 4) = hi; *reinterpret_cast<uint32_t*>(xf + plane + base + 4) = lo;
 }
+__device__ __forceinline__ size_t xf_tile_elems(int K) { return (size_t)2 * (K >> 7) * 256 * 8; }
+__device__ __forceinline__ void xf_rows_store4(uint16_t* __restrict__ xf, int K, int row, int k, float4 v, int nat) {
+    uint16_t* t = xf + (size_t)(row >> 4) * xf_tile_elems(K);
+    if (!nat) { xf_store4(t, K, row & 15, k, v); return; }
+    const int q = k >> 7, j = (k >> 5) & 3, e = k & 31, half = e >> 4, g = (e & 15) >> 2;
+    const size_t base = ((size_t)((q * 4 + j) * 64 + g * 16 + (row & 15))) * 8 + 4 * half;
+    const size_t plane = (size_t)(K >> 7) * 256 * 8;
+    uint2 hi, lo;
+    split_pair(v.x, v.y, hi.x, lo.x); split_pair(v.z, v.w, hi.y, lo.y);
+    *reinterpret_cast<uint2*>(t + base) = hi; *reinterpret_cast<uint2*>(t + plane + base) = lo;
+}
+__device__ __forceinline__ void xf_rows_store8(uint16_t* __restrict__ xf, int K, int row, int k32, int g, float4 a, float4 b, int nat) {
+    uint4* t = reinterpret_cast<uint4*>(xf + (size_t)(row >> 4) * xf_tile_elems(K)) + (size_t)((k32 >> 5) * 64 + g * 16 + (row & 15));
+    uint4 hi, lo;
+    if (nat) split_bf16x8(a, b, hi, lo);
+    else { split_pair(a.x, a.z, hi.x, lo.x); split_pair(b.x, b.z, hi.y, lo.y); split_pair(a.y, a.w, hi.z, lo.z); split_pair(b.y, b.w, hi.w, lo.w); }
+    t[0] = hi; t[(size_t)(K >> 7) * 256] = lo;
+}
+__device__ __forceinline__ void xf_rows_store_wave(uint16_t* __restrict__ xf, int K, int row, int c, float4 v, int nat, bool live) {
+    uint32_t h0, h1, l0, l1;
+    if (nat) { split_pair(v.x, v.y, h0, l0); split_pair(v.z, v.w, h1, l1); } else { split_pair(v.x, v.z, h0, l0); split_pair(v.y, v.w, h1, l1); }
+    const bool second = (c >> 2) & 1;
+    const uint32_t r0 = (uint32_t)__shfl_xor((int)(second ? h0 : l0), 4, 64), r1 = (uint32_t)__shfl_xor((int)(second ? h1 : l1), 4, 64);
+    if (!live) return;
+    const int k = 4 * c, g = c & 3;
+    uint4* t = reinterpret_cast<uint4*>(xf + (size_t)(row >> 4) * xf_tile_elems(K)) + (size_t)((k >> 5) * 64 + g * 16 + (row & 15)) + (second ? (size_t)(K >> 7) * 256 : 0);
+    const uint32_t a0 = second ? r0 : h0, a1 = second ? r1 : h1, b0 = second ? l0 : r0, b1 = second ? l1 : r1;
+    *t = nat ? make_uint4(a0, a1, b0, b1) : make_uint4(a0, b0, a1, b1);
+}
+__device__ __forceinline__ void xf_rows_store1(uint16_t* __restrict__ xf, int K, int row, int k, float v, int nat) {
+    const int q = k >> 7, j = (k >> 5) & 3, e = k & 31, half = e >> 4, g = (e & 15) >> 2, ix = e & 3;
+    const int sl = nat ? 4 * half + ix : 2 * half + (ix >> 1) + 4 * (ix & 1);
+    const size_t base = (size_t)(row >> 4) * xf_tile_elems(K) + ((size_t)((q * 4 + j) * 64 + g * 16 + (row & 15))) * 8 + sl;
+    uint32_t hi, lo; split_pair(v, 0.f, hi, lo);
+    xf[base] = (uint16_t)hi; xf[base + (size_t)(K >> 7) * 256 * 8] = (uint16_t)lo;
+}
 
 template <int EPI, int FMT>
 __global__ __launch_bounds__(256) __attribute__((amdgpu_waves_per_eu(2))) void q4_gemm_k32_kernel(const GemmParams p) {
@@ -808,7 +844,7 @@
         }
 }
 
-template <int MT, int NT, int EPI, int FMT, int TB = 0>
+template <int MT, int NT, int EPI, int FMT, int TB = 0, int XIN = 0>
 __global__ __launch_bounds__(256) __attribute__((amdgpu_waves_per_eu(2))) void q4_gemm_kernel(const GemmParams p) {
     extern __shared__ __attribute__((aligned(16))) uint4 glds[];
     constexpr int PLANE = 4 * MT * 64, BUF = 2 * PLANE;
@@ -825,6 +861,15 @@
         slot[i] = (j * MT + (sm >> 4)) * 64 + g * 16 + ((sm & 15) ^ (4 * j + g));
         xo_a[i] = 32 * j + (FMT == WFMT_Q4_0 ? 4 * g : 8 * g); xo_b[i] = 32 * j + (FMT == WFMT_Q4_0 ? 16 + 4 * g : 8 * g + 4);
     }
+    const uint4* xft[MT]; const size_t xf_plane = (size_t)nq * 256;
+    if (XIN) {
+#pragma unroll
+        for (int i = 0; i < MT; i++) {
+            const int j = tid >> 6, g = (tid >> 4) & 3, mi = tid & 15;
+            xft[i] = p.xf + (size_t)min((m0 >> 4) + i, ((M + 15) >> 4) - 1) * (2 * xf_plane) + tid;
+            slot[i] = (j * MT + i) * 64 + g * 16 + (mi ^ (4 * j + g));
+        }
+    }
     const int wg = lane >> 4;
     int rdl[4];
 #pragma unroll
@@ -850,8 +895,13 @@
     uint32_t wd[NT][4]; uint2 wsc[NT]; uint4 wdv[NT][4];
 #define VOX_GLOAD(Q_)                                                                                          \
     _Pragma("unroll") for (int i = 0; i < MT; i++) {                                                           \
-        xa[i] = *reinterpret_cast<const float4*>(xrow[i] + 128 * (Q_) + xo_a[i]);                              \
-        xb[i] = *reinterpret_cast<const float4*>(xrow[i] + 128 * (Q_) + xo_b[i]);                              \
+        if (XIN) {                               \
+            xa[i] = *reinterpret_cast<const float4*>(xft[i] + (size_t)256 * (Q_));                             \
+            xb[i] = *reinterpret_cast<const float4*>(xft[i] + xf_plane + (size_t)256 * (Q_));                  \
+        } else {                                                                                               \
+            xa[i] = *reinterpret_cast<const float4*>(xrow[i] + 128 * (Q_) + xo_a[i]);                          \
+            xb[i] = *reinterpret_cast<const float4*>(xrow[i] + 128 * (Q_) + xo_b[i]);                          \
+        }                                                                                                      \
     }                                                                                                          \
     _Pragma("unroll") for (int t = 0; t < NT; t++) {                                                           \
         if (FMT == WFMT_Q4_0) {                                                                                \
@@ -867,11 +917,16 @@
         uint4 hi_, lo_; split_bf16x8(sxa[i], sxb[i], hi_, lo_);                                                \
         glds[(BUF_) * BUF + slot[i]] = hi_; glds[(BUF_) * BUF + PLANE + slot[i]] = lo_;                        \
     }
+#define VOX_STAGE_XF(BUF_)                                                                                     \
+    _Pragma("unroll") for (int i = 0; i < MT; i++) {                                                           \
+        glds[(BUF_) * BUF + slot[i]] = make_uint4(__float_as_uint(xa[i].x), __float_as_uint(xa[i].y), __float_as_uint(xa[i].z), __float_as_uint(xa[i].w));         \
+        glds[(BUF_) * BUF + PLANE + slot[i]] = make_uint4(__float_as_uint(xb[i].x), __float_as_uint(xb[i].y), __float_as_uint(xb[i].z), __float_as_uint(xb[i].w)); \
+    }
     VOX_GLOAD(qb)
     float4 sxa[MT], sxb[MT];
 #pragma unroll
     for (int i = 0; i < MT; i++) { sxa[i] = xa[i]; sxb[i] = xb[i]; }
-    VOX_STAGE(0)
+    if (XIN) { VOX_STAGE_XF(0) } else { VOX_STAGE(0) }
     uint32_t cwd[NT][4]; uint2 csc[NT]; uint4 cwdv[NT][4];
 #pragma unroll
     for (int t = 0; t < NT; t++) { csc[t] = wsc[t];
@@ -881,8 +936,11 @@
     __syncthreads();
     for (int q = qb; q < qe; q++) {
         const int buf = (q - qb) & 1;
-#pragma unroll
-        for (int i = 0; i < MT; i++) { sxa[i] = xa[i]; sxb[i] = xb[i]; }
+        if (XIN) { if (q + 1 < qe) { VOX_STAGE_XF(buf ^ 1) } }
+        else {
+#pragma unroll
+            for (int i = 0; i < MT; i++) { sxa[i] = xa[i]; sxb[i] = xb[i]; }
+        }
         uint32_t nwd[NT][4]; uint2 nsc[NT]; uint4 nwdv[NT][4];
 #pragma unroll
         for (int t = 0; t < NT; t++) { nsc[t] = wsc[t];
@@ -911,7 +969,7 @@
             }
         }
         if (q + 1 < qe) {
-            VOX_STAGE(buf ^ 1)
+            if (!XIN) { VOX_STAGE(buf ^ 1) }
 #pragma unroll
             for (int t = 0; t < NT; t++) { csc[t] = nsc[t];
 #pragma unroll
@@ -921,6 +979,7 @@
     }
 #undef VOX_GLOAD
 #undef VOX_STAGE
+#undef VOX_STAGE_XF
 #pragma unroll
     for (int t = 0; t < NT; t++) {
         const float bias = (p.bias && wok[t] && kz == 0) ? p.bias[wn[t]] : 0.f;
@@ -932,7 +991,10 @@
                 float v = acc[t][i][r] + bias;
                 if (EPI == EPI_SWIGLU) {
                     const float other = dpp_mov<0xB1>(v);
-                    if (m < M && wok[t] && !(wn[t] & 1)) p.out[(size_t)m * p.out_stride + (wn[t] >> 1)] = silu_f(v) * other;
+                    if (m < M && wok[t] && !(wn[t] & 1)) {
+                        if (XIN && p.xf_out) xf_rows_store1(p.xf_out, N >> 1, m, wn[t] >> 1, silu_f(v) * other, p.xf_out_nat);
+                        else p.out[(size_t)m * p.out_stride + (wn[t] >> 1)] = silu_f(v) * other;
+                    }
                 } else if (m < M && wok[t]) {
                     if (EPI == EPI_RESID) v = v + p.resid[(size_t)m * p.resid_stride + wn[t]];
                     if (EPI == EPI_GELU) v = gelu_f(v);
@@ -1880,7 +1942,7 @@
 __device__ __forceinline__ uint4 vbuf_u4(vsrd_t sd, unsigned voff, unsigned soff) { const vu32x4_t v = __builtin_bit_cast(vu32x4_t, __builtin_amdgcn_raw_buffer_load_b128(sd, (int)voff, (int)soff, 0)); return make_uint4(v.x, v.y, v.z, v.w); }
 __device__ __forceinline__ uint2 vbuf_u2(vsrd_t sd, unsigned voff, unsigned soff) { const vu32x2_t v = __builtin_bit_cast(vu32x2_t, __builtin_amdgcn_raw_buffer_load_b64(sd, (int)voff, (int)soff, 0)); return make_uint2(v.x, v.y); }
 
-template <int WGM, int WGN, int EPI>
+template <int WGM, int WGN, int EPI, int XIN = 0>
 __global__ __launch_bounds__(256) __attribute__((amdgpu_waves_per_eu(2))) void q4_gemm_big_kernel(const GemmParams p) {
     constexpr int BM = 64 * WGM, MTB = BM / 16;
     constexpr int PAIRS = 4 * MTB, NU = PAIRS / 4;
@@ -1892,7 +1954,9 @@
     const int m0 = blockIdx.y * BM, n0 = blockIdx.x * (64 * WGN);
     const int n_tiles = (N + 15) >> 4;
     static_assert(WGM == 1, "the staging map below is written for 64-row workgroups");
-    const vsrd_t xsrd = vmake_srd(p.x, (unsigned)min((size_t)0xFFFFFFF0u, ((size_t)(M - 1) * p.x_stride + (size_t)p.w.K) * 4));
+    const vsrd_t xsrd = XIN ? vmake_srd(p.xf, (unsigned)((size_t)((M + 15) >> 4) * nq * 8192))
+                            : vmake_srd(p.x, (unsigned)min((size_t)0xFFFFFFF0u, ((size_t)(M - 1) * p.x_stride + (size_t)p.w.K) * 4));
+    const unsigned xfo = (unsigned)((size_t)((m0 >> 4) + wave) * nq * 8192) + (unsigned)lane * 16u, xfpl = (unsigned)nq * 4096u;
     const vsrd_t qsrd = vmake_srd(p.w.qt, (unsigned)((size_t)n_tiles * nq * 1024)), ssrd = vmake_srd(p.w.st, (unsigned)((size_t)n_tiles * nq * 128));
     const unsigned xo = (unsigned)(((size_t)min(m0 + 16 * wave + li, M - 1) * p.x_stride + 4 * g) * 4);
     const unsigned qo = (unsigned)lane * 16u, so = (unsigned)li * 8u;
@@ -1905,8 +1969,12 @@
     float4 xa[NU], xb[NU]; uint4 bw[4], bwn[4]; uint2 bs[4], bsn[4];
 #define VOX_ALOAD(Q_)                                                                                          \
     _Pragma("unroll") for (int u = 0; u < NU; u++) {                                                           \
-        xa[u] = vbuf_f4(xsrd, xo + (unsigned)(Q_) * 512u + (unsigned)u * 128u, 0);                             \
-        xb[u] = vbuf_f4(xsrd, xo + (unsigned)(Q_) * 512u + (unsigned)u * 128u + 64u, 0); }
+        if (XIN) {      \
+            xa[u] = vbuf_f4(xsrd, xfo + (unsigned)(Q_) * 4096u + (unsigned)u * 1024u, 0);                      \
+            xb[u] = vbuf_f4(xsrd, xfo + xfpl + (unsigned)(Q_) * 4096u + (unsigned)u * 1024u, 0);               \
+        } else {                                                                                               \
+            xa[u] = vbuf_f4(xsrd, xo + (unsigned)(Q_) * 512u + (unsigned)u * 128u, 0);                         \
+            xb[u] = vbuf_f4(xsrd, xo + (unsigned)(Q_) * 512u + (unsigned)u * 128u + 64u, 0); } }
 #define VOX_BLOAD(W_, S_, Q_)                                                                                  \
     _Pragma("unroll") for (int t = 0; t < 4; t++) {                                                            \
         W_[t] = vbuf_u4(qsrd, qo + (unsigned)(Q_) * 1024u, (unsigned)(tile0 + t) * (unsigned)nq * 1024u);      \
@@ -1918,8 +1986,13 @@
 #define VOX_STAGE(BUF_)                                                                                        \
     _Pragma("unroll") for (int u = 0; u < NU; u++) {      \
         uint4 hi, lo;                                                                                          \
-        split_pair(xa[u].x, xa[u].z, hi.x, lo.x); split_pair(xb[u].x, xb[u].z, hi.y, lo.y);                    \
-        split_pair(xa[u].y, xa[u].w, hi.z, lo.z); split_pair(xb[u].y, xb[u].w, hi.w, lo.w);                    \
+        if (XIN) {                                                                                             \
+            hi = make_uint4(__float_as_uint(xa[u].x), __float_as_uint(xa[u].y), __float_as_uint(xa[u].z), __float_as_uint(xa[u].w)); \
+            lo = make_uint4(__float_as_uint(xb[u].x), __float_as_uint(xb[u].y), __float_as_uint(xb[u].z), __float_as_uint(xb[u].w)); \
+        } else {                                                                                               \
+            split_pair(xa[u].x, xa[u].z, hi.x, lo.x); split_pair(xb[u].x, xb[u].z, hi.y, lo.y);                \
+            split_pair(xa[u].y, xa[u].w, hi.z, lo.z); split_pair(xb[u].y, xb[u].w, hi.w, lo.w);                \
+        }                                                                                                      \
         f32x4 c_ = __builtin_amdgcn_mfma_f32_16x16x32_bf16(as_bf16x8(hi), m136, (f32x4){0.f, 0.f, 0.f, 0.f}, 0, 0, 0); \
         c_ = __builtin_amdgcn_mfma_f32_16x16x32_bf16(as_bf16x8(lo), m136, c_, 0, 0, 0);                        \
         if (li == 0) *reinterpret_cast<f32x4*>(&s_bcs[(BUF_) == blds ? 0 : 1][u][wave][g][0]) = c_;             \
@@ -1984,7 +2057,10 @@
                 float v = acc[t][i][r] + bias;
                 if (EPI == EPI_SWIGLU) {
                     const float other = dpp_mov<0xB1>(v);
-                    if (m < M && nok && !(n & 1)) p.out[(size_t)m * p.out_stride + (n >> 1)] = silu_f(v) * other;
+                    if (m < M && nok && !(n & 1)) {
+                        if (XIN && p.xf_out) xf_rows_store1(p.xf_out, N >> 1, m, n >> 1, silu_f(v) * other, p.xf_out_nat);
+                        else p.out[(size_t)m * p.out_stride + (n >> 1)] = silu_f(v) * other;
+                    }
                 } else if (EPI == EPI_ROPE_ROWS) {
                     const float other = dpp_mov<0xB1>(v);
                     if (m < M && nok) {
@@ -2005,11 +2081,11 @@
             }
     }
 }
-template <int WGM, int WGN>
+template <int WGM, int WGN, int XIN = 0>
 static hipError_t gemm_big_launch(const GemmParams& p, int epi, hipStream_t s) {
     dim3 grid((p.w.N + 64 * WGN - 1) / (64 * WGN), (p.M + 64 * WGM - 1) / (64 * WGM));
     const size_t lds = (size_t)2 * 2 * 4 * (4 * WGM) * 64 * sizeof(uint4);
-#define VOX_E(E_) case E_: { auto kern = q4_gemm_big_kernel<WGM, WGN, E_>; static DevOnce done;          \
+#define VOX_E(E_) case E_: { auto kern = q4_gemm_big_kernel<WGM, WGN, E_, XIN>; static DevOnce done;         \
         hipError_t e = ensure_dyn_lds(kern, lds, &done); if (e != hipSuccess) return e;                       \
         gemm_form_note(E_ == EPI_ROPE_ROWS ? GEMM_FORM_BIG_ROPE : GEMM_FORM_BIG); kern<<<grid, dim3(256), lds, s>>>(p); break; }
     switch (epi) { VOX_E(EPI_STORE) VOX_E(EPI_RESID) VOX_E(EPI_GELU) VOX_E(EPI_SWIGLU) VOX_E(EPI_ROPE_ROWS) default: return hipErrorInvalidValue; }
@@ -2201,12 +2277,12 @@
     return e;
 }
 
-template <int MT, int NT, int FMT, int TB = 0>
+template <int MT, int NT, int FMT, int TB = 0, int XIN = 0>
 static hipError_t gemm_launch_mn(const GemmParams& p, int epi, hipStream_t s) {
     if (p.ksplit > 1 && (epi != EPI_STORE || p.ksplit > p.w.nb / 4)) return hipErrorInvalidValue;
     dim3 grid((p.w.N + 64 * NT - 1) / (64 * NT), (p.M + 16 * MT - 1) / (16 * MT), p.ksplit > 1 ? p.ksplit : 1);
     const size_t lds = (size_t)2 * 2 * 4 * MT * 64 * sizeof(uint4);
-#define VOX_E(E_) case E_: { auto kern = q4_gemm_kernel<MT, NT, E_, FMT, TB>; static DevOnce done;      \
+#define VOX_E(E_) case E_: { auto kern = q4_gemm_kernel<MT, NT, E_, FMT, TB, XIN>; static DevOnce done;     \
         hipError_t e = ensure_dyn_lds(kern, lds, &done); if (e != hipSuccess) return e;                       \
         gemm_form_note(TB ? (NT == 2 ? GEMM_FORM_TILE_22_TB : GEMM_FORM_TILE_21_TB) : MT == 1 ? (NT == 2 ? GEMM_FORM_TILE_12 : GEMM_FORM_TILE_11) : (NT == 2 ? GEMM_FORM_TILE_22 : GEMM_FORM_TILE_21)); \
         kern<<<grid, dim3(256), lds, s>>>(p); break; }
@@ -2244,6 +2320,15 @@
 }
 hipError_t launch_rope(float* buf, int M, int stride, int n_rot, int hd, int pos_off, const float* cos_t, const float* sin_t, hipStream_t s, int seq_rows, const int* row_pos);
 static hipError_t launch_q4_gemm_epi(const GemmParams& p, int epi, hipStream_t s, bool* fused_rope);
+int q4_gemm_xf_rows_form(const Q4W& w, int M, int ksplit) {
+    if (M <= 48 || w.fmt != WFMT_Q4_0 || !w.qt || !w.st || w.nb % 4 || w.K % 128) return 0;
+    if (((size_t)((M + 15) & ~15) + 64) * w.K * 4 >= 0xFFFFFFF0ull) return 0;
+    const int big = env_int("VOX_GEMM_BIG");
+    const long wg14 = (long)((w.N + 255) / 256) * ((M + 63) / 64);
+    const bool fits32 = (size_t)((w.N + 15) / 16) * (w.nb / 4) * 1024 < 0xFFFFFFF0ull;
+    if (ksplit <= 1 && fits32 && w.N % 256 == 0 && (big == 1 || (big == 0 && wg14 >= 200))) return 1;
+    return 2;
+}
 hipError_t launch_q4_gemm(const GemmParams& p, int epi, hipStream_t s, bool* fused_rope) {
     if (fused_rope) *fused_rope = false;
     if (epi != EPI_ROPE_ROWS) return launch_q4_gemm_epi(p, epi, s, nullptr);
@@ -2258,11 +2343,23 @@
     int epi = epi_in == EPI_ROPE_ROWS ? EPI_STORE : epi_in;
     if (p.w.K % 32 || p.M <= 0) return hipErrorInvalidValue;
     if (p.kv_pos && !(p.xf && p.M <= 16)) return hipErrorInvalidValue;
-    if (p.ksplit > 1 && (p.M <= 48 || p.xf || p.w.nb % 4 || p.w.fmt == WFMT_F32)) return hipErrorInvalidValue;
+    if (p.ksplit > 1 && (p.M <= 48 || p.w.nb % 4 || p.w.fmt == WFMT_F32)) return hipErrorInvalidValue;
     if (p.w.fmt == WFMT_F32) {
         if (p.xf) return hipErrorInvalidValue;
         GemmParams v = p; v.w.fmt = WFMT_BF16X2; v.w.qt = nullptr; v.w.st = nullptr;
         return launch_dense2_gemm(v, epi, s);
+    }
+    if (p.xf && p.M > 48) {
+        const int form = q4_gemm_xf_rows_form(p.w, p.M, p.ksplit);
+        if (!form || form != (p.xf_nat ? 2 : 1) || (p.xf_out && epi != EPI_SWIGLU)) return hipErrorInvalidValue;
+        if (epi != EPI_STORE && epi != EPI_RESID && epi != EPI_GELU && epi != EPI_SWIGLU) return hipErrorInvalidValue;
+        if (form == 1) {
+            const long wg14 = (long)((p.w.N + 255) / 256) * ((p.M + 63) / 64);
+            if (epi_in == EPI_ROPE_ROWS && wg14 >= 1024 && (p.hd & (p.hd - 1)) == 0 && !knob_str("VOX_NO_ROPE_FUSE")) { if (fused_rope) *fused_rope = true; return gemm_big_launch<1, 4, 1>(p, EPI_ROPE_ROWS, s); }
+            return gemm_big_launch<1, 4, 1>(p, epi, s);
+        }
+        const long wg22 = (long)((p.w.N + 127) / 128) * ((p.M + 31) / 32);
+        return wg22 >= 128 ? gemm_launch_mn<2, 2, WFMT_Q4_0, 1, 1>(p, epi, s) : gemm_launch_mn<2, 1, WFMT_Q4_0, 1, 1>(p, epi, s);
     }
     if (p.xf && p.M > 16) return (p.M <= 48 && p.w.fmt == WFMT_Q4_0 && p.w.nb % 4 == 0 && p.w.qt && p.w.st && (epi == EPI_STORE || epi == EPI_RESID || epi == EPI_GELU || epi == EPI_SWIGLU))
                                      ? launch_q4_skinny_mt(p, epi, s) : hipErrorInvalidValue;
@@ -2287,8 +2384,11 @@
 
 __global__ __launch_bounds__(256) void rms_norm_kernel(const float* __restrict__ x, int x_stride, int rows, int dim,
                                                        const float* __restrict__ gamma, const float* __restrict__ mul,
-                                                       float eps, float* __restrict__ out, int out_stride) {
-    const int row = min(blockIdx.x * 4 + (threadIdx.x >> 6), rows - 1), lane = threadIdx.x & 63;
+                                                       float eps, float* __restrict__ out, int out_stride,
+                                                       uint16_t* __restrict__ xf = nullptr, int xf_nat = 0) {
+    const int row_raw = blockIdx.x * 4 + (threadIdx.x >> 6);
+    const int row = min(row_raw, rows - 1), lane = threadIdx.x & 63;
+    const bool pad = row_raw >= rows;
     const float4* xr = reinterpret_cast<const float4*>(x + (size_t)row * x_stride);
     const int n4 = dim >> 2;
     float4 v[16];
@@ -2309,7 +2409,7 @@
     { float4 t = (T_); const float4 gm = g4[C_];                                                                \
       t.x = (t.x / rms) * gm.x; t.y = (t.y / rms) * gm.y; t.z = (t.z / rms) * gm.z; t.w = (t.w / rms) * gm.w;   \
       if (mul) { const float4 mm = m4[C_]; t.x *= mm.x; t.y *= mm.y; t.z *= mm.z; t.w *= mm.w; }               \
-      o[C_] = t; }
+      if (xf) xf_rows_store_wave(xf, dim, row_raw, C_, pad ? make_float4(0.f, 0.f, 0.f, 0.f) : t, xf_nat, true); else o[C_] = t; }
 #pragma unroll
     for (int i = 0; i < 16; i++) {
         const int c = lane + 64 * i;
@@ -2355,9 +2455,13 @@
     }
 }
 __global__ __launch_bounds__(256) VOX_NO_PK_F32 void rms_norm_sumk_kernel(float* __restrict__ x, int x_stride, int rows, int dim, const float* __restrict__ part, size_t part_stride, int ks,
-                                                            const float* __restrict__ gamma, float eps, float* __restrict__ out, int out_stride) {
+                                                            const float* __restrict__ gamma, float eps, float* __restrict__ out, int out_stride,
+                                                            uint16_t* __restrict__ xf = nullptr, int xf_nat = 0) {
     const int row = blockIdx.x * 4 + (threadIdx.x >> 6), lane = threadIdx.x & 63;
-    if (row >= rows) return;
+    if (row >= rows) {
+        if (xf && row < ((rows + 15) & ~15)) for (int c = lane; c < (dim >> 2); c += 64) xf_rows_store_wave(xf, dim, row, c, make_float4(0.f, 0.f, 0.f, 0.f), xf_nat, true);
+        return;
+    }
     float4* xr = reinterpret_cast<float4*>(x + (size_t)row * x_stride);
     const int n4 = dim >> 2;
     float4 v[16];
@@ -2379,12 +2483,22 @@
 #pragma unroll
     for (int i = 0; i < 16; i++) {
         const int c = lane + 64 * i;
-        if (c < n4) { const float4 g = g4[c]; o[c] = make_float4((v[i].x / rms) * g.x, (v[i].y / rms) * g.y, (v[i].z / rms) * g.z, (v[i].w / rms) * g.w); }
-    }
-}
-hipError_t launch_rms_norm_sumk(float* x, int x_stride, int rows, int dim, const float* part, size_t part_stride, int ksplit, const float* gamma, float eps, float* out, int out_stride, hipStream_t s) {
-    if (dim % 4 || dim > 4096 || rows <= 0 || ksplit < 1) return hipErrorInvalidValue;
-    rms_norm_sumk_kernel<<<dim3((rows + 3) / 4), dim3(256), 0, s>>>(x, x_stride, rows, dim, part, part_stride, ksplit, gamma, eps, out, out_stride);
+        if (c < n4) {
+            const float4 g = g4[c]; const float4 t = make_float4((v[i].x / rms) * g.x, (v[i].y / rms) * g.y, (v[i].z / rms) * g.z, (v[i].w / rms) * g.w);
+            if (xf) xf_rows_store_wave(xf, dim, row, c, t, xf_nat, true); else o[c] = t;
+        }
+    }
+}
+hipError_t launch_rms_norm_sumk(float* x, int x_stride, int rows, int dim, const float* part, size_t part_stride, int ksplit, const float* gamma, float eps, float* out, int out_stride, hipStream_t s,
+                                uint16_t* xf_rows, int xf_nat) {
+    if (dim % 4 || dim > 4096 || rows <= 0 || ksplit < 1 || (xf_rows && dim % 128)) return hipErrorInvalidValue;
+    const int grid_rows = xf_rows ? (rows + 15) & ~15 : rows;
+    rms_norm_sumk_kernel<<<dim3((grid_rows + 3) / 4), dim3(256), 0, s>>>(x, x_stride, rows, dim, part, part_stride, ksplit, gamma, eps, out, out_stride, xf_rows, xf_nat);
+    return hipGetLastError();
+}
+hipError_t launch_rms_norm_xf_rows(const float* x, int x_stride, int rows, int dim, const float* gamma, float eps, uint16_t* xf_rows, int xf_nat, hipStream_t s) {
+    if (dim % 128 || dim > 4096 || rows <= 0 || !xf_rows) return hipErrorInvalidValue;
+    rms_norm_kernel<<<dim3((((rows + 15) & ~15) + 3) / 4), dim3(256), 0, s>>>(x, x_stride, rows, dim, gamma, nullptr, eps, nullptr, 0, xf_rows, xf_nat);
     return hipGetLastError();
 }
 hipError_t launch_rms_norm_xf_sumk(float* x, int x_stride, int rows, int dim, const float* planes, int kz, const float* gamma, const float* mul, float eps,
@@ -2704,9 +2818,17 @@
     if (m < M) {
         const float inv = 1.0f / lsum;
         float* op = p.out + (p.seq_row_off ? (size_t)p.seq_row_off[sq] * p.out_stride : (size_t)sq * p.out_seq_stride) + (size_t)m * p.out_stride + h * HD + 4 * g;
-#pragma unroll
-        for (int dt = 0; dt < DT; dt++)
-            *reinterpret_cast<float4*>(op + dt * 16) = make_float4(o[dt][0] * inv, o[dt][1] * inv, o[dt][2] * inv, o[dt][3] * inv);
+        if (p.out_xf_rows) {
+            const int row = (p.seq_row_off ? p.seq_row_off[sq] : sq * (int)(p.out_seq_stride / p.out_stride)) + m;
+#pragma unroll
+            for (int dt = 0; dt < DT; dt += 2)
+                xf_rows_store8(p.out_xf_rows, p.n_heads * HD, row, h * HD + dt * 16, g, make_float4(o[dt][0] * inv, o[dt][1] * inv, o[dt][2] * inv, o[dt][3] * inv),
+                               make_float4(o[dt + 1][0] * inv, o[dt + 1][1] * inv, o[dt + 1][2] * inv, o[dt + 1][3] * inv), p.out_xf_nat);
+        } else {
+#pragma unroll
+            for (int dt = 0; dt < DT; dt++)
+                *reinterpret_cast<float4*>(op + dt * 16) = make_float4(o[dt][0] * inv, o[dt][1] * inv, o[dt][2] * inv, o[dt][3] * inv);
+        }
     }
 }
 template <int HD, bool PFX>
@@ -2794,7 +2916,12 @@
            p.M >= 1 && p.kv_len == p.prefix_len + p.M && (p.q_stride % 4) == 0 && (p.kv_row_stride % 4) == 0 && (p.prefix_row_stride % 4) == 0 && (p.prefix_head_stride % 4) == 0 &&
            !env_int("VOX_ATTN_F32");
 }
+bool attn_prefill_xf_rows_ok(const AttnParams& p, int hd, int n_seq) {
+    if (attn_prefill_small_ok(p, hd, n_seq) || env_int("VOX_ATTN_F32") || (hd != 64 && hd != 128) || (p.q_stride % 4) || (p.kv_row_stride % 4) || (p.n_heads * hd) % 128 || p.out_stride <= 0) return false;
+    return p.prefix_len > 0 ? attn_prefill_prefix_ok(p, hd, n_seq) : true;
+}
 hipError_t launch_attn_prefill(const AttnParams& p, int hd, hipStream_t s, int n_seq) {
+    if (p.out_xf_rows && !attn_prefill_xf_rows_ok(p, hd, n_seq)) return hipErrorInvalidValue;
     if (attn_prefill_small_ok(p, hd, n_seq)) return attn_prefill_small_launch(p, s, n_seq);
     if (p.out_xf_tiles) return hipErrorInvalidValue;
     const int f32_only = env_int("VOX_ATTN_F32");
```

Result: no change. 1498 (median of 6 runs) (+0.5%).
